# RashmikaDushan/MocapV2

Hardware: AMD Instinct MI355X
Metric: frames/sec (6-cam 1080p) (higher is better)
Workload: dtype u8+int64+f64; 1 GPU; 6-camera 1920x1080 synthetic IR frames, 8 markers (BASELINE.json configs[1]); cameras=6, width=1920, height=1080, markers=8, distortion=mild, frames_resident_in_hbm=True, batches_in_flight=3, resident_batches=3, status_ok=True, input=gray frames, parallelism=single launch, time-major

## Files before the change

include/mocap_hip.h:

```cpp
#ifndef MOCAP_HIP_H
#define MOCAP_HIP_H

#include <stddef.h>
#include <stdint.h>

#ifdef __cplusplus
extern "C" {
#endif

#define MOCAP_ABI_VERSION 7
#define MOCAP_API __attribute__((visibility("default")))

enum {
    MOCAP_OK = 0,
    MOCAP_E_INVALID = -1,
    MOCAP_E_HIP = -2,
    MOCAP_E_UNSUPPORTED = -3,
    MOCAP_E_STATE = -4
};

enum {
    MOCAP_BLOB_E_CANDIDATES = -2,
    MOCAP_BLOB_E_CONTOURS = -3,
    MOCAP_BLOB_E_STEPS = -4,
    MOCAP_BLOB_E_DEPTH = -5,
    MOCAP_CORR_E_GROUPS = -2,
    MOCAP_CORR_E_TRUNCATED = -3,
    MOCAP_CORR_E_BLOB = -4,
    MOCAP_FUND_E_SAMPLE = -2,
    MOCAP_FUND_E_DEGENERATE = -3
};

typedef struct mocap_ctx* mocap_ctx_t;

typedef struct mocap_blob_params {
    int32_t ksize;
    int32_t median;
    double thresh;
    double min_area;
    double min_circ;
} mocap_blob_params;

typedef struct mocap_contour {
    int32_t key, is_hole, sx, sy, npts, steps;
    int64_t a00, a10, a01;
    double area, perimeter;
    int32_t kept, cx, cy, link, parent, order;
} mocap_contour;

MOCAP_API int mocap_abi_version(void);
MOCAP_API const char* mocap_last_error(void);

MOCAP_API int mocap_ctx_create(int device_id, int width, int height, int n_slots, mocap_ctx_t* out);
MOCAP_API int mocap_ctx_destroy(mocap_ctx_t ctx);
MOCAP_API int mocap_sync(mocap_ctx_t ctx, void* stream);

MOCAP_API int mocap_set_blob_params(mocap_ctx_t ctx, const mocap_blob_params* p);

MOCAP_API int mocap_set_tuning(mocap_ctx_t ctx, const char* name, int value);

MOCAP_API int mocap_set_undistort(mocap_ctx_t ctx, int slot, const double K[9], const double dist[5], int* identity_out);

typedef struct mocap_undistort_info_t {
    int32_t identity;
    int32_t compact_table;
    int32_t early_out_provable;
    int32_t max_source_weight;
    int32_t sparse_path;
} mocap_undistort_info_t;
MOCAP_API int mocap_undistort_info(mocap_ctx_t ctx, int slot, mocap_undistort_info_t* out);

MOCAP_API int mocap_set_cameras(mocap_ctx_t ctx, int n, const double* K , const double* dist ,
                      const double* R , const double* t );
MOCAP_API int mocap_set_fundamentals(mocap_ctx_t ctx, int n, const double* F );

MOCAP_API int mocap_blob_centroids(mocap_ctx_t ctx, const void* frames_dev, int n_images, int cam_mod, int slot_base,
                         size_t image_stride, int pitch, int32_t* out_xy_dev, long xy_stride, int32_t* out_count_dev,
                         long count_stride, int max_blobs, void* stream);

MOCAP_API int mocap_filter_mask(mocap_ctx_t ctx, const void* frames_dev, int n_images, int cam_mod, int slot_base,
                      size_t image_stride, int pitch, uint32_t* mask_dev, void* stream);
MOCAP_API int mocap_contours_from_mask(mocap_ctx_t ctx, const uint32_t* mask_dev, int n_images, int32_t* out_xy_dev,
                             long xy_stride, int32_t* out_count_dev, long count_stride, int max_blobs,
                             mocap_contour* dbg_dev , int32_t* dbg_count_dev,
                             int dbg_cap, void* stream);

MOCAP_API int mocap_image_filter_u8(mocap_ctx_t ctx, const void* src_dev, void* dst_dev, int spitch, int dpitch, int order,
                          int slot, void* stream);
MOCAP_API int mocap_undistort_u8(mocap_ctx_t ctx, int slot, const void* src_dev, void* dst_dev, int spitch, int dpitch,
                       void* stream);
MOCAP_API int mocap_box_blur_u8(mocap_ctx_t ctx, const void* src_dev, void* dst_dev, int height, int width, int spitch,
                      int dpitch, int ksize, void* stream);
MOCAP_API int mocap_bayer_gray_u8(mocap_ctx_t ctx, const void* bayer_dev, void* gray_dev, int n_images, int height, int width,
                        long spitch, long dpitch, size_t src_image_stride, size_t dst_image_stride, int pattern,
                        int gray_shift, void* stream);
MOCAP_API int mocap_blob_centroids_bayer(mocap_ctx_t ctx, const void* bayer_frames_dev, void* gray_frames_dev, int n_images,
                               int cam_mod, int slot_base, size_t image_stride, int pitch, int pattern, int gray_shift,
                               int32_t* out_xy_dev, long xy_stride, int32_t* out_count_dev, long count_stride,
                               int max_blobs, void* stream);
MOCAP_API int mocap_demosaic_u8(mocap_ctx_t ctx, const void* bayer_dev, void* bgr_dev, int height, int width, int spitch,
                      void* stream);

MOCAP_API int mocap_correspond(mocap_ctx_t ctx, const void* pts_dev, long pt_stride_t, long pt_stride_c,
                     const int32_t* counts_dev, long cnt_stride_t, long cnt_stride_c, int pts_f64, int T, int C,
                     int P, double cutoff, int max_groups, double* root_xyz_dev, double* root_err_dev,
                     double* root_grp_dev, int32_t* root_idx_dev, int32_t* order_dev, int32_t* n_roots_dev,
                     void* stream);

MOCAP_API int mocap_epipolar_scores(mocap_ctx_t ctx, const void* roots_dev, int n_roots, const void* cand_dev, int n_cand,
                                    int pts_f64, int f_index, double* dist_dev, float* lines_dev, void* stream);

MOCAP_API int mocap_triangulate_batch(mocap_ctx_t ctx, const double* pts_dev, const uint8_t* valid_dev, int N, int C,
                            int compact_k, double* xyz_dev, int32_t* ok_dev, void* stream);
MOCAP_API int mocap_reproject_batch(mocap_ctx_t ctx, const double* pts_dev, const uint8_t* valid_dev, const double* xyz_dev,
                          int N, int C, int compact_k, double* mse_dev, int32_t* ok_dev, void* stream);

MOCAP_API int mocap_ba_residuals(mocap_ctx_t ctx, const double* params_host, int B, const double* pts_dev,
                                 const uint8_t* valid_dev, int N, int C, float* residuals_host, int32_t* counts_host,
                                 void* stream);

MOCAP_API int mocap_fundamental_ransac(mocap_ctx_t ctx, int n_pairs, const double* pts_a_dev, const double* pts_b_dev,
                                       const int32_t* pair_offset_host, const int32_t* samples_dev, int H, double threshold,
                                       int refit, double* F_sample_dev, double* F_refit_dev, uint8_t* inlier_dev,
                                       int32_t* status_dev, int32_t* counts_dev, void* stream);

enum {
    MOCAP_RIG_STOP_MAX_ITERS = 1,
    MOCAP_RIG_STOP_FTOL = 2,
    MOCAP_RIG_STOP_LAMBDA = 3,
    MOCAP_RIG_STOP_CHOLESKY = 4,
    MOCAP_RIG_E_LAYOUT = -2,
    MOCAP_RIG_E_BEHIND = -3
};
MOCAP_API int mocap_rig_bundle_adjust(mocap_ctx_t ctx, int C, int N, int n_obs, const int32_t* obs_offset_dev,
                                      const int32_t* obs_cam_dev, const double* obs_uv_dev, double* poses_dev, double* points_dev,
                                      int max_iters, double ftol, double lambda0, double* history_dev, double* result_dev,
                                      void* stream);
MOCAP_API int mocap_rig_linearize(mocap_ctx_t ctx, int C, int N, int n_obs, const int32_t* obs_offset_dev,
                                  const int32_t* obs_cam_dev, const double* obs_uv_dev, const double* poses_dev,
                                  const double* points_dev, double lambda, double* cost_dev, double* gradient_dev, double* S_dev,
                                  double* rhs_dev, int32_t* status_dev, void* stream);

enum {
    MOCAP_INTR_E_LAYOUT = -2,
    MOCAP_INTR_E_BEHIND = -3,
    MOCAP_INTR_E_DEGENERATE = -4
};
MOCAP_API int mocap_intrinsics_calibrate(mocap_ctx_t ctx, int n_cams, const int32_t* view_offset_host,
                                         const int32_t* point_offset_host, const double* obj_xy_dev, const double* img_uv_dev,
                                         const int32_t* image_size_host, int have_start, int max_iters, double ftol,
                                         double lambda0, double* kd_dev, double* view_poses_dev, double* view_rms_dev,
                                         double* history_dev, double* result_dev, void* stream);
MOCAP_API int mocap_intrinsics_linearize(mocap_ctx_t ctx, int n_cams, const int32_t* view_offset_host,
                                         const int32_t* point_offset_host, const double* obj_xy_dev, const double* img_uv_dev,
                                         const double* kd_dev, const double* view_poses_dev, double lambda, double* cost_dev,
                                         double* gradient_dev, double* S_dev, double* rhs_dev, int32_t* status_dev, void* stream);

#define MOCAP_COMM_ID_BYTES 128
MOCAP_API int mocap_comm_unique_id(void* id_out );
MOCAP_API int mocap_comm_available(void);
MOCAP_API int mocap_comm_init(mocap_ctx_t ctx, const void* id , int rank, int world);
MOCAP_API int mocap_comm_share(mocap_ctx_t dst, mocap_ctx_t src);
MOCAP_API int mocap_comm_destroy(mocap_ctx_t ctx);
MOCAP_API int mocap_allgather_centroids(mocap_ctx_t ctx, const int32_t* local_records_dev, int32_t* gathered_dev,
                                        long ints_per_rank, void* stream);

MOCAP_API int mocap_tile_stats(mocap_ctx_t ctx, uint64_t* tiles, uint64_t* skipped);
MOCAP_API int mocap_profile_enable(mocap_ctx_t ctx, int on);
MOCAP_API int mocap_profile_read(mocap_ctx_t ctx, double ms[5], int launches[5]);

#ifdef __cplusplus
}
#endif
#endif
```

mocapv2_amd/_abi.py:

```python
import ctypes as C
import os

_HERE = os.path.dirname(os.path.abspath(__file__))
LIB_PATH = os.path.join(_HERE, "libmocap_hip.so")
ABI_VERSION = 7
COMM_ID_BYTES = 128


class MocapError(RuntimeError):
    def __init__(self, code, msg):
        super().__init__(f"libmocap_hip error {code}: {msg}")
        self.code = code


class BlobParams(C.Structure):
    _fields_ = [("ksize", C.c_int32), ("median", C.c_int32), ("thresh", C.c_double), ("min_area", C.c_double),
                ("min_circ", C.c_double)]


class UndistortInfo(C.Structure):
    _fields_ = [("identity", C.c_int32), ("compact_table", C.c_int32), ("early_out_provable", C.c_int32),
                ("max_source_weight", C.c_int32), ("sparse_path", C.c_int32)]


class Contour(C.Structure):
    _fields_ = [("key", C.c_int32), ("is_hole", C.c_int32), ("sx", C.c_int32), ("sy", C.c_int32), ("npts", C.c_int32),
                ("steps", C.c_int32), ("a00", C.c_int64), ("a10", C.c_int64), ("a01", C.c_int64), ("area", C.c_double),
                ("perimeter", C.c_double), ("kept", C.c_int32), ("cx", C.c_int32), ("cy", C.c_int32), ("link", C.c_int32),
                ("parent", C.c_int32), ("order", C.c_int32)]


_vp, _i, _d, _sz, _l = C.c_void_p, C.c_int, C.c_double, C.c_size_t, C.c_long
_dp, _ip = C.POINTER(C.c_double), C.POINTER(C.c_int)

SIGNATURES = {
    "mocap_abi_version": [],
    "mocap_last_error": [],
    "mocap_ctx_create": [_i, _i, _i, _i, C.POINTER(_vp)],
    "mocap_ctx_destroy": [_vp],
    "mocap_sync": [_vp, _vp],
    "mocap_set_blob_params": [_vp, C.POINTER(BlobParams)],
    "mocap_set_tuning": [_vp, C.c_char_p, _i],
    "mocap_set_undistort": [_vp, _i, _dp, _dp, _ip],
    "mocap_undistort_info": [_vp, _i, C.POINTER(UndistortInfo)],
    "mocap_set_cameras": [_vp, _i, _dp, _dp, _dp, _dp],
    "mocap_set_fundamentals": [_vp, _i, _dp],
    "mocap_blob_centroids": [_vp, _vp, _i, _i, _i, _sz, _i, _vp, _l, _vp, _l, _i, _vp],
    "mocap_blob_centroids_bayer": [_vp, _vp, _vp, _i, _i, _i, _sz, _i, _i, _i, _vp, _l, _vp, _l, _i, _vp],
    "mocap_filter_mask": [_vp, _vp, _i, _i, _i, _sz, _i, _vp, _vp],
    "mocap_contours_from_mask": [_vp, _vp, _i, _vp, _l, _vp, _l, _i, _vp, _vp, _i, _vp],
    "mocap_image_filter_u8": [_vp, _vp, _vp, _i, _i, _i, _i, _vp],
    "mocap_undistort_u8": [_vp, _i, _vp, _vp, _i, _i, _vp],
    "mocap_box_blur_u8": [_vp, _vp, _vp, _i, _i, _i, _i, _i, _vp],
    "mocap_demosaic_u8": [_vp, _vp, _vp, _i, _i, _i, _vp],
    "mocap_bayer_gray_u8": [_vp, _vp, _vp, _i, _i, _i, _l, _l, _sz, _sz, _i, _i, _vp],
    "mocap_correspond": [_vp, _vp, _l, _l, _vp, _l, _l, _i, _i, _i, _i, _d, _i, _vp, _vp, _vp, _vp, _vp, _vp, _vp],
    "mocap_epipolar_scores": [_vp, _vp, _i, _vp, _i, _i, _i, _vp, _vp, _vp],
    "mocap_ba_residuals": [_vp, _dp, _i, _vp, _vp, _i, _i, C.POINTER(C.c_float), _ip, _vp],
    "mocap_fundamental_ransac": [_vp, _i, _vp, _vp, _ip, _vp, _i, _d, _i, _vp, _vp, _vp, _vp, _vp, _vp],
    "mocap_rig_bundle_adjust": [_vp, _i, _i, _i, _vp, _vp, _vp, _vp, _vp, _i, _d, _d, _vp, _vp, _vp],
    "mocap_rig_linearize": [_vp, _i, _i, _i, _vp, _vp, _vp, _vp, _vp, _d, _vp, _vp, _vp, _vp, _vp, _vp],
    "mocap_intrinsics_calibrate": [_vp, _i, _ip, _ip, _vp, _vp, _ip, _i, _i, _d, _d, _vp, _vp, _vp, _vp, _vp, _vp],
    "mocap_intrinsics_linearize": [_vp, _i, _ip, _ip, _vp, _vp, _vp, _vp, _d, _vp, _vp, _vp, _vp, _vp, _vp],
    "mocap_triangulate_batch": [_vp, _vp, _vp, _i, _i, _i, _vp, _vp, _vp],
    "mocap_reproject_batch": [_vp, _vp, _vp, _vp, _i, _i, _i, _vp, _vp, _vp],
    "mocap_comm_unique_id": [_vp],
    "mocap_comm_available": [],
    "mocap_comm_init": [_vp, _vp, _i, _i],
    "mocap_comm_share": [_vp, _vp],
    "mocap_comm_destroy": [_vp],
    "mocap_allgather_centroids": [_vp, _vp, _vp, _l, _vp],
    "mocap_tile_stats": [_vp, C.POINTER(C.c_uint64), C.POINTER(C.c_uint64)],
    "mocap_profile_enable": [_vp, _i],
    "mocap_profile_read": [_vp, _dp, _ip],
}

_lib = None


def load():
    global _lib
    if _lib is not None:
        return _lib
    if not os.path.exists(LIB_PATH):
        raise RuntimeError(f"{LIB_PATH} is missing: build it with `make -C mocapv2_amd/csrc` "
                           "(hipcc --offload-arch=gfx950); there is no CPU fallback")
    try:
        import torch
    except ImportError:
        pass
    lib = C.CDLL(LIB_PATH)
    for name, args in SIGNATURES.items():
        fn = getattr(lib, name)
        fn.argtypes = args
        fn.restype = C.c_char_p if name == "mocap_last_error" else C.c_int
    if lib.mocap_abi_version() != ABI_VERSION:
        raise RuntimeError(f"libmocap_hip ABI {lib.mocap_abi_version()} != expected {ABI_VERSION}")
    _lib = lib
    return lib


def check(rc):
    if rc != 0:
        msg = load().mocap_last_error()
        raise MocapError(rc, msg.decode() if msg else "")
```

mocapv2_amd/csrc/abi.hip:

```cpp
#include <hip/hip_runtime.h>
#include <stdint.h>
#include <stdio.h>
#include <stdarg.h>
#include <stdlib.h>
#include <string.h>
#include <math.h>
#include <string>
#include <vector>
#include <mutex>
#include <memory>
#include <dlfcn.h>
#include "../../include/mocap_hip.h"
#include "kernels.h"

using namespace mocap;

static_assert(sizeof(mocap_contour) == sizeof(ContourRec), "debug record layout");

static thread_local std::string g_err;

static int fail(int code, const char* fmt, ...)
{
    char buf[512];
    va_list ap;
    va_start(ap, fmt);
    vsnprintf(buf, sizeof(buf), fmt, ap);
    va_end(ap);
    g_err = buf;
    return code;
}

#define HIP_TRY(expr)                                                                                         \
    do {                                                                                                      \
        hipError_t e_ = (expr);                                                                               \
        if (e_ != hipSuccess) return fail(MOCAP_E_HIP, "%s failed: %s", #expr, hipGetErrorString(e_));        \
    } while (0)
#define TRY(expr) do { if (int rc_ = (expr)) return rc_; } while (0)

template <class T, bool Pinned = false>
struct Buf {
    T* p = nullptr;
    size_t n = 0;
    Buf() = default;
    Buf(Buf&& o) : p(o.p), n(o.n) { o.p = nullptr; o.n = 0; }
    Buf& operator=(Buf&& o) { if (this != &o) { release(); p = o.p; n = o.n; o.p = nullptr; o.n = 0; } return *this; }
    ~Buf() { release(); }
    operator T*() const { return p; }
    T* operator->() const { return p; }
    void release()
    {
        if (p) (void)(Pinned ? hipHostFree(p) : hipFree(p));
        p = nullptr; n = 0;
    }
    int reserve(size_t count, bool zero = false)
    {
        if (count <= n) return 0;
        if (p) { HIP_TRY(hipDeviceSynchronize()); release(); }
        HIP_TRY(Pinned ? hipHostMalloc((void**)&p, sizeof(T) * count) : hipMalloc((void**)&p, sizeof(T) * count));
        if (zero) HIP_TRY(hipMemset(p, 0, sizeof(T) * count));
        n = count;
        return 0;
    }
};

struct EvPair { hipEvent_t a, b; };
constexpr size_t PROBE_BYTES = 128 * mocap::PROBE_STRIDE * sizeof(uint32_t);
using mocap::PROBE_STRIDE;

struct SharedComm {
    void* comm = nullptr;
    int rank = 0, world = 1, device = 0;
    hipEvent_t last = nullptr;
    bool have_last = false;
    std::mutex mu;
    bool (*destroy_comm)(void*) = nullptr;
    ~SharedComm()
    {
        if (!comm && !last) return;
        (void)hipSetDevice(device);
        if (last) { if (have_last) (void)hipEventSynchronize(last); (void)hipEventDestroy(last); }
        if (comm && destroy_comm) (void)destroy_comm(comm);
    }
};

struct Tuning {
    int rows = 68;
    int general_filter = 0;
    int skip_dark = 1;
    int dense_boxes = 0;
    int remap_pipeline = 1;
    int cluster = 1;
    int wide_quads_remap = 34, wide_quads_identity = 34;
    int wide_bands = 1;
    int wide_fork = 0;
    int box_prio = 0, scan_prio = 0, contour_prio = 0, corr_prio = 0;
    int box_stage_bytes = BOX_SCAP;
    int box_blocks_per_cu = 0;
    int box_timing = 0, contour_timing = 0, follow_timing = 0;
    int scan_wide = 1;
    int rows_staged = 0;
    int wide_blocks_per_cu = 3;
    int rows_stage_dw = -1;
    int scan_serial = 1;
    int scan_hotmap = 1;
    int scan_blocks_per_cu = 0;
    int scan_slices = 1;
    int excess_base = -1;
    int base_sel = 1;
    int probe_debug = 0;
    int contour_boxes = 1;
    int contours_split = 1;
    int contour_defer = 1;
    int mark_blocks_per_cu = 0;
    int contour_blocks_per_cu = 0;
    int corr_threads = 256;
    int corr_step_groups = 0;
};
struct TuneName { const char* name; int Tuning::*field; int lo, hi; };
static const TuneName kTuneNames[] = {
    {"rows", &Tuning::rows, 16, 68}, {"general_filter", &Tuning::general_filter, 0, 1}, {"skip_dark", &Tuning::skip_dark, 0, 1},
    {"dense_boxes", &Tuning::dense_boxes, 0, 1}, {"remap_pipeline", &Tuning::remap_pipeline, 0, 1}, {"cluster", &Tuning::cluster, 0, 1},
    {"wide_quads_remap", &Tuning::wide_quads_remap, 0, 100000}, {"wide_quads_identity", &Tuning::wide_quads_identity, 0, 100000},
    {"wide_bands", &Tuning::wide_bands, 1, 4}, {"wide_fork", &Tuning::wide_fork, 0, 1},
    {"box_prio", &Tuning::box_prio, 0, 1}, {"scan_prio", &Tuning::scan_prio, 0, 3}, {"contour_prio", &Tuning::contour_prio, 0, 3},
    {"corr_prio", &Tuning::corr_prio, 0, 3}, {"box_stage_bytes", &Tuning::box_stage_bytes, 0, BOX_SCAP},
    {"box_blocks_per_cu", &Tuning::box_blocks_per_cu, 0, 32}, {"box_timing", &Tuning::box_timing, 0, 1},
    {"contour_timing", &Tuning::contour_timing, 0, 1}, {"follow_timing", &Tuning::follow_timing, 0, 2}, {"scan_wide", &Tuning::scan_wide, 0, 1}, {"scan_hotmap", &Tuning::scan_hotmap, 0, 2}, {"scan_serial", &Tuning::scan_serial, 0, 1}, {"rows_staged", &Tuning::rows_staged, 0, 1}, {"wide_blocks_per_cu", &Tuning::wide_blocks_per_cu, 1, 8}, {"rows_stage_dw", &Tuning::rows_stage_dw, -1, 1 << 20}, {"scan_blocks_per_cu", &Tuning::scan_blocks_per_cu, 0, 64}, {"scan_slices", &Tuning::scan_slices, 1, 64}, {"excess_base", &Tuning::excess_base, -1, 254},
    {"base_sel", &Tuning::base_sel, 0, 1}, {"probe_debug", &Tuning::probe_debug, 0, 1}, {"contour_boxes", &Tuning::contour_boxes, 0, 1},
    {"contours_split", &Tuning::contours_split, 0, 1}, {"contour_blocks_per_cu", &Tuning::contour_blocks_per_cu, 0, 16}, {"mark_blocks_per_cu", &Tuning::mark_blocks_per_cu, 0, 16}, {"contour_defer", &Tuning::contour_defer, 0, 2}, {"corr_threads", &Tuning::corr_threads, 64, 256},
    {"corr_step_groups", &Tuning::corr_step_groups, 0, 0x7fffffff},
};
static bool tune_set(Tuning& t, const char* name, int v)
{
    for (const TuneName& n : kTuneNames)
        if (!strcmp(n.name, name)) {
            t.*(n.field) = v < n.lo ? n.lo : (v > n.hi ? n.hi : v);
            return true;
        }
    return false;
}
static Tuning tuning_from_env()
{
    Tuning t;
    for (const TuneName& n : kTuneNames) {
        char env[64] = "MOCAP_";
        size_t k = strlen(env);
        for (const char* p = n.name; *p && k + 1 < sizeof(env); p++) env[k++] = (char)((*p >= 'a' && *p <= 'z') ? *p - 32 : *p);
        env[k] = 0;
        const char* e = getenv(env);
        if (e && *e) tune_set(t, n.name, atoi(e));
    }
    { const char* e = getenv("MOCAP_WIDE_QUADS"); int r_ = 0, i_ = 0;
      if (e && sscanf(e, "%d,%d", &r_, &i_) == 2) { tune_set(t, "wide_quads_remap", r_); tune_set(t, "wide_quads_identity", i_); } }
    return t;
}

struct mocap_ctx {
    int device = 0, W = 0, H = 0, n_slots = 0, wpr = 0;
    int box_grid = 2048;
    int n_cu = 256;
    mocap_blob_params prm{5, 5, 255 * 0.85, 500.0, 0.5};
    Tuning tune;
    Buf<uint32_t> maps;
    Buf<uint32_t> map4;
    Buf<ushort4> srcbox;
    Buf<ushort4> rowbox;
    Buf<uint32_t> map_flags;
    std::vector<int> slot_state;
    std::vector<int> slot_compact;
    std::vector<uint32_t> slot_wmax;
    Buf<uint2> reach;
    Buf<uint8_t> cflags;
    Buf<uint32_t> mask; size_t mask_images = 0;
    bool mask_dirty = false;
    Buf<uint32_t> cells;
    int last_images = 0;
    Buf<uint32_t> hotmap;
    Buf<uint32_t> tile_rows;
    int tile_rows_flip = 0;
    int tile_rows_hold[2] = {0, 0};
    Buf<uint32_t> cur_box;
    Buf<BoxItem> items;
    Buf<uint4> wide_tiles;
    Buf<uint32_t> n_items;
    hipStream_t side = nullptr; hipEvent_t ev_fork = nullptr, ev_join = nullptr;
    int base_sel = 1; int probe_age = 0; bool probe_pending = false; Buf<uint32_t> probe_dev; Buf<uint32_t, true> probe_host; hipEvent_t probe_ev = nullptr;
    bool walk_count_zeroed = false;
    int probe_images = 0;
    bool hot_dense = false;
    Buf<uint32_t> cells_ext, cur_box_ext; size_t cells_ext_images = 0;
    Buf<uint32_t> mask_out;
    Buf<uint32_t> mask_in;
    Buf<uint8_t> gray_scratch;
    Buf<uint8_t> cwork; size_t cwork_images = 0;
    Buf<uint64_t> walk_list, link_list;
    Buf<uint32_t> walk_count;
    Buf<CameraTable> cams; int n_cam = 0, n_F = 0;
    Buf<double> scratch;
    Buf<double> ba_obj;
    Buf<char> fund_scratch;
    Buf<char> rig_scratch;
    Buf<char> intr_scratch;
    Buf<char, true> ba_pinned;
    std::shared_ptr<struct SharedComm> comm;
    bool profiling = false;
    std::vector<EvPair> ev[5];
    std::mutex mu;
};

static int set_device(mocap_ctx* c) { HIP_TRY(hipSetDevice(c->device)); return 0; }

struct ScanTurn { std::mutex mu; hipEvent_t done = nullptr; bool have = false; };
static ScanTurn g_scan_turn[64];

struct Tiling { int rows, n_cgroups, n_strips; };
static Tiling tiling(const mocap_ctx* c)
{
    Tiling t;
    t.rows = c->tune.rows;
    if (c->H < 4 * 32) t.rows = (c->H + 3) / 4 > 8 ? (c->H + 3) / 4 : 8;
    t.n_cgroups = (c->H + 4 * t.rows - 1) / (4 * t.rows);
    t.n_strips = (c->W + 239) / 240;
    return t;
}

static size_t source_cells(const mocap_ctx* c) { return (size_t)((c->H + 7) / 8) * ((c->W + 7) / 8); }
static size_t cells_per_image(const mocap_ctx* c) { Tiling t = tiling(c); return (size_t)t.n_cgroups * 4 * t.n_strips; }
static uint32_t* slot_map(const mocap_ctx* c, int slot) { return c->maps ? c->maps + (size_t)slot * c->H * c->W : nullptr; }
static uint32_t* slot_mapw(const mocap_ctx* c, int slot) { return c->maps ? c->maps + (size_t)(c->n_slots + slot) * c->H * c->W : nullptr; }
static uint32_t* slot_map4(const mocap_ctx* c, int slot) { return c->map4 ? c->map4 + (size_t)slot * c->H * c->W : nullptr; }

struct IdBytes { char internal[MOCAP_COMM_ID_BYTES]; };
namespace {
struct Rccl {
    void* lib = nullptr;
    int (*GetUniqueId)(void*) = nullptr;
    int (*CommInitRank)(void**, int, IdBytes, int) = nullptr;
    int (*CommDestroy)(void*) = nullptr;
    int (*AllGather)(const void*, void*, size_t, int, void*, hipStream_t) = nullptr;
    const char* (*GetErrorString)(int) = nullptr;
};
}
static Rccl g_rccl;
static std::mutex g_rccl_mu;
static int load_rccl()
{
    std::lock_guard<std::mutex> lk(g_rccl_mu);
    if (g_rccl.lib) return 0;
    void* h = dlopen("librccl.so.1", RTLD_NOW | RTLD_GLOBAL);
    if (!h) h = dlopen("librccl.so", RTLD_NOW | RTLD_GLOBAL);
    if (!h) h = dlopen("/opt/rocm/lib/librccl.so.1", RTLD_NOW | RTLD_GLOBAL);
    if (!h) return fail(MOCAP_E_UNSUPPORTED, "librccl.so.1 not found: %s", dlerror());
    Rccl r;
    r.GetUniqueId = (decltype(r.GetUniqueId))dlsym(h, "ncclGetUniqueId");
    r.CommInitRank = (decltype(r.CommInitRank))dlsym(h, "ncclCommInitRank");
    r.CommDestroy = (decltype(r.CommDestroy))dlsym(h, "ncclCommDestroy");
    r.AllGather = (decltype(r.AllGather))dlsym(h, "ncclAllGather");
    r.GetErrorString = (decltype(r.GetErrorString))dlsym(h, "ncclGetErrorString");
    if (!r.GetUniqueId || !r.CommInitRank || !r.CommDestroy || !r.AllGather || !r.GetErrorString)
        return fail(MOCAP_E_UNSUPPORTED, "librccl lacks an expected symbol");
    r.lib = h;
    g_rccl = r;
    return 0;
}
#define RCCL_TRY(expr)                                                                                        \
    do {                                                                                                      \
        int r_ = (expr);                                                                                      \
        if (r_ != 0) return fail(MOCAP_E_HIP, "%s failed: %s", #expr, g_rccl.GetErrorString(r_));             \
    } while (0)

struct Carver {
    char* base;
    size_t used = 0;
    template <class T> void take(T*& p, size_t count) { p = base ? (T*)(base + used) : nullptr; used += (sizeof(T) * count + 15) & ~(size_t)15; }
};

extern "C" {

int mocap_abi_version(void) { return MOCAP_ABI_VERSION; }
const char* mocap_last_error(void) { return g_err.c_str(); }

int mocap_ctx_create(int device_id, int width, int height, int n_slots, mocap_ctx_t* out)
{
    if (!out || width < 1 || height < 1 || width > 32767 || height > 32767 || n_slots < 1 || n_slots > 64)
        return fail(MOCAP_E_INVALID, "mocap_ctx_create: bad geometry %dx%d slots=%d", width, height, n_slots);
    int ndev = 0;
    HIP_TRY(hipGetDeviceCount(&ndev));
    if (device_id < 0 || device_id >= ndev) return fail(MOCAP_E_HIP, "mocap_ctx_create: no HIP device %d (%d visible)", device_id, ndev);
    HIP_TRY(hipSetDevice(device_id));
    std::unique_ptr<mocap_ctx, int (*)(mocap_ctx*)> c(new mocap_ctx(), mocap_ctx_destroy);
    c->device = device_id; c->W = width; c->H = height; c->n_slots = n_slots; c->wpr = (width + 31) / 32;
    c->tune = tuning_from_env();
    c->base_sel = c->tune.base_sel;
    {
        hipDeviceProp_t prop;
        if (hipGetDeviceProperties(&prop, device_id) == hipSuccess && prop.multiProcessorCount > 0) {
            c->box_grid = box_filter_blocks_per_cu() * prop.multiProcessorCount;
            c->n_cu = prop.multiProcessorCount;
            if (c->tune.box_blocks_per_cu >= 1) c->box_grid = c->tune.box_blocks_per_cu * prop.multiProcessorCount;
        }
    }
    c->slot_state.assign(n_slots, 0);
    c->slot_compact.assign(n_slots, 0);
    c->slot_wmax.assign(n_slots, 0);
    TRY(c->map_flags.reserve(n_slots + 64, true));
    TRY(c->n_items.reserve(256, true));
    TRY(c->probe_dev.reserve(PROBE_BYTES / sizeof(uint32_t)));
    TRY(c->probe_host.reserve(PROBE_BYTES / sizeof(uint32_t)));
    HIP_TRY(hipEventCreateWithFlags(&c->probe_ev, hipEventDisableTiming));
    HIP_TRY(hipEventCreateWithFlags(&c->ev_fork, hipEventDisableTiming));
    HIP_TRY(hipEventCreateWithFlags(&c->ev_join, hipEventDisableTiming));
    TRY(c->cams.reserve(1, true));
    *out = c.release();
    return MOCAP_OK;
}

int mocap_ctx_destroy(mocap_ctx_t c)
{
    if (!c) return MOCAP_OK;
    (void)hipSetDevice(c->device);
    for (auto& v : c->ev) for (auto& p : v) { (void)hipEventDestroy(p.a); (void)hipEventDestroy(p.b); }
    (void)mocap_comm_destroy(c);
    if (c->side) { (void)hipStreamSynchronize(c->side); (void)hipStreamDestroy(c->side); }
    if (c->ev_fork) (void)hipEventDestroy(c->ev_fork);
    if (c->ev_join) (void)hipEventDestroy(c->ev_join);
    if (c->probe_ev) { (void)hipEventSynchronize(c->probe_ev); (void)hipEventDestroy(c->probe_ev); }
    delete c;
    return MOCAP_OK;
}

int mocap_sync(mocap_ctx_t c, void* stream)
{
    if (!c) return fail(MOCAP_E_INVALID, "null context");
// ... 30 lines not shown
    std::lock_guard<std::mutex> lk(c->mu);
    size_t per = (size_t)c->H * c->W;
    TRY(c->maps.reserve(per * c->n_slots * 2));
    TRY(c->map4.reserve(per * c->n_slots + 4));
    const int ncx_ = (c->W + 7) / 8, ncy_ = (c->H + 7) / 8;
    TRY(c->srcbox.reserve((size_t)ncx_ * ncy_ * c->n_slots));
    const int n_strips_ = tiling(c).n_strips;
    TRY(c->rowbox.reserve((size_t)c->H * n_strips_ * c->n_slots));
    MapArgs m;
    memcpy(m.K, K, sizeof(m.K));
    memcpy(m.dist, dist, sizeof(m.dist));
    m.H = c->H; m.W = c->W;
    m.map = slot_map(c, slot);
    m.mapw = slot_mapw(c, slot);
    m.map4 = slot_map4(c, slot);
    m.flags = c->map_flags + slot;
    HIP_TRY(hipMemset(m.flags, 0, sizeof(uint32_t)));
    launch_undistort_map(m, 0);
    HIP_TRY(hipGetLastError());
    uint32_t flags = 0;
    HIP_TRY(hipMemcpy(&flags, m.flags, sizeof(flags), hipMemcpyDeviceToHost));
    c->slot_state[slot] = (flags & 1u) ? 2 : 1;
    c->slot_compact[slot] = (flags & 2u) ? 0 : 1;
    c->slot_wmax[slot] = c->slot_state[slot] == 1 ? 1024u : 0u;
    launch_srcbox(m.map4, c->srcbox + (size_t)ncx_ * ncy_ * slot, c->H, c->W, 0);
    HIP_TRY(hipGetLastError());
    launch_rowbox(m.map4, c->rowbox + (size_t)c->H * n_strips_ * slot, c->H, c->W, n_strips_, 0);
    HIP_TRY(hipGetLastError());
    std::vector<uint32_t> edge((size_t)ncx_ * ncy_, 0);
    std::vector<int> reach32((size_t)ncx_ * ncy_ * 4);
    for (size_t i = 0; i < reach32.size(); i += 2) { reach32[i] = 0x7fffffff; reach32[i + 1] = -0x7fffffff - 1; }
    if (c->slot_state[slot] == 2) {
        Buf<uint32_t> tmp;
        const size_t edge_words = edge.size();
        TRY(tmp.reserve(per + 4 + edge_words + reach32.size()));
        HIP_TRY(hipMemset(tmp, 0, sizeof(uint32_t) * (per + 4 + edge_words)));
        int* reach_dev = (int*)(tmp + per + 4 + edge_words);
        HIP_TRY(hipMemcpy(reach_dev, reach32.data(), sizeof(int) * reach32.size(), hipMemcpyHostToDevice));
        uint32_t st3[3] = {0, 0, 0};
        StatArgs sg{m.map, m.mapw, tmp, tmp + per, c->H, c->W, tmp + per + 4, reach_dev};
        launch_remap_stats(sg, 0);
        HIP_TRY(hipGetLastError());
        HIP_TRY(hipMemcpy(st3, tmp + per, sizeof(st3), hipMemcpyDeviceToHost));
        HIP_TRY(hipMemcpy(edge.data(), tmp + per + 4, sizeof(uint32_t) * edge.size(), hipMemcpyDeviceToHost));
        HIP_TRY(hipMemcpy(reach32.data(), reach_dev, sizeof(int) * reach32.size(), hipMemcpyDeviceToHost));
        if (st3[1] <= 9 && st3[2] <= 9 && c->W >= 8) c->slot_wmax[slot] = st3[0];
    }
    {
        const int H = c->H, W = c->W, ncx = ncx_, ncy = ncy_;
        std::vector<uint2> reach((size_t)ncx * ncy);
        std::vector<uint8_t> cflags((size_t)ncx * ncy);
        for (int cr = 0; cr < ncy; cr++)
            for (int cx = 0; cx < ncx; cx++) {
                const size_t i = (size_t)cr * ncx + cx;
                int x0, x1, y0, y1;
                if (c->slot_state[slot] == 1) {
                    x0 = 8 * cx; x1 = 8 * cx + 7 < W - 1 ? 8 * cx + 7 : W - 1; y0 = 8 * cr; y1 = 8 * cr + 7 < H - 1 ? 8 * cr + 7 : H - 1;
                    const bool xc = 8 * cx < 4 || 8 * cx + 7 >= W - 4, yc = 8 * cr < 4 || 8 * cr + 7 >= H - 4;
                    edge[i] = (xc && yc) ? 2u : (xc || yc) ? 1u : 0u;
                } else {
                    x0 = reach32[4 * i]; x1 = reach32[4 * i + 1]; y0 = reach32[4 * i + 2]; y1 = reach32[4 * i + 3];
                }
                if (x0 > x1 || y0 > y1) reach[i] = make_uint2(1u, 0u);
                else reach[i] = make_uint2((uint32_t)x0 | ((uint32_t)x1 << 16), (uint32_t)y0 | ((uint32_t)y1 << 16));
                cflags[i] = (edge[i] & 2u) ? 2 : (edge[i] & 1u) ? 1 : 0;
            }
        TRY(c->reach.reserve(reach.size() * c->n_slots));
        HIP_TRY(hipMemcpy(c->reach + reach.size() * slot, reach.data(), sizeof(uint2) * reach.size(), hipMemcpyHostToDevice));
        TRY(c->cflags.reserve(cflags.size() * c->n_slots));
        HIP_TRY(hipMemcpy(c->cflags + cflags.size() * slot, cflags.data(), cflags.size(), hipMemcpyHostToDevice));
    }
    if (identity_out) *identity_out = c->slot_state[slot] == 1;
    return MOCAP_OK;
}

int mocap_undistort_info(mocap_ctx_t c, int slot, mocap_undistort_info_t* out)
{
    if (!c || !out) return fail(MOCAP_E_INVALID, "null argument");
    if (slot < 0 || slot >= c->n_slots) return fail(MOCAP_E_INVALID, "slot %d out of range", slot);
    if (c->slot_state[slot] == 0) return fail(MOCAP_E_STATE, "mocap_set_undistort was not called for slot %d", slot);
    out->identity = c->slot_state[slot] == 1;
    out->compact_table = c->slot_compact[slot] != 0 && c->W >= 8;
    out->early_out_provable = c->slot_wmax[slot] != 0 && c->W >= 8;
    out->max_source_weight = (int32_t)c->slot_wmax[slot];
    out->sparse_path = out->compact_table && out->early_out_provable && c->tune.skip_dark && !c->tune.general_filter;
    return MOCAP_OK;
}

int mocap_set_cameras(mocap_ctx_t c, int n, const double* K, const double* dist, const double* R, const double* t)
{
    if (!c || !K || !dist || !R || !t) return fail(MOCAP_E_INVALID, "null argument");
    if (n < 1 || n > 32) return fail(MOCAP_E_INVALID, "camera count %d not in 1..32", n);
    if (set_device(c)) return MOCAP_E_HIP;
    HIP_TRY(hipMemcpy(&c->cams->K[0][0], K, sizeof(double) * 9 * n, hipMemcpyHostToDevice));
    HIP_TRY(hipMemcpy(&c->cams->dist[0][0], dist, sizeof(double) * 5 * n, hipMemcpyHostToDevice));
    HIP_TRY(hipMemcpy(&c->cams->R[0][0], R, sizeof(double) * 9 * n, hipMemcpyHostToDevice));
    HIP_TRY(hipMemcpy(&c->cams->t[0][0], t, sizeof(double) * 3 * n, hipMemcpyHostToDevice));
    c->n_cam = n;
    return MOCAP_OK;
}

int mocap_set_fundamentals(mocap_ctx_t c, int n, const double* F)
{
    if (!c || (n > 0 && !F)) return fail(MOCAP_E_INVALID, "null argument");
    if (n < 0 || n > 31) return fail(MOCAP_E_INVALID, "fundamental matrix count %d not in 0..31", n);
    if (set_device(c)) return MOCAP_E_HIP;
    if (n) HIP_TRY(hipMemcpy(&c->cams->F[0][0], F, sizeof(double) * 9 * n, hipMemcpyHostToDevice));
    c->n_F = n;
    return MOCAP_OK;
}

static void prof_begin(mocap_ctx* c, int which, hipStream_t s, EvPair& p, bool& on)
{
    on = c->profiling;
    if (!on) return;
    if (hipEventCreate(&p.a) != hipSuccess || hipEventCreate(&p.b) != hipSuccess) { on = false; return; }
    (void)hipEventRecord(p.a, s);
    (void)which;
}
static void prof_end(mocap_ctx* c, int which, hipStream_t s, EvPair& p, bool on)
{
    if (!on) return;
    (void)hipEventRecord(p.b, s);
    std::lock_guard<std::mutex> lk(c->mu);
    c->ev[which].push_back(p);
}

int mocap_profile_enable(mocap_ctx_t c, int on)
{
    if (!c) return fail(MOCAP_E_INVALID, "null context");
    c->profiling = on != 0;
    return MOCAP_OK;
}

int mocap_profile_read(mocap_ctx_t c, double ms[5], int cnt[5])
{
    if (!c || !ms || !cnt) return fail(MOCAP_E_INVALID, "null argument");
    if (set_device(c)) return MOCAP_E_HIP;
    for (int w = 0; w < 5; w++) { ms[w] = 0; cnt[w] = 0; }
    std::lock_guard<std::mutex> lk(c->mu);
    for (int w = 0; w < 5; w++) {
        for (auto& p : c->ev[w]) {
            HIP_TRY(hipEventSynchronize(p.b));
            float f = 0;
            HIP_TRY(hipEventElapsedTime(&f, p.a, p.b));
            ms[w] += f; cnt[w]++;
            (void)hipEventDestroy(p.a); (void)hipEventDestroy(p.b);
        }
        c->ev[w].clear();
    }
    return MOCAP_OK;
}

int mocap_tile_stats(mocap_ctx_t c, uint64_t* tiles, uint64_t* skipped)
{
    if (!c) return fail(MOCAP_E_INVALID, "null context");
    if (set_device(c)) return MOCAP_E_HIP;
    uint64_t total = 0, full = 0;
    if (c->cells && c->last_images > 0) {
        HIP_TRY(hipDeviceSynchronize());
        Tiling t = tiling(c);
        size_t per = cells_per_image(c), n = per * (size_t)c->last_images;
        std::vector<uint32_t> w(n);
        HIP_TRY(hipMemcpy(w.data(), c->cells, sizeof(uint32_t) * n, hipMemcpyDeviceToHost));
        int valid_chunks = (c->H + t.rows - 1) / t.rows;
        total = (uint64_t)c->last_images * valid_chunks * t.n_strips;
        for (size_t i = 0; i < n; i++) full += w[i] >> 31;
    }
    if (tiles) *tiles = total;
    if (skipped) *skipped = total - full;
    return MOCAP_OK;
}

static int check_frames(mocap_ctx* c, const void* frames, int n_images, int cam_mod, int slot_base, size_t image_stride, int pitch)
{
    if (!c || !frames) return fail(MOCAP_E_INVALID, "null argument");
    if (n_images < 1) return fail(MOCAP_E_INVALID, "n_images = %d", n_images);
    if (cam_mod < 1 || slot_base < 0 || slot_base + cam_mod > c->n_slots)
        return fail(MOCAP_E_INVALID, "slots %d..%d not in 0..%d", slot_base, slot_base + cam_mod - 1, c->n_slots - 1);
    if (pitch < c->W) return fail(MOCAP_E_INVALID, "pitch %d < width %d", pitch, c->W);
    if (n_images > 1 && image_stride < (size_t)pitch * (c->H - 1) + c->W) return fail(MOCAP_E_INVALID, "image_stride too small");
    for (int s = slot_base; s < slot_base + cam_mod; s++)
        if (c->slot_state[s] == 0) return fail(MOCAP_E_STATE, "mocap_set_undistort was not called for slot %d", s);
    return 0;
}


static int excess_base(int thr_mul, int sel)
{
    int c = sel ? thr_mul - 67 : thr_mul - 154;
    if (c > thr_mul - 1) c = thr_mul - 1;
    if (c > 254) c = 254;
    return c < 0 ? 0 : c;
}

static int ensure_gray_scratch(mocap_ctx* c, size_t bytes)
{
    if (bytes <= c->gray_scratch.n) return 0;
    std::lock_guard<std::mutex> lk(c->mu);
    return c->gray_scratch.reserve(bytes);
}

static int threshold_mul(const mocap_ctx* c)
{
    const double ft = floor(c->prm.thresh);
    return ft < -1.0 ? 0 : (ft > 255.0 ? 256 : (int)ft + 1);
}

static FilterArgs filter_args(const mocap_ctx* c, const void* src, size_t image_stride, int pitch, uint32_t* mask, uint32_t* cells,
                              int slot_base, int cam_mod, int n_images, int thr_mul)
{
    const Tiling tl = tiling(c);
    FilterArgs a{};
    a.src = (const uint8_t*)src; a.image_stride = image_stride; a.pitch = pitch; a.H = c->H; a.W = c->W;
    a.mask = mask; a.words_per_row = c->wpr; a.cam_mod = cam_mod; a.cells = cells;
    a.n_images = n_images; a.n_steps = (n_images + cam_mod - 1) / cam_mod;
    a.thr_mul = thr_mul;
    a.n_strips = tl.n_strips; a.rows_per_chunk = tl.rows; a.n_cgroups = tl.n_cgroups;
    a.pipelined = c->W >= 4 && (c->W & 3) == 0 && c->H >= 2;
    if (slot_base >= 0) {
        a.map = slot_map(c, slot_base); a.mapw = slot_mapw(c, slot_base); a.map4 = slot_map4(c, slot_base);
        a.rowbox = c->rowbox ? c->rowbox + (size_t)slot_base * c->H * tl.n_strips : nullptr;
    }
    return a;
}

struct Batch {
    int n_images, cam_mod, slot_base;
    size_t image_stride; int pitch;
    uint32_t* mask; uint32_t* cells;
    bool own_mask;
    hipStream_t s;
};

static void read_probe(mocap_ctx* c, int thr_mul)
{
    if (!c->probe_pending || hipEventQuery(c->probe_ev) != hipSuccess) return;
    unsigned long long n_cur = 0, n_alt = 0;
    for (int i = 0; i < 128; i++) { n_cur += c->probe_host[PROBE_STRIDE * i]; n_alt += c->probe_host[PROBE_STRIDE * i + 1]; }
    if (c->tune.probe_debug) fprintf(stderr, "[probe] base %d: %llu hot cells, alternative %d: %llu\n", excess_base(thr_mul, c->base_sel), n_cur, excess_base(thr_mul, c->base_sel ^ 1), n_alt);
    const unsigned long long n_lo = c->base_sel == 0 ? n_cur : n_alt, n_hi = c->base_sel == 0 ? n_alt : n_cur;
    c->base_sel = (n_lo * 4 <= n_hi * 5) ? 0 : 1;
    const unsigned long long n_now = c->base_sel == 0 ? n_lo : n_hi;
    c->hot_dense = c->probe_images > 0 && n_now > 400ull * (unsigned long long)c->probe_images;
    c->probe_pending = false;
}

struct ScanBounds {
    int thr_mul;
    int fixed_base;
    int base, base_alt;
    int allow, allow_cut1, allow_cut2, allow_alt;
};
static ScanBounds scan_bounds(const mocap_ctx* c, int slot_base, int cam_mod, int thr_mul)
{
    ScanBounds b{thr_mul, c->tune.excess_base, 0, 0, -1, -1, -1, -1};
    if (b.fixed_base >= 0) { if (b.fixed_base > thr_mul - 1) b.fixed_base = thr_mul - 1; if (b.fixed_base > 254) b.fixed_base = 254; if (b.fixed_base < 0) b.fixed_base = 0; }
    b.base = b.fixed_base >= 0 ? b.fixed_base : excess_base(thr_mul, c->base_sel);
    b.base_alt = excess_base(thr_mul, c->base_sel ^ 1);
    long long wmax = 0;
    bool ok = true;
    for (int sl = slot_base; sl < slot_base + cam_mod; sl++) {
        if (c->slot_wmax[sl] == 0) ok = false;
        wmax = c->slot_wmax[sl] > wmax ? c->slot_wmax[sl] : wmax;
    }
    auto t5 = [](int n) { return (n - 1 < 2 ? n - 1 : 2) + 1; };
    auto t5full = [](int n) { return n < 5 ? n : 5; };
    const long long per_tap = 1024LL * (2LL * thr_mul - 2LL * b.base - 1), per_tap_alt = 1024LL * (2LL * thr_mul - 2LL * b.base_alt - 1);
    if (!c->tile_rows || !c->reach || !c->cflags) ok = false;
    if (ok && wmax > 0 && per_tap > 0) {
        b.allow = (int)((per_tap * t5full(c->W) * t5full(c->H) - 1) / wmax);
        const long long taps1 = t5(c->W) * t5full(c->H) < t5full(c->W) * t5(c->H) ? t5(c->W) * t5full(c->H) : t5full(c->W) * t5(c->H);
        b.allow_cut1 = (int)((per_tap * taps1 - 1) / wmax);
        b.allow_cut2 = (int)((per_tap * t5(c->W) * t5(c->H) - 1) / wmax);
        if (per_tap_alt > 0) b.allow_alt = (int)((per_tap_alt * t5full(c->W) * t5full(c->H) - 1) / wmax);
    }
    if (!c->tune.skip_dark) b.allow = -1;
    return b;
}

struct FilterPath {
    bool remap;
    bool compact;
    bool rows_staged;
    bool direct;
    bool bayer;
    uint64_t remap_bits;
    int rows_dw;
    const void* frames;
    BayerArgs bl;
};
static int choose_path(mocap_ctx* c, const Batch& bt, const void* frames, const BayerArgs* bayer, int allow, FilterPath& p)
{
    p = FilterPath{};
    p.compact = c->W >= 8 && bt.cam_mod <= 64;
    for (int sl = bt.slot_base; sl < bt.slot_base + bt.cam_mod; sl++) {
        if (c->slot_state[sl] == 2) { p.remap = true; if (sl - bt.slot_base < 64) p.remap_bits |= 1ull << (sl - bt.slot_base); }
        if (c->slot_state[sl] == 2 && !c->slot_compact[sl]) p.compact = false;
    }
    if (c->tune.general_filter) p.compact = false;
    p.rows_staged = p.remap && c->tune.rows_staged && c->map4 && c->rowbox && (c->W & 15) == 0 && c->H >= 2;
    for (int sl = bt.slot_base; sl < bt.slot_base + bt.cam_mod; sl++)
        if (!c->slot_compact[sl]) p.rows_staged = false;
    p.rows_dw = c->tune.rows_stage_dw < 0 || c->tune.rows_stage_dw > rows_stage_dwords() ? rows_stage_dwords() : c->tune.rows_stage_dw;
    if (allow < 0 && !c->tune.dense_boxes) p.compact = false;
    p.frames = frames;
    p.bayer = bayer != nullptr;
    if (bayer) p.bl = *bayer;
    if (bayer && !bayer->dst) {
        p.direct = p.compact && allow >= 0 && bt.own_mask && bayer_scan_direct(p.bl);
        if (!p.direct) {
            const size_t bytes = (size_t)(bt.n_images - 1) * bt.image_stride + (size_t)(c->H - 1) * bt.pitch + c->W;
            TRY(ensure_gray_scratch(c, bytes));
            p.bl.dst = c->gray_scratch;
        }
        p.frames = p.direct ? (const void*)p.bl.src : (const void*)p.bl.dst;
    }
    return 0;
}

static int filter_dense(mocap_ctx* c, const Batch& bt, const FilterPath& p, int thr_mul)
{
    FilterArgs a = filter_args(c, p.frames, bt.image_stride, bt.pitch, bt.mask, bt.cells, bt.slot_base, bt.cam_mod, bt.n_images, thr_mul);
    if (!c->tune.remap_pipeline) a.pipelined = 0;
    a.staged = p.rows_staged; a.stage_dw = p.rows_dw;
    if (p.bayer) { launch_bayer_gray(p.bl, bt.s); HIP_TRY(hipGetLastError()); }
    if (bt.own_mask) c->mask_dirty = true;
    EvPair ev; bool on;
    prof_begin(c, 0, bt.s, ev, on);
    launch_filter_mask(a, p.remap, bt.s);
    prof_end(c, 0, bt.s, ev, on);
    HIP_TRY(hipGetLastError());
    return 0;
}

static BoxArgs box_args(const mocap_ctx* c, const Batch& bt, const FilterPath& p, const ScanBounds& sb)
{
    const Tiling tl = tiling(c);
    BoxArgs a{};
    a.src = (const uint8_t*)p.frames; a.image_stride = bt.image_stride; a.pitch = bt.pitch; a.H = c->H; a.W = c->W;
    a.mask = bt.mask; a.words_per_row = c->wpr; a.cells = bt.cells;
    a.map4 = slot_map4(c, bt.slot_base);
    a.srcbox = c->srcbox ? c->srcbox + (size_t)bt.slot_base * source_cells(c) : nullptr;
    a.remap_bits = p.remap_bits;
    a.cam_mod = bt.cam_mod; a.n_images = bt.n_images; a.n_steps = (bt.n_images + bt.cam_mod - 1) / bt.cam_mod;
    a.thr_mul = sb.thr_mul;
    a.rows_per_chunk = tl.rows; a.n_strips = tl.n_strips; a.n_chunks = tl.n_cgroups * 4;
    const size_t tr_words = c->mask_images * cells_per_image(c) * 4;
    a.tile_rows = c->tile_rows + (c->tile_rows_flip ? tr_words : 0);
    a.tile_rows_next = c->tile_rows + (c->tile_rows_flip ? 0 : tr_words);
    a.n_clear = c->tile_rows_hold[c->tile_rows_flip ^ 1];
    a.cluster = c->tune.cluster;
    a.cur_box = bt.own_mask ? c->cur_box : c->cur_box_ext;
    a.items = c->items; a.n_items = c->n_items; a.cap_items = (uint32_t)c->items.n;
    a.dense = sb.allow < 0;
    a.wide_tiles = c->wide_tiles; a.cap_wide = (uint32_t)c->wide_tiles.n; a.wide_quads_remap = c->tune.wide_quads_remap; a.wide_quads_identity = c->tune.wide_quads_identity;
    a.wide_bands = c->tune.wide_bands;
    if (c->W < 4 || p.direct) a.wide_tiles = nullptr;
    a.bayer = p.direct ? p.bl : BayerArgs{};
    a.stage_bytes = c->tune.box_stage_bytes;
    a.prio = c->tune.box_prio;
    a.ext_mask = bt.own_mask ? 0 : 1;
    return a;
}

static BrightArgs bright_args(const mocap_ctx* c, const Batch& bt, const FilterPath& p, const ScanBounds& sb, uint32_t* tile_rows, bool scan_zeroes)
{
    const Tiling tl = tiling(c);
    uint64_t ncx64 = (uint64_t)((c->W + 7) / 8);
    const uint64_t ncells = ncx64 * (uint64_t)((c->H + 7) / 8);
    int wide = (c->W % 16 == 0) && (bt.pitch % 16 == 0) && (bt.image_stride % 16 == 0) && (((uintptr_t)p.frames & 15) == 0) && ncx64 >= 4;
    if (wide && ncells * (ncx64 / 2) >= (1ull << 32)) wide = 0;
    if (!c->tune.scan_wide) wide = 0;
    if (wide) ncx64 /= 2;
    const uint32_t ncx_magic = (ncx64 > 1 && ncells * ncx64 < (1ull << 32)) ? (uint32_t)(((1ull << 32) + ncx64 - 1) / ncx64) : 0u;
    BrightArgs b{(const uint8_t*)p.frames, bt.image_stride, bt.pitch, c->H, c->W, bt.n_images, bt.cam_mod, ncx_magic, wide, sb.base, sb.allow / 4, sb.allow_cut1 / 4, sb.allow_cut2 / 4,
                 c->reach + (size_t)bt.slot_base * source_cells(c), c->cflags + (size_t)bt.slot_base * source_cells(c),
                 tile_rows, tl.n_cgroups * 4, tl.n_strips, (uint32_t)(((1u << 23) + tl.rows - 1) / tl.rows),
                 bt.mask, bt.own_mask ? 0 : (size_t)bt.n_images * mask_image_words(c->H, c->wpr), ((uintptr_t)bt.mask & 15) == 0, nullptr, sb.base_alt, sb.allow_alt / 4, 0};
    b.prio = c->tune.scan_prio;
    b.max_blocks = c->tune.scan_blocks_per_cu * c->n_cu; b.blocks_x = 0;
    b.zero_counters = scan_zeroes ? c->n_items.p : nullptr;
    b.block_ctr = c->n_items + 160;
    b.slices = c->tune.scan_slices; b.image0 = 0; b.slice_images = bt.n_images;
    return b;
}

static int scan_tiles(mocap_ctx* c, const Batch& bt, const FilterPath& p, const ScanBounds& sb, uint32_t* tile_rows, bool scan_zeroes,
                      BrightArgs& b, bool& mark_after_scan)
{
    const hipStream_t s = bt.s;
    b = bright_args(c, bt, p, sb, tile_rows, scan_zeroes);
    const bool probe = sb.fixed_base < 0 && !c->probe_pending && sb.allow_alt >= 0 && sb.base_alt != sb.base && !p.bayer &&
                       (c->probe_age == 0 || c->probe_age >= 32);
    if (probe) {
        HIP_TRY(hipMemsetAsync(c->probe_dev, 0, PROBE_BYTES, s));
        b.probe = c->probe_dev;
    }
    c->probe_age = probe ? 1 : c->probe_age + 1;
    const bool fused = p.bayer && bt.own_mask && (p.direct || bayer_scan_fusable(p.bl));
    const bool two_step = !fused && c->hotmap && (c->tune.scan_hotmap == 2 || (c->tune.scan_hotmap == 1 && c->hot_dense));
    if (two_step) { b.hotmap = c->hotmap; b.hot_words = hot_map_words(c->H, c->W, b.wide); b.mark_grid = c->tune.mark_blocks_per_cu * c->n_cu; }
    ScanTurn* turn = c->tune.scan_serial && c->device >= 0 && c->device < 64 ? &g_scan_turn[c->device] : nullptr;
    std::unique_lock<std::mutex> turn_lock;
    if (turn) {
        turn_lock = std::unique_lock<std::mutex>(turn->mu);
        if (!turn->done) HIP_TRY(hipEventCreateWithFlags(&turn->done, hipEventDisableTiming));
        if (turn->have) HIP_TRY(hipStreamWaitEvent(s, turn->done, 0));
    }
    EvPair ev; bool on;
    prof_begin(c, 3, s, ev, on);
    if (fused) launch_bayer_gray_scan(p.bl, b, s);
    else {
        if (p.bayer) launch_bayer_gray(p.bl, s);
        launch_bright_cells(b, s);
    }
    prof_end(c, 3, s, ev, on);
    HIP_TRY(hipGetLastError());
    if (turn) {
        HIP_TRY(hipEventRecord(turn->done, s));
        turn->have = true;
        turn_lock.unlock();
    }
    mark_after_scan = two_step;
    if (probe) {
        HIP_TRY(hipMemcpyAsync(c->probe_host, c->probe_dev, PROBE_BYTES, hipMemcpyDeviceToHost, s));
        HIP_TRY(hipEventRecord(c->probe_ev, s));
        c->probe_pending = true;
        c->probe_images = (bt.n_images + 15) / 16;
    }
    return 0;
}

static int settle_tiles(mocap_ctx* c, const BoxArgs& a, const BrightArgs& mark_args, bool mark_after_scan, hipStream_t s)
{
    EvPair ev; bool on;
    prof_begin(c, 4, s, ev, on);
    if (mark_after_scan) {
        launch_mark_tiles(mark_args, s);
        HIP_TRY(hipGetLastError());
    }
    launch_settle_tiles(a, s);
    prof_end(c, 4, s, ev, on);
    HIP_TRY(hipGetLastError());
    if (!a.dense) {
        if (a.n_images > c->tile_rows_hold[c->tile_rows_flip]) c->tile_rows_hold[c->tile_rows_flip] = a.n_images;
        c->tile_rows_hold[c->tile_rows_flip ^ 1] = 0;
        c->tile_rows_flip ^= 1;
    }
    return 0;
}

static int report_box_timing(mocap_ctx* c, const uint64_t* timing, hipStream_t s)
{
    std::vector<uint64_t> t((size_t)6 * c->box_grid);
    HIP_TRY(hipStreamSynchronize(s));
    HIP_TRY(hipMemcpy(t.data(), timing, sizeof(uint64_t) * t.size(), hipMemcpyDeviceToHost));
    double sum[6] = {0, 0, 0, 0, 0, 0}, mx = 0;
    for (int b = 0; b < c->box_grid; b++) {
        double tot = 0;
        for (int i = 0; i < 6; i++) { sum[i] += (double)t[6 * b + i]; if (i < 5) tot += (double)t[6 * b + i]; }
        mx = tot > mx ? tot : mx;
    }
    const double n = sum[5] > 0 ? sum[5] : 1;
    uint32_t cnt[16];
    HIP_TRY(hipMemcpy(cnt, c->n_items, sizeof(cnt), hipMemcpyDeviceToHost));
    fprintf(stderr, "[box] list: %u items, %u wide-tile entries\n", cnt[0], cnt[8]);
    fprintf(stderr, "[box] items %.0f (%.1f per wave) | cycles per item: header+wait %.0f, stage %.0f, patch %.0f, threshold %.0f, majority+next %.0f | busiest wave %.0f cycles\n",
            sum[5], sum[5] / c->box_grid, sum[0] / n, sum[1] / n, sum[2] / n, sum[3] / n, sum[4] / n, mx);
    return 0;
}

static int filter_boxes(mocap_ctx* c, const Batch& bt, const FilterPath& p, BoxArgs& a)
{
    const hipStream_t s = bt.s;
    Buf<uint64_t> timing;
    if (c->tune.box_timing) {
        TRY(timing.reserve((size_t)6 * c->box_grid));
        HIP_TRY(hipMemsetAsync(timing, 0, sizeof(uint64_t) * 6 * c->box_grid, s));
    }
    a.timing = timing;
    EvPair ev; bool on;
    prof_begin(c, 0, s, ev, on);
    const bool fork_wide = c->tune.wide_fork != 0;
    if (a.wide_tiles) {
        FilterArgs f = filter_args(c, a.src, bt.image_stride, bt.pitch, bt.mask, bt.cells, bt.slot_base, bt.cam_mod, bt.n_images, a.thr_mul);
        f.tiles = c->wide_tiles; f.n_tiles = c->n_items + 8; f.cap_tiles = a.cap_wide;
        f.staged = p.rows_staged; f.stage_dw = p.rows_dw;
        hipStream_t ws = s;
        if (fork_wide) {
            HIP_TRY(hipEventRecord(c->ev_fork, s));
            if (!c->side) HIP_TRY(hipStreamCreateWithFlags(&c->side, hipStreamNonBlocking));
            HIP_TRY(hipStreamWaitEvent(c->side, c->ev_fork, 0));
            ws = c->side;
        }
        launch_filter_tiles(f, p.remap, c->tune.wide_blocks_per_cu * c->n_cu, ws);
        HIP_TRY(hipGetLastError());
        if (fork_wide) HIP_TRY(hipEventRecord(c->ev_join, c->side));
    }
    launch_box_filter(a, c->box_grid, s, p.direct);
    HIP_TRY(hipGetLastError());
    if (a.wide_tiles && fork_wide) HIP_TRY(hipStreamWaitEvent(s, c->ev_join, 0));
    prof_end(c, 0, s, ev, on);
    return timing ? report_box_timing(c, timing, s) : 0;
}

static int run_filter(mocap_ctx* c, const void* frames, int n_images, int cam_mod, int slot_base, size_t image_stride,
                      int pitch, uint32_t* mask, uint32_t* cells, hipStream_t s, const BayerArgs* bayer = nullptr)
{
    const Batch bt{n_images, cam_mod, slot_base, image_stride, pitch, mask, cells, mask == c->mask, s};
    c->walk_count_zeroed = false;
    if (cells == c->cells) c->last_images = n_images;
    const int thr_mul = threshold_mul(c);
    read_probe(c, thr_mul);
    const ScanBounds sb = scan_bounds(c, slot_base, cam_mod, thr_mul);
    FilterPath p;
    TRY(choose_path(c, bt, frames, bayer, sb.allow, p));
    if (!p.compact) return filter_dense(c, bt, p, thr_mul);
    if (bt.own_mask && c->mask_dirty) {
        HIP_TRY(hipMemsetAsync(c->mask, 0, sizeof(uint32_t) * c->mask_images * mask_image_words(c->H, c->wpr), s));
        std::vector<uint32_t> init(c->mask_images * cells_per_image(c) * 4);
        for (size_t i = 0; i < init.size(); i += 4) { init[i] = 1u; init[i + 1] = 1u; init[i + 2] = 1u; init[i + 3] = 1u; }
        HIP_TRY(hipStreamSynchronize(s));
        HIP_TRY(hipMemcpy(c->cur_box, init.data(), sizeof(uint32_t) * init.size(), hipMemcpyHostToDevice));
        c->mask_dirty = false;
    }
    BoxArgs a = box_args(c, bt, p, sb);
    if ((size_t)n_images * cells_per_image(c) * BOX_MAX_PARTS > c->items.n) return fail(MOCAP_E_STATE, "work list smaller than the batch");
    const bool scan_zeroes = !a.dense && !p.bayer && c->tune.scan_blocks_per_cu == 0 && c->tune.scan_slices <= 1;
    if (!scan_zeroes) HIP_TRY(hipMemsetAsync(c->n_items, 0, 1024, s));
    a.zero8 = bt.own_mask ? c->walk_count.p : nullptr;
    c->walk_count_zeroed = a.zero8 != nullptr;
    BrightArgs mark_args{}; bool mark_after_scan = false;
    if (!a.dense) TRY(scan_tiles(c, bt, p, sb, a.tile_rows, scan_zeroes, mark_args, mark_after_scan));
    else if (p.bayer) {
        launch_bayer_gray(p.bl, s);
        HIP_TRY(hipGetLastError());
    }
    TRY(settle_tiles(c, a, mark_args, mark_after_scan, s));
    return filter_boxes(c, bt, p, a);
}

static const uint32_t* contour_boxes(mocap_ctx* c)
{
    return (c->mask_dirty || !c->tune.contour_boxes) ? nullptr : c->cur_box;
}

static int ensure_contour_work(mocap_ctx* c, size_t n_images)
{
    if (n_images <= c->cwork_images) return 0;
    std::lock_guard<std::mutex> lk(c->mu);
    if (n_images <= c->cwork_images) return 0;
    c->cwork_images = 0;
    int rc = c->cwork.reserve(contour_work_bytes() * n_images);
    if (!rc) rc = c->walk_list.reserve((contour_walk_bytes() * n_images + 7) / 8);
    if (!rc) rc = c->link_list.reserve(((contour_link_bytes() + sizeof(uint32_t)) * n_images + 7) / 8);
    if (!rc) rc = c->walk_count.reserve(64);
    if (rc) { c->cwork.release(); c->walk_list.release(); c->link_list.release(); return rc; }
    c->cwork_images = n_images;
    return 0;
}

static int report_follow_timing(const uint64_t* follow_dbg, int follow_grid, hipStream_t s)
{
    std::vector<uint64_t> t((size_t)8 * follow_grid);
    HIP_TRY(hipStreamSynchronize(s));
    HIP_TRY(hipMemcpy(t.data(), follow_dbg, sizeof(uint64_t) * t.size(), hipMemcpyDeviceToHost));
    double sum[8] = {0, 0, 0, 0, 0, 0, 0, 0}, mx[3] = {0, 0, 0}, mxsteps = 0; int used = 0;
    for (int b = 0; b < follow_grid; b++) {
        if (t[8 * b + 5] == 0) continue;
        used++;
        for (int i = 0; i < 8; i++) sum[i] += (double)t[8 * b + i];
        for (int i = 0; i < 3; i++) mx[i] = (double)t[8 * b + i] > mx[i] ? (double)t[8 * b + i] : mx[i];
        mxsteps = (double)t[8 * b + 3] > mxsteps ? (double)t[8 * b + 3] : mxsteps;
    }
    const double u = used ? used : 1;
    fprintf(stderr, "[follow] %d of %d waves had work | per wave (mean / max us): store %.1f / %.1f, refill %.1f / %.1f, walk %.1f / %.1f | wave steps %.0f (max %.0f), "
                    "lanes alive per step %.1f, walks %.1f, refills %.1f | us per wave step %.3f\n",
            used, follow_grid, sum[0] / u / 100, mx[0] / 100, sum[1] / u / 100, mx[1] / 100, sum[2] / u / 100, mx[2] / 100, sum[3] / u, mxsteps,
            sum[3] > 0 ? sum[4] / sum[3] : 0.0, sum[5] / u, sum[6] / u, sum[3] > 0 ? sum[2] / 100 / sum[3] : 0.0);
    return 0;
}

static int report_contour_timing(const uint64_t* timing, int n_images, hipStream_t s)
{
    std::vector<uint64_t> t((size_t)8 * n_images);
    HIP_TRY(hipStreamSynchronize(s));
    HIP_TRY(hipMemcpy(t.data(), timing, sizeof(uint64_t) * t.size(), hipMemcpyDeviceToHost));
    double sum[4] = {0, 0, 0, 0}, mx = 0; uint64_t lo = ~0ull, hi = 0;
    for (int i = 0; i < n_images; i++) {
        for (int k = 0; k < 4; k++) sum[k] += (double)(t[8 * i + k + 1] - t[8 * i + k]);
        double tot = (double)(t[8 * i + 4] - t[8 * i]); mx = tot > mx ? tot : mx;
        lo = t[8 * i] < lo ? t[8 * i] : lo; hi = t[8 * i + 4] > hi ? t[8 * i + 4] : hi;
    }
    {
        int worst = 0; double wt = 0, sc = 0, ss = 0;
        for (int i = 0; i < n_images; i++) {
            double tot = (double)(t[8 * i + 4] - t[8 * i]);
            if (tot > wt) { wt = tot; worst = i; }
            sc += (double)t[8 * i + 5]; ss += (double)t[8 * i + 6];
        }
        fprintf(stderr, "[contours] slowest image %d: %.1f us, candidates %llu, longest border %llu steps, borders %llu | mean candidates %.1f, mean longest border %.1f steps\n",
                worst, wt / 100, (unsigned long long)t[8 * worst + 5], (unsigned long long)t[8 * worst + 6], (unsigned long long)t[8 * worst + 7],
                sc / n_images, ss / n_images);
    }
    fprintf(stderr, "[contours] mean us per block: candidates %.1f follow %.1f link %.1f order %.1f | slowest block %.1f | first start to last end %.1f\n",
            sum[0] / n_images / 100, sum[1] / n_images / 100, sum[2] / n_images / 100, sum[3] / n_images / 100, mx / 100, (double)(hi - lo) / 100);
    return 0;
}

static int run_contours(mocap_ctx* c, const uint32_t* mask, const uint32_t* cells, const uint32_t* boxes, int n_images, int32_t* out_xy, long xy_stride,
                        int32_t* out_count, long count_stride, int max_blobs, mocap_contour* dbg, int32_t* dbg_count, int dbg_cap, hipStream_t s)
{
    ContourArgs a;
    a.mask = mask; a.words_per_row = c->wpr; a.H = c->H; a.W = c->W; a.n_images = n_images;
    a.out_xy = out_xy; a.out_count = out_count; a.max_blobs = max_blobs;
    a.xy_stride = xy_stride; a.count_stride = count_stride;
    a.min_area = c->prm.min_area; a.min_circ = c->prm.min_circ;
    a.dbg = (ContourRec*)dbg; a.dbg_count = dbg_count; a.dbg_cap = dbg_cap;
    long long ms = 4LL * c->H * c->W + 16;
    a.max_steps = ms > (1 << 22) ? (1 << 22) : (int)ms;
    Tiling tl = tiling(c);
    a.cells = cells; a.boxes = boxes; a.rows_per_chunk = tl.rows; a.n_chunks = tl.n_cgroups * 4; a.n_strips = tl.n_strips;
    if ((long long)a.n_chunks * a.n_strips * ((tl.rows + 7) / 8) > 65535 || c->wpr > 4096) a.cells = nullptr;
    TRY(ensure_contour_work(c, n_images));
    a.work = c->cwork;
    const bool split = c->tune.contours_split != 0;
    a.walk_list = split ? c->walk_list : nullptr; a.link_list = c->link_list; a.walk_count = c->walk_count;
    a.follow_grid = c->n_cu * 4;
    a.follow_grid2 = c->n_cu;
    a.image_grid = c->tune.contour_blocks_per_cu * c->n_cu;
    a.counters_zeroed = mask == c->mask && c->walk_count_zeroed;
    c->walk_count_zeroed = false;
    a.defer_links = c->tune.contour_defer == 2 || (c->tune.contour_defer == 1 && c->hot_dense);
    a.wait_list = (uint32_t*)((uint8_t*)c->link_list.p + contour_link_bytes() * c->cwork_images);
    a.follow_list = 0; a.tree_pass = 0; a.follow_dbg_list = c->tune.follow_timing == 2 ? 1 : 0;
    Buf<uint64_t> follow_dbg, timing;
    if (c->tune.follow_timing && split) {
        TRY(follow_dbg.reserve((size_t)8 * a.follow_grid));
        HIP_TRY(hipMemsetAsync(follow_dbg, 0, sizeof(uint64_t) * 8 * a.follow_grid, s));
    }
    a.follow_dbg = follow_dbg;
    a.prio = c->tune.contour_prio;
    if (c->tune.contour_timing) {
        TRY(timing.reserve((size_t)8 * n_images));
        HIP_TRY(hipMemsetAsync(timing, 0, sizeof(uint64_t) * 8 * n_images, s));
    }
    a.timing = timing;
    EvPair p; bool on;
    prof_begin(c, 1, s, p, on);
    launch_contours(a, s);
    prof_end(c, 1, s, p, on);
    HIP_TRY(hipGetLastError());
    if (follow_dbg) TRY(report_follow_timing(follow_dbg, a.follow_grid, s));
    if (timing) TRY(report_contour_timing(timing, n_images, s));
    return 0;
}

static int grow_mask_group(mocap_ctx* c, size_t n_images)
{
    const size_t tiles = n_images * cells_per_image(c);
    TRY(c->mask.reserve(n_images * mask_image_words(c->H, c->wpr), true));
    TRY(c->cells.reserve(tiles, true));
    std::vector<uint32_t> init(tiles * 4);
    for (size_t i = 0; i < init.size(); i += 2) { init[i] = 0xffffffffu; init[i + 1] = 0u; }
    TRY(c->tile_rows.reserve(2 * init.size()));
    HIP_TRY(hipMemcpy(c->tile_rows, init.data(), sizeof(uint32_t) * init.size(), hipMemcpyHostToDevice));
    HIP_TRY(hipMemcpy(c->tile_rows + init.size(), init.data(), sizeof(uint32_t) * init.size(), hipMemcpyHostToDevice));
    const int hw0 = hot_map_words(c->H, c->W, 0), hw1 = hot_map_words(c->H, c->W, 1);
    TRY(c->hotmap.reserve(n_images * (hw0 > hw1 ? hw0 : hw1), true));
    for (size_t i = 0; i < init.size(); i++) init[i] = 1u;
    TRY(c->cur_box.reserve(init.size()));
    HIP_TRY(hipMemcpy(c->cur_box, init.data(), sizeof(uint32_t) * init.size(), hipMemcpyHostToDevice));
    const size_t cap = tiles * BOX_MAX_PARTS;
    if (cap > 0xffffffffull) return fail(MOCAP_E_UNSUPPORTED, "batch too large for the work list");
    TRY(c->items.reserve(cap));
    return c->wide_tiles.reserve(4 * tiles);
}
static int ensure_mask(mocap_ctx* c, int n_images)
{
    if ((size_t)n_images <= c->mask_images) return 0;
    std::lock_guard<std::mutex> lk(c->mu);
    if ((size_t)n_images <= c->mask_images) return 0;
    c->mask_images = 0; c->last_images = 0;
    if (int rc = grow_mask_group(c, n_images)) {
        c->mask.release(); c->cells.release(); c->tile_rows.release(); c->hotmap.release(); c->cur_box.release();
        c->items.release(); c->wide_tiles.release();
        return rc;
    }
    c->tile_rows_flip = 0; c->tile_rows_hold[0] = c->tile_rows_hold[1] = 0;
    c->mask_dirty = false;
    c->mask_images = n_images;
    return 0;
}

static int ensure_blocked(mocap_ctx* c, Buf<uint32_t>& m, int n_images)
{
    const size_t words = (size_t)n_images * mask_image_words(c->H, c->wpr);
    if (words <= m.n) return 0;
    std::lock_guard<std::mutex> lk(c->mu);
    return m.reserve(words, true);
}

static int ensure_ext(mocap_ctx* c, int n_images)
{
    if ((size_t)n_images <= c->cells_ext_images) return 0;
    std::lock_guard<std::mutex> lk(c->mu);
    if ((size_t)n_images <= c->cells_ext_images) return 0;
    c->cells_ext_images = 0;
    int rc = c->cells_ext.reserve((size_t)n_images * cells_per_image(c));
    if (!rc) rc = c->cur_box_ext.reserve(4 * (size_t)n_images * cells_per_image(c));
    if (rc) { c->cells_ext.release(); c->cur_box_ext.release(); return rc; }
    c->cells_ext_images = n_images;
    return 0;
}

int mocap_filter_mask(mocap_ctx_t c, const void* frames, int n_images, int cam_mod, int slot_base, size_t image_stride,
                      int pitch, uint32_t* mask_dev, void* stream)
{
    int rc = check_frames(c, frames, n_images, cam_mod, slot_base, image_stride, pitch);
    if (rc) return rc;
    if (!mask_dev) return fail(MOCAP_E_INVALID, "null mask");
    if (set_device(c)) return MOCAP_E_HIP;
    if ((rc = ensure_mask(c, n_images))) return rc;
    if ((rc = ensure_ext(c, n_images))) return rc;
    if ((rc = ensure_blocked(c, c->mask_out, n_images))) return rc;
    if ((rc = run_filter(c, frames, n_images, cam_mod, slot_base, image_stride, pitch, c->mask_out, c->cells_ext, (hipStream_t)stream)))
        return rc;
    launch_mask_convert(c->mask_out, mask_dev, n_images, c->H, c->wpr, false, (hipStream_t)stream);
    HIP_TRY(hipGetLastError());
    return MOCAP_OK;
}

int mocap_contours_from_mask(mocap_ctx_t c, const uint32_t* mask_dev, int n_images, int32_t* out_xy, long xy_stride,
                             int32_t* out_count, long count_stride, int max_blobs, mocap_contour* dbg, int32_t* dbg_count,
                             int dbg_cap, void* stream)
{
    if (!c || !mask_dev || !out_xy || !out_count) return fail(MOCAP_E_INVALID, "null argument");
    if (n_images < 1 || max_blobs < 1 || xy_stride < 2L * max_blobs || count_stride < 1)
        return fail(MOCAP_E_INVALID, "n_images=%d max_blobs=%d strides %ld %ld", n_images, max_blobs, xy_stride, count_stride);
    if ((dbg != nullptr) != (dbg_count != nullptr) || (dbg && dbg_cap < 1)) return fail(MOCAP_E_INVALID, "inconsistent debug buffers");
    if (set_device(c)) return MOCAP_E_HIP;
    int rc = ensure_blocked(c, c->mask_in, n_images);
    if (rc) return rc;
    launch_mask_convert(mask_dev, c->mask_in, n_images, c->H, c->wpr, true, (hipStream_t)stream);
    HIP_TRY(hipGetLastError());
    return run_contours(c, c->mask_in, nullptr, nullptr, n_images, out_xy, xy_stride, out_count, count_stride, max_blobs, dbg, dbg_count, dbg_cap,
                        (hipStream_t)stream);
}

int mocap_blob_centroids(mocap_ctx_t c, const void* frames, int n_images, int cam_mod, int slot_base, size_t image_stride,
                         int pitch, int32_t* out_xy, long xy_stride, int32_t* out_count, long count_stride, int max_blobs,
                         void* stream)
{
    int rc = check_frames(c, frames, n_images, cam_mod, slot_base, image_stride, pitch);
    if (rc) return rc;
    if (!out_xy || !out_count || max_blobs < 1 || xy_stride < 2L * max_blobs || count_stride < 1)
        return fail(MOCAP_E_INVALID, "bad output arguments");
    if (set_device(c)) return MOCAP_E_HIP;
    if ((rc = ensure_mask(c, n_images))) return rc;
    if ((rc = run_filter(c, frames, n_images, cam_mod, slot_base, image_stride, pitch, c->mask, c->cells, (hipStream_t)stream))) return rc;
    return run_contours(c, c->mask, c->cells, contour_boxes(c), n_images, out_xy, xy_stride, out_count, count_stride, max_blobs, nullptr, nullptr, 0,
                        (hipStream_t)stream);
}

static int bayer_args(BayerArgs& a, const void* bayer, void* gray, int n_images, int H, int W, long spitch, long dpitch,
                      size_t src_image_stride, size_t dst_image_stride, int pattern, int gray_shift, bool gray_optional = false);

int mocap_blob_centroids_bayer(mocap_ctx_t c, const void* bayer_frames, void* gray_frames, int n_images, int cam_mod, int slot_base,
                               size_t image_stride, int pitch, int pattern, int gray_shift, int32_t* out_xy, long xy_stride,
                               int32_t* out_count, long count_stride, int max_blobs, void* stream)
{
    int rc = check_frames(c, bayer_frames, n_images, cam_mod, slot_base, image_stride, pitch);
    if (rc) return rc;
    if (!out_xy || !out_count || max_blobs < 1 || xy_stride < 2L * max_blobs || count_stride < 1)
        return fail(MOCAP_E_INVALID, "bad output arguments");
    BayerArgs b;
    if ((rc = bayer_args(b, bayer_frames, gray_frames, n_images, c->H, c->W, pitch, pitch, image_stride, image_stride, pattern, gray_shift,
                         true)))
        return rc;
    if (set_device(c)) return MOCAP_E_HIP;
    if ((rc = ensure_mask(c, n_images))) return rc;
    if ((rc = run_filter(c, gray_frames, n_images, cam_mod, slot_base, image_stride, pitch, c->mask, c->cells, (hipStream_t)stream, &b)))
        return rc;
    return run_contours(c, c->mask, c->cells, contour_boxes(c), n_images, out_xy, xy_stride, out_count, count_stride, max_blobs, nullptr, nullptr, 0,
                        (hipStream_t)stream);
}

int mocap_undistort_u8(mocap_ctx_t c, int slot, const void* src, void* dst, int spitch, int dpitch, void* stream)
{
    if (!c || !src || !dst) return fail(MOCAP_E_INVALID, "null argument");
    if (slot < 0 || slot >= c->n_slots || c->slot_state[slot] == 0) return fail(MOCAP_E_STATE, "undistort slot %d not set", slot);
    if (spitch < c->W || dpitch < c->W) return fail(MOCAP_E_INVALID, "pitch < width");
    if (set_device(c)) return MOCAP_E_HIP;
    launch_undistort((const uint8_t*)src, (uint8_t*)dst, c->H, c->W, spitch, dpitch, slot_map(c, slot), slot_mapw(c, slot), (hipStream_t)stream);
    HIP_TRY(hipGetLastError());
    return MOCAP_OK;
}

int mocap_image_filter_u8(mocap_ctx_t c, const void* src, void* dst, int spitch, int dpitch, int order, int slot, void* stream)
{
    if (!c || !src || !dst) return fail(MOCAP_E_INVALID, "null argument");
    if (order != 0 && order != 1) return fail(MOCAP_E_INVALID, "order must be 0 (image_filter_gpu) or 1 (image_filter_cpu)");
    if (spitch < c->W || dpitch < c->W) return fail(MOCAP_E_INVALID, "pitch < width");
    if (slot >= c->n_slots || (slot >= 0 && c->slot_state[slot] == 0)) return fail(MOCAP_E_STATE, "undistort slot %d not set", slot);
    if (set_device(c)) return MOCAP_E_HIP;
    hipStream_t s = (hipStream_t)stream;
    const int thr_mul = threshold_mul(c), ithresh = thr_mul - 1;
    if (order == 1) {
        const uint8_t* in = (const uint8_t*)src;
        int ip = spitch;
        if (slot >= 0 && c->slot_state[slot] == 2) {
            return fail(MOCAP_E_UNSUPPORTED, "image_filter_cpu order with undistortion: call mocap_undistort_u8 first");
        }
        launch_median5(in, (uint8_t*)dst, c->H, c->W, ip, dpitch, ithresh, 1, s);
        HIP_TRY(hipGetLastError());
        return MOCAP_OK;
    }
    int rc = ensure_mask(c, 1);
    if (rc) return rc;
    const FilterArgs a = filter_args(c, src, 0, spitch, c->mask, c->cells, slot, 1, 1, thr_mul);
    c->mask_dirty = true; c->last_images = 1;
    launch_filter_mask(a, slot >= 0 && c->slot_state[slot] == 2, s);
    HIP_TRY(hipGetLastError());
    launch_mask_expand(c->mask, c->wpr, (uint8_t*)dst, c->H, c->W, dpitch, s);
    HIP_TRY(hipGetLastError());
    return MOCAP_OK;
}

int mocap_box_blur_u8(mocap_ctx_t c, const void* src, void* dst, int H, int W, int spitch, int dpitch, int ksize, void* stream)
{
    if (!c || !src || !dst) return fail(MOCAP_E_INVALID, "null argument");
    if (H < 1 || W < 1 || spitch < W || dpitch < W || ksize < 1 || ksize > 31) return fail(MOCAP_E_INVALID, "bad geometry");
    if (set_device(c)) return MOCAP_E_HIP;
    launch_box_blur((const uint8_t*)src, (uint8_t*)dst, H, W, spitch, dpitch, ksize, (hipStream_t)stream);
    HIP_TRY(hipGetLastError());
    return MOCAP_OK;
}

// ... 439 lines not shown
```

mocapv2_amd/csrc/bayer_gray.hip:

```cpp
#include <hip/hip_runtime.h>
#include <stdint.h>
#include "kernels.h"
#include "scan_mark.h"
#include "bayer.h"

namespace mocap {

__device__ __forceinline__ uint32_t wave_prev(uint32_t v) { return (uint32_t)__builtin_amdgcn_update_dpp(0, (int)v, 0x138, 0xf, 0xf, true); }
__device__ __forceinline__ uint32_t wave_next(uint32_t v) { return (uint32_t)__builtin_amdgcn_update_dpp(0, (int)v, 0x130, 0xf, 0xf, true); }

template <int ND> struct RowPairs { uint32_t e[ND], o[ND], Le[ND], Ro[ND]; };

template <int ND, bool NEED_LE, bool NEED_RO>
__device__ __forceinline__ RowPairs<ND> row_pairs(const uint32_t (&w)[ND])
{
    RowPairs<ND> r;
#pragma unroll
    for (int i = 0; i < ND; i++) {
        r.e[i] = prm(0, w[i], 0x0c020c00u);
        r.o[i] = prm(0, w[i], 0x0c030c01u);
    }
    if (NEED_LE) {
        const uint32_t pw = wave_prev(w[ND - 1]);
        r.Le[0] = prm(pw, w[0], 0x0c010c07u);
// ... 9 lines not shown
    return r;
}

template <int ND> struct LaneLoad;
template <> struct LaneLoad<2> { typedef uint2 type; };
template <> struct LaneLoad<4> { typedef uint4 type; };

template <int ND>
__global__ __launch_bounds__(256) void bayer_gray_kernel(BayerArgs a)
{
    constexpr int PX = 4 * ND, WAVE_PX = 62 * PX;
    typedef typename LaneLoad<ND>::type vec_t;
    const int lane = threadIdx.x;
    const int y = __builtin_amdgcn_readfirstlane(blockIdx.y * 4 + threadIdx.y);
    if (y >= a.H) return;
    const int x0 = blockIdx.x * WAVE_PX - PX + PX * lane;
    const int yc = y < 1 ? 1 : (y > a.H - 2 ? a.H - 2 : y);
    const uint8_t* __restrict__ src = a.src + (size_t)blockIdx.z * a.sstride + (size_t)(yc - 1) * a.spitch;
    const bool in = x0 >= 0 && x0 < a.W;
    const uint32_t off = in ? (uint32_t)x0 : 0u;
    uint32_t wu[ND], wc[ND], wd[ND];
    {
        const vec_t vu = *(const vec_t*)(src + off), vc = *(const vec_t*)(src + a.spitch + off), vd = *(const vec_t*)(src + 2 * a.spitch + off);
        __builtin_memcpy(wu, &vu, sizeof(vu)); __builtin_memcpy(wc, &vc, sizeof(vc)); __builtin_memcpy(wd, &vd, sizeof(vd));
    }
    if (!in) {
#pragma unroll
        for (int i = 0; i < ND; i++) wu[i] = wc[i] = wd[i] = 0u;
    }

    const bool red_row = (yc & 1) == a.ry;
    const bool even_is_colour = (red_row ? a.rx : 1 - a.rx) == 0;
    const uint32_t cx = red_row ? a.cr : a.cb, cy = red_row ? a.cb : a.cr;
    const LumaCoef k{cx, a.cg, cy, cx << 16, a.cg << 16, cy << 16, 1u << (a.shift - 1), a.shift};

    uint32_t g[PX];
    const RowPairs<ND> C = row_pairs<ND, true, true>(wc);
    if (even_is_colour) {
        const RowPairs<ND> U = row_pairs<ND, true, false>(wu), D = row_pairs<ND, true, false>(wd);
#pragma unroll
        for (int i = 0; i < ND; i++) {
            luma2(C.e[i], mean4(C.Le[i], C.o[i], U.e[i], D.e[i]), mean4(U.Le[i], U.o[i], D.Le[i], D.o[i]), k, g[4 * i], g[4 * i + 2]);
            luma2(mean2(C.e[i], C.Ro[i]), C.o[i], mean2(U.o[i], D.o[i]), k, g[4 * i + 1], g[4 * i + 3]);
        }
    } else {
        const RowPairs<ND> U = row_pairs<ND, false, true>(wu), D = row_pairs<ND, false, true>(wd);
#pragma unroll
        for (int i = 0; i < ND; i++) {
            luma2(mean2(C.Le[i], C.o[i]), C.e[i], mean2(U.e[i], D.e[i]), k, g[4 * i], g[4 * i + 2]);
            luma2(C.o[i], mean4(C.e[i], C.Ro[i], U.o[i], D.o[i]), mean4(U.e[i], U.Ro[i], D.e[i], D.Ro[i]), k, g[4 * i + 1], g[4 * i + 3]);
        }
    }
    if (x0 == 0) g[0] = g[1];
    if (x0 + PX == a.W) g[PX - 1] = g[PX - 2];
    if (in && lane >= 1 && lane <= 62) {
        uint32_t out[ND];
#pragma unroll
        for (int i = 0; i < ND; i++) out[i] = g[4 * i] | (g[4 * i + 1] << 8) | (g[4 * i + 2] << 16) | (g[4 * i + 3] << 24);
        vec_t v;
        __builtin_memcpy(&v, out, sizeof(v));
        *(vec_t*)(a.dst + (size_t)blockIdx.z * a.dstride + (size_t)y * a.dpitch + x0) = v;
    }
}

__device__ __forceinline__ LumaCoef luma_coef(const BayerArgs& a, bool red_row)
{
    const uint32_t cx = red_row ? a.cr : a.cb, cy = red_row ? a.cb : a.cr;
    return LumaCoef{cx, a.cg, cy, cx << 16, a.cg << 16, cy << 16, 1u << (a.shift - 1), a.shift};
}

template <bool WRITE>
__global__ __launch_bounds__(256) void bayer_gray_scan_kernel(BayerArgs a, BrightArgs b)
{
    constexpr int ND = 4, PX = 16, WAVE_PX = 62 * PX;
    const int lane = threadIdx.x;
    const int cy = __builtin_amdgcn_readfirstlane(blockIdx.y * 4 + threadIdx.y);
    if (8 * cy >= a.H) return;
    const int image = blockIdx.z;
    const int x0 = blockIdx.x * WAVE_PX - PX + PX * lane;
    const bool in = x0 >= 0 && x0 < a.W;
    const uint32_t off = in ? (uint32_t)x0 : 0u;
    const uint8_t* __restrict__ src = a.src + (size_t)image * a.sstride;
    uint8_t* __restrict__ dst = a.dst + (size_t)image * a.dstride;

    const bool red0 = a.ry == 0, red1 = a.ry == 1;
    const bool eic0 = (red0 ? a.rx : 1 - a.rx) == 0, eic1 = (red1 ? a.rx : 1 - a.rx) == 0;
    const LumaCoef k0 = luma_coef(a, red0), k1 = luma_coef(a, red1);

    auto load_row = [&](int r) {
        r = r < 0 ? 0 : (r > a.H - 1 ? a.H - 1 : r);
        uint4 v = *(const uint4*)(src + (size_t)r * a.spitch + off);
        if (!in) v = make_uint4(0u, 0u, 0u, 0u);
        return v;
    };
    auto pairs_of = [&](uint4 v) {
        uint32_t w[ND];
        __builtin_memcpy(w, &v, sizeof(v));
        return row_pairs<ND, true, true>(w);
    };
    uint4 raw[10];
#pragma unroll
    for (int r = 0; r < 10; r++) raw[r] = load_row(8 * cy - 1 + r);

    RowPairs<ND> U = pairs_of(raw[0]), C = pairs_of(raw[1]);
    uint32_t acc0 = 0, acc1 = 0;
    const bool writer = in && lane >= 1 && lane <= 62;
#pragma unroll
    for (int j = 0; j < 8; j++) {
        const int y = 8 * cy + j;
        const RowPairs<ND> D = pairs_of(raw[j + 2]);
        if (y != 0 && y != a.H - 1) {
            const bool eic = (j & 1) ? eic1 : eic0;
            const LumaCoef& k = (j & 1) ? k1 : k0;
            uint32_t g[PX];
            if (eic) {
#pragma unroll
                for (int i = 0; i < ND; i++) {
                    luma2(C.e[i], mean4(C.Le[i], C.o[i], U.e[i], D.e[i]), mean4(U.Le[i], U.o[i], D.Le[i], D.o[i]), k, g[4 * i], g[4 * i + 2]);
                    luma2(mean2(C.e[i], C.Ro[i]), C.o[i], mean2(U.o[i], D.o[i]), k, g[4 * i + 1], g[4 * i + 3]);
                }
            } else {
#pragma unroll
                for (int i = 0; i < ND; i++) {
                    luma2(mean2(C.Le[i], C.o[i]), C.e[i], mean2(U.e[i], D.e[i]), k, g[4 * i], g[4 * i + 2]);
                    luma2(C.o[i], mean4(C.e[i], C.Ro[i], U.o[i], D.o[i]), mean4(U.e[i], U.Ro[i], D.e[i], D.Ro[i]), k, g[4 * i + 1], g[4 * i + 3]);
                }
            }
            if (x0 == 0) g[0] = g[1];
            if (x0 + PX == a.W) g[PX - 1] = g[PX - 2];
            uint4 out;
            out.x = g[0] | (g[1] << 8) | (g[2] << 16) | (g[3] << 24);
            out.y = g[4] | (g[5] << 8) | (g[6] << 16) | (g[7] << 24);
            out.z = g[8] | (g[9] << 8) | (g[10] << 16) | (g[11] << 24);
            out.w = g[12] | (g[13] << 8) | (g[14] << 16) | (g[15] << 24);
            const bool twice = y == 1 || y == a.H - 2;
            if (WRITE && writer) {
                *(uint4*)(dst + (size_t)y * a.dpitch + x0) = out;
                if (y == 1) *(uint4*)(dst + x0) = out;
                if (y == a.H - 2) *(uint4*)(dst + (size_t)(a.H - 1) * a.dpitch + x0) = out;
            }
            const uint32_t base4 = (uint32_t)b.base * 0x01010101u, c8 = 8u * (uint32_t)b.base;
            const uint32_t e0 = excess2_row(out.x, out.y, base4, c8), e1 = excess2_row(out.z, out.w, base4, c8);
            acc0 += twice ? 2u * e0 : e0;
            acc1 += twice ? 2u * e1 : e1;
        }
        U = C; C = D;
    }
    if (writer) {
        const int ncx = a.W >> 3, n = ncx * (a.H >> 3);
        const int slot = image % b.cam_mod;
        const uint2* __restrict__ reach = b.reach + (size_t)slot * n;
        const uint8_t* __restrict__ cflags = b.cflags + (size_t)slot * n;
        uint32_t* __restrict__ rows = b.tile_rows + (size_t)image * b.n_chunks * b.n_strips * 4;
        const int ci = cy * ncx + (x0 >> 3);
        mark_hot_cell(b, reach, cflags, rows, ci, acc0);
        mark_hot_cell(b, reach, cflags, rows, ci + 1, acc1);
    }
}

__global__ __launch_bounds__(256) void bayer_gray_any_kernel(BayerArgs a)
{
    const int x = blockIdx.x * 64 + threadIdx.x, y = blockIdx.y * 4 + threadIdx.y;
    if (x >= a.W || y >= a.H) return;
    const int yc = y < 1 ? 1 : (y > a.H - 2 ? a.H - 2 : y), xc = x < 1 ? 1 : (x > a.W - 2 ? a.W - 2 : x);
    const uint8_t* __restrict__ p = a.src + (size_t)blockIdx.z * a.sstride + (size_t)yc * a.spitch + xc;
    const long sp = a.spitch;
    a.dst[(size_t)blockIdx.z * a.dstride + (size_t)y * a.dpitch + x] =
        (uint8_t)site_gray(p[0], p[-1], p[1], p[-sp], p[sp], p[-sp - 1], p[-sp + 1], p[sp - 1], p[sp + 1], (yc & 1) == a.ry,
                           (xc & 1) == a.rx, a);
}

void launch_bayer_gray(const BayerArgs& a, hipStream_t s)
{
    auto aligned = [&](int n) {
        return a.W % n == 0 && a.spitch % n == 0 && a.dpitch % n == 0 && a.sstride % n == 0 && a.dstride % n == 0 &&
               (uintptr_t)a.src % n == 0 && (uintptr_t)a.dst % n == 0;
    };
    if (aligned(16))
        hipLaunchKernelGGL(bayer_gray_kernel<4>, dim3((a.W + 62 * 16 - 1) / (62 * 16), (a.H + 3) / 4, a.n_images), dim3(64, 4), 0, s, a);
    else if (aligned(8))
        hipLaunchKernelGGL(bayer_gray_kernel<2>, dim3((a.W + 62 * 8 - 1) / (62 * 8), (a.H + 3) / 4, a.n_images), dim3(64, 4), 0, s, a);
    else
        hipLaunchKernelGGL(bayer_gray_any_kernel, dim3((a.W + 63) / 64, (a.H + 3) / 4, a.n_images), dim3(64, 4), 0, s, a);
}

bool bayer_scan_direct(const BayerArgs& a)
{
    return a.W % 16 == 0 && a.H % 8 == 0 && a.H >= 8 && a.spitch % 16 == 0 && a.sstride % 16 == 0 && (uintptr_t)a.src % 16 == 0;
}

bool bayer_scan_fusable(const BayerArgs& a)
{
    return bayer_scan_direct(a) && a.dpitch % 16 == 0 && a.dstride % 16 == 0 && (uintptr_t)a.dst % 16 == 0;
}

void launch_bayer_gray_scan(const BayerArgs& a, const BrightArgs& b, hipStream_t s)
{
    const dim3 grid((a.W + 62 * 16 - 1) / (62 * 16), (a.H / 8 + 3) / 4, a.n_images);
    if (a.dst) hipLaunchKernelGGL(bayer_gray_scan_kernel<true>, grid, dim3(64, 4), 0, s, a, b);
    else hipLaunchKernelGGL(bayer_gray_scan_kernel<false>, grid, dim3(64, 4), 0, s, a, b);
}

}
```

mocapv2_amd/csrc/blob_boxes.hip:

```cpp
#include <hip/hip_runtime.h>
#include <stdint.h>
#include <type_traits>
#include "kernels.h"
#include "bayer.h"

namespace mocap {

namespace {

__device__ __forceinline__ uint32_t from_prev(uint32_t v)
{
    return (uint32_t)__builtin_amdgcn_update_dpp(0, (int)v, 0x138 , 0xf, 0xf, true);
}
__device__ __forceinline__ uint32_t from_next(uint32_t v)
{
    return (uint32_t)__builtin_amdgcn_update_dpp(0, (int)v, 0x130 , 0xf, 0xf, true);
}
__device__ __forceinline__ uint32_t dot4(uint32_t a, uint32_t sel, uint32_t acc) { return __builtin_amdgcn_udot4(a, sel, acc, false); }
__device__ __forceinline__ int uni(int v) { return __builtin_amdgcn_readfirstlane(v); }
__device__ __forceinline__ int imin(int a, int b) { return a < b ? a : b; }
__device__ __forceinline__ int imax(int a, int b) { return a > b ? a : b; }
__device__ __forceinline__ int taps5(int v, int n)
{
    int lo = v - 2 < 0 ? 0 : v - 2, hi = v + 2 > n - 1 ? n - 1 : v + 2;
    return hi - lo + 1;
}
__device__ __forceinline__ int small_div(int n, float rcp_d) { return (int)(((float)n + 0.5f) * rcp_d); }

struct BayerK { int ry, rx; uint32_t cb, cg, cr; int shift; };

struct BayerWin { uint32_t w[9]; };
__device__ __forceinline__ void bayer_win_load(BayerWin& b, const uint8_t* __restrict__ img, int pitch, int W, int H, int x, int y)
{
    const int yc = y < 1 ? 1 : (y > H - 2 ? H - 2 : y);
    const uint32_t xl = (uint32_t)imax(x - 4, 0), xr = (uint32_t)imin(x + 4, W - 4);
#pragma unroll
    for (int r = 0; r < 3; r++) {
        const uint32_t o = (uint32_t)(yc - 1 + r) * (uint32_t)pitch;
        b.w[3 * r] = *(const uint32_t*)(img + o + xl);
        b.w[3 * r + 1] = *(const uint32_t*)(img + o + (uint32_t)x);
        b.w[3 * r + 2] = *(const uint32_t*)(img + o + xr);
    }
}
__device__ __forceinline__ uint32_t bayer_gray4(const BayerWin& b, int W, int H, int x, int y, const BayerK& k)
{
    const int yc = y < 1 ? 1 : (y > H - 2 ? H - 2 : y);
    const bool red_row = (yc & 1) == k.ry;
    const bool eic = (red_row ? k.rx : 1 - k.rx) == 0;
    uint32_t Pc[3], Lc[3], Rc[3], Pg[3];
    uint32_t Lg = 0, Rg = 0;
#pragma unroll
    for (int r = 0; r < 3; r++) {
        const uint32_t pw = b.w[3 * r], w = b.w[3 * r + 1], nw = b.w[3 * r + 2];
        const uint32_t e = prm(0, w, 0x0c020c00u), o = prm(0, w, 0x0c030c01u);
        const uint32_t Le = prm(pw, w, 0x0c010c07u), Ro = prm(nw, w, 0x0c040c02u);
        Pc[r] = eic ? e : o; Lc[r] = eic ? Le : e; Rc[r] = eic ? o : Ro; Pg[r] = eic ? o : e;
        if (r == 1) { Lg = eic ? e : Le; Rg = eic ? Ro : o; }
    }
    const uint32_t cx = red_row ? k.cr : k.cb, cy = red_row ? k.cb : k.cr;
    const LumaCoef kc{cx, k.cg, cy, cx << 16, k.cg << 16, cy << 16, 1u << (k.shift - 1), k.shift};
    uint32_t ca, cb, ga, gb;
    luma2(Pc[1], mean4(Lc[1], Rc[1], Pc[0], Pc[2]), mean4(Lc[0], Rc[0], Lc[2], Rc[2]), kc, ca, cb);
    luma2(mean2(Lg, Rg), Pg[1], mean2(Pg[0], Pg[2]), kc, ga, gb);
    uint32_t g0 = eic ? ca : ga, g1 = eic ? ga : ca, g2 = eic ? cb : gb, g3 = eic ? gb : cb;
    if (x == 0) g0 = g1;
    if (x + 3 == W - 1) g3 = g2;
    return g0 | (g1 << 8) | (g2 << 16) | (g3 << 24);
}
__device__ __forceinline__ uint32_t bayer_gray1(const uint8_t* __restrict__ img, int pitch, int W, int H, int x, int y, const BayerK& k)
{
    const int yc = y < 1 ? 1 : (y > H - 2 ? H - 2 : y), xc = x < 1 ? 1 : (x > W - 2 ? W - 2 : x);
    const uint32_t c = (uint32_t)yc * (uint32_t)pitch + (uint32_t)xc, u = c - (uint32_t)pitch, d = c + (uint32_t)pitch;
    return site_gray(img[c], img[c - 1], img[c + 1], img[u], img[d], img[u - 1], img[u + 1], img[d - 1], img[d + 1], (yc & 1) == k.ry,
                     (xc & 1) == k.rx, k);
}

}

__global__ void srcbox_kernel(const uint32_t* __restrict__ map4, ushort4* __restrict__ srcbox, int H, int W)
{
    const int ncx = (W + 7) >> 3, ncy = (H + 7) >> 3;
    const int c = blockIdx.x * blockDim.x + threadIdx.x;
    if (c >= ncx * ncy) return;
    const int cy = c / ncx, cx = c - cy * ncx;
    int x0 = 0x7fff, x1 = -0x8000, y0 = 0x7fff, y1 = -0x8000;
    for (int y = 8 * cy; y < 8 * cy + 8 && y < H; y++)
        for (int x = 8 * cx; x < 8 * cx + 8 && x < W; x++) {
            const uint32_t w = map4[(size_t)y * W + x];
            const int sx = x + ((int)(w << 21) >> 21), sy = y + ((int)(w << 10) >> 21);
            x0 = imin(x0, sx); x1 = imax(x1, sx + 1); y0 = imin(y0, sy); y1 = imax(y1, sy + 1);
        }
    srcbox[c] = make_ushort4((unsigned short)(x0 + 2), (unsigned short)(x1 + 2), (unsigned short)(y0 + 2), (unsigned short)(y1 + 2));
}

void launch_srcbox(const uint32_t* map4, ushort4* srcbox, int H, int W, hipStream_t s)
{
    const int n = ((W + 7) >> 3) * ((H + 7) >> 3);
    hipLaunchKernelGGL(srcbox_kernel, dim3((n + 63) / 64), dim3(64), 0, s, map4, srcbox, H, W);
}

__device__ __forceinline__ void choose_split(int nb, int h, int& nx, int& ny)
{
    int best = 0x7fffffff;
    nx = 1; ny = 1;
    for (int cx = 1; cx <= 4; cx++) {
        const int pb = (nb + cx - 1) / cx, Q = 2 * pb + 2;
        if (Q > 64) continue;
        const int rpw = 64 / Q, mr = BOX_HCAP / Q - 8;
        if (mr < 1) continue;
        const int cy = (h + mr - 1) / mr;
        if (cx * cy > BOX_MAX_PARTS) continue;
        const int ph = (h + cy - 1) / cy;
        const int cost = cx * cy * ((ph + 8 + rpw - 1) / rpw + 8);
        if (cost < best) { best = cost; nx = cx; ny = cy; }
    }
}

__global__ __launch_bounds__(256) void settle_tiles_kernel(BoxArgs a)
{
    const int lane = threadIdx.x & 63;
    if (a.zero8 && blockIdx.x == 0 && threadIdx.x < 8) a.zero8[threadIdx.x] = 0u;
    const int tiles = a.n_chunks * a.n_strips;
    const int n_all = a.n_clear > a.n_images ? a.n_clear : a.n_images;
    const int steps_all = (n_all + a.cam_mod - 1) / a.cam_mod;
    const long long total = (long long)tiles * a.cam_mod * steps_all;
    const long long i = (long long)blockIdx.x * 256 + threadIdx.x;
    int image = 0, chunk = 0, strip = 0;
    bool valid = i < total;
    if (valid) {
        const int t = (int)(i % steps_all);
        const long long rest = i / steps_all;
        const int slot = (int)(rest % a.cam_mod), tile = (int)(rest / a.cam_mod);
        image = t * a.cam_mod + slot;
        chunk = tile / a.n_strips; strip = tile - chunk * a.n_strips;
        valid = chunk * a.rows_per_chunk < a.H;
    }
    const size_t idx = ((size_t)image * a.n_chunks + chunk) * a.n_strips + strip;
    if (valid && !a.dense && image < n_all) {
        const uint4 nxt = *(const uint4*)(a.tile_rows_next + 4 * idx);
        if (nxt.x <= nxt.y) *(uint4*)(a.tile_rows_next + 4 * idx) = make_uint4(0xffffffffu, 0u, 0xffffffffu, 0u);
    }
    valid = valid && image < a.n_images;
    const int tile_r0 = chunk * a.rows_per_chunk, tile_r1 = imin(tile_r0 + a.rows_per_chunk, a.H) - 1;
    const int tile_x0 = 240 * strip, tile_x1 = imin(tile_x0 + 239, a.W - 1);
    int bx0 = 0, bx1 = a.W - 1, by0 = 0, by1 = a.H - 1;
    bool marked = valid;
    uint4 raw = make_uint4(0xffffffffu, 0u, 0xffffffffu, 0u);
    if (valid && !a.dense) {
        raw = *(const uint4*)(a.tile_rows + 4 * idx);
        marked = raw.x <= raw.y;
        if (marked) { by0 = (int)raw.x; by1 = (int)raw.y; bx0 = (int)raw.z; bx1 = (int)raw.w; }
    }
    int ox0 = imax(bx0, tile_x0) & ~7, ox1 = imin(imin(bx1, tile_x1) | 7, tile_x1);
    int oy0 = imax(by0, tile_r0), oy1 = imin(by1, tile_r1);
    if (marked && (ox0 > ox1 || oy0 > oy1)) marked = false;
    if (!marked) { ox0 = 1; ox1 = 0; oy0 = 1; oy1 = 0; }
    int nx = 0, ny = 0, nb = 0, h = 0;
    bool wide = false;
    int ix0 = ox0, ix1 = ox1, iy0 = oy0, iy1 = oy1;
    int ux0 = bx0, ux1 = bx1, uy0 = by0, uy1 = by1;
    bool emits = marked;
    if (marked && !a.dense && a.cluster) {
        const int c0 = chunk & ~1, s0 = strip & ~1;
        int n_marked = 0, first = -1, X0 = 0x7fffffff, X1 = -1, Y0 = 0x7fffffff, Y1 = -1;
        for (int k = 0; k < 4; k++) {
            const int cy = c0 + (k >> 1), sx = s0 + (k & 1);
            if (cy >= a.n_chunks || sx >= a.n_strips || cy * a.rows_per_chunk >= a.H) continue;
            const uint4 o = *(const uint4*)(a.tile_rows + 4 * (((size_t)image * a.n_chunks + cy) * a.n_strips + sx));
            if (o.x > o.y) continue;
            if (first < 0) first = k;
            n_marked++;
            Y0 = imin(Y0, (int)o.x); Y1 = imax(Y1, (int)o.y); X0 = imin(X0, (int)o.z); X1 = imax(X1, (int)o.w);
        }
        if (n_marked >= 2) {
            const int bx_lo = 240 * s0, bx_hi = imin(240 * (s0 + 2) - 1, a.W - 1), by_lo = c0 * a.rows_per_chunk, by_hi = imin((c0 + 2) * a.rows_per_chunk, a.H) - 1;
            const int ex0 = imax(X0, bx_lo) & ~7, ex1 = imin(X1 | 7, bx_hi), ey0 = imax(Y0, by_lo), ey1 = imin(Y1, by_hi);
            if (((ex1 - ex0 + 8) >> 3) <= 13 && ey1 - ey0 + 1 <= 100) {
                emits = first == ((chunk - c0) * 2 + (strip - s0));
                ix0 = ex0; ix1 = ex1; iy0 = ey0; iy1 = ey1;
                ux0 = X0; ux1 = X1; uy0 = Y0; uy1 = Y1;
            }
        }
    }
    if (marked) {
        nb = (ix1 - ix0 + 8) >> 3; h = iy1 - iy0 + 1;
        choose_split(nb, h, nx, ny);
        const int slot_ = image % a.cam_mod;
        const int limit = ((a.remap_bits >> slot_) & 1ull) ? a.wide_quads_remap : a.wide_quads_identity;
        wide = emits && ix0 == ox0 && ix1 == ox1 && iy0 == oy0 && iy1 == oy1 && a.wide_tiles != nullptr && 2 * nb + 2 * nx >= limit;
        if (wide) { ox0 = tile_x0; ox1 = tile_x1; ix0 = ox0; ix1 = ox1; }
    }
    const uint32_t nout_x = (uint32_t)ox0 | ((uint32_t)ox1 << 16), nout_y = (uint32_t)oy0 | ((uint32_t)oy1 << 16);

    bool need_clear = false;
    uint32_t pout_x = 1u, pout_y = 1u;
    if (valid) {
        uint4* cb = (uint4*)(a.cur_box + 4 * idx);
        if (!a.ext_mask) {
            const uint4 prev = *cb;
            pout_x = prev.x; pout_y = prev.y;
            const int px0 = (int)(prev.x & 0xffffu), px1 = (int)(prev.x >> 16), py0 = (int)(prev.y & 0xffffu), py1 = (int)(prev.y >> 16);
            if (px0 <= px1) need_clear = !(marked && ox0 <= px0 && px1 <= ox1 && oy0 <= py0 && py1 <= oy1);
            if (prev.x != nout_x || prev.y != nout_y || marked)
                *cb = make_uint4(nout_x, nout_y, (uint32_t)bx0 | ((uint32_t)bx1 << 16), (uint32_t)by0 | ((uint32_t)by1 << 16));
            if (a.cells[idx] != 0u) a.cells[idx] = 0u;
        } else {
            *cb = make_uint4(nout_x, nout_y, (uint32_t)bx0 | ((uint32_t)bx1 << 16), (uint32_t)by0 | ((uint32_t)by1 << 16));
            a.cells[idx] = 0u;
        }
    }
    for (uint64_t todo = __ballot(need_clear); todo; todo &= todo - 1) {
        const int src = __ffsll((long long)todo) - 1;
        const uint32_t cx = (uint32_t)__builtin_amdgcn_readlane((int)pout_x, src), cy = (uint32_t)__builtin_amdgcn_readlane((int)pout_y, src);
        const int cimage = __builtin_amdgcn_readlane(image, src);
        const int x0 = (int)(cx & 0xffffu), x1 = (int)(cx >> 16), y0 = (int)(cy & 0xffffu), y1 = (int)(cy >> 16);
        uint8_t* m = (uint8_t*)(a.mask + (size_t)cimage * mask_image_words(a.H, a.words_per_row));
        const int b0 = x0 >> 3, nr = y1 - y0 + 1, n = nr * ((x1 >> 3) - b0 + 1);
        for (int i = lane; i < n; i += 64) {
            const int bc = i / nr;
            m[mask_byte_index(y0 + (i - bc * nr), b0 + bc, a.words_per_row)] = 0;
        }
    }

    if (uint64_t wb = __ballot(wide)) {
        const int nbands = a.wide_bands;
        uint32_t base_w = 0;
        if (lane == 0) base_w = atomicAdd(a.n_items + 8, (uint32_t)(__popcll(wb) * nbands));
        base_w = (uint32_t)__builtin_amdgcn_readfirstlane((int)base_w);
        const uint32_t ow = base_w + (uint32_t)(__popcll(wb & ((1ull << lane) - 1ull)) * nbands);
        if (wide) {
            const int hb = (oy1 - oy0 + nbands) / nbands;
            for (int b = 0; b < nbands; b++) {
                const int y0 = oy0 + b * hb, y1 = imin(y0 + hb - 1, oy1);
                if (ow + b < a.cap_wide)
                    a.wide_tiles[ow + b] = make_uint4((uint32_t)image, (uint32_t)(chunk * a.n_strips + strip), (uint32_t)y0, (uint32_t)(y0 <= y1 ? y1 : y0 - 1));
            }
        }
    }
    const int cnt = (wide || !emits) ? 0 : nx * ny;
    int incl = cnt;
#pragma unroll
    for (int d = 1; d < 64; d <<= 1) {
        const int o = __shfl_up(incl, d);
        if (lane >= d) incl += o;
    }
    const int wave_total = __builtin_amdgcn_readlane(incl, 63);
    if (wave_total == 0) return;
    uint32_t base = 0;
    if (lane == 0) base = atomicAdd(a.n_items, (uint32_t)wave_total);
    base = (uint32_t)__builtin_amdgcn_readfirstlane((int)base);
    uint32_t o = base + (uint32_t)(incl - cnt);
    if (cnt) {
        const int pb = (nb + nx - 1) / nx, ph = (h + ny - 1) / ny;
        for (int jy = 0; jy < ny; jy++)
            for (int jx = 0; jx < nx; jx++, o++) {
                const int x0 = ix0 + 8 * pb * jx, x1 = imin(x0 + 8 * pb - 1, ix1);
                const int y0 = iy0 + ph * jy, y1 = imin(y0 + ph - 1, iy1);
                if (o >= a.cap_items) continue;
                uint4 it;
                it.x = (uint32_t)image;
                it.y = (uint32_t)(chunk * a.n_strips + strip);
                it.z = (uint32_t)x0 | ((uint32_t)x1 << 16);
                it.w = (uint32_t)y0 | ((uint32_t)y1 << 16);
                if (x0 > x1 || y0 > y1) it.z = 1u;
                ((uint4*)a.items)[2 * o] = it;
                ((uint4*)a.items)[2 * o + 1] = make_uint4((uint32_t)ux0 | ((uint32_t)ux1 << 16), (uint32_t)uy0 | ((uint32_t)uy1 << 16), 0u, 0u);
            }
    }
}

#ifndef MOCAP_BOX_GROUP
#define MOCAP_BOX_GROUP 3
#endif
#ifndef MOCAP_BOX_SU
#define MOCAP_BOX_SU 7
#endif
#ifndef MOCAP_BOX_WAVES
#define MOCAP_BOX_WAVES 4
#endif
constexpr int BOX_GROUP = MOCAP_BOX_GROUP;

struct BoxGeom {
    int image, tile, slot, remap;
    int ox0, ox1, oy0, oy1, Q, px0, ty0, ty1, hy0, hy1, PR, ey0, ey1, eq0, eq1;
    bool valid, exact;
};
__device__ __forceinline__ BoxGeom box_geometry(int H, int W, int cam_mod, uint64_t remap_bits, uint4 h0, uint4 h1)
{
    BoxGeom g;
    g.image = uni((int)h0.x); g.tile = uni((int)h0.y);
    g.ox0 = uni((int)(h0.z & 0xffffu)); g.ox1 = uni((int)(h0.z >> 16)); g.oy0 = uni((int)(h0.w & 0xffffu)); g.oy1 = uni((int)(h0.w >> 16));
    const int bx0 = uni((int)(h1.x & 0xffffu)), bx1 = uni((int)(h1.x >> 16)), by0 = uni((int)(h1.y & 0xffffu)), by1 = uni((int)(h1.y >> 16));
    g.valid = g.ox0 <= g.ox1 && g.oy0 <= g.oy1;
    g.slot = g.image % cam_mod;
    g.remap = (int)((remap_bits >> g.slot) & 1ull);
    const int nb = (g.ox1 - g.ox0 + 8) >> 3;
    g.Q = 2 * nb + 2; g.px0 = g.ox0 - 4;
    g.ty0 = imax(g.oy0 - 2, 0); g.ty1 = imin(g.oy1 + 2, H - 1);
    g.hy0 = g.ty0 - 2; g.hy1 = g.ty1 + 2; g.PR = g.hy1 - g.hy0 + 1;
    g.ey0 = imax(imax(by0, g.hy0), 0); g.ey1 = imin(imin(by1, g.hy1), H - 1);
    g.eq0 = imax((imax(bx0, 0) - g.px0) >> 2, 0); g.eq1 = imin((imin(bx1, W - 1) - g.px0) >> 2, g.Q - 1);
    g.exact = g.valid && g.ey0 <= g.ey1 && g.eq0 <= g.eq1;
    return g;
}
struct SrcBounds { int xa, xb, ya, yb; };
__device__ __forceinline__ SrcBounds source_bounds_partial(const ushort4* __restrict__ srcbox, int H, int W, const BoxGeom& g, int lane)
{
    SrcBounds b{0x7fff, -0x8000, 0x7fff, -0x8000};
    if (!g.exact || !g.remap) return b;
    const int ncx8 = (W + 7) >> 3;
    const ushort4* __restrict__ sbx = srcbox + (size_t)g.slot * ncx8 * ((H + 7) >> 3);
    const int cx0 = imax(g.px0 + 4 * g.eq0, 0) >> 3, cx1 = imin(g.px0 + 4 * g.eq1 + 3, W - 1) >> 3, cy0 = g.ey0 >> 3, cy1 = g.ey1 >> 3;
    const int ncw = cx1 - cx0 + 1, ncells = ncw * (cy1 - cy0 + 1);
    const float rcpw = __builtin_amdgcn_rcpf((float)ncw);
    for (int c0 = 0; c0 < ncells; c0 += 64) {
        const int c = imin(c0 + lane, ncells - 1);
        const int cyi = small_div(c, rcpw), cxi = c - cyi * ncw;
        const ushort4 sb = sbx[(cy0 + cyi) * ncx8 + cx0 + cxi];
        b.xa = imin(b.xa, (int)sb.x - 2); b.xb = imax(b.xb, (int)sb.y - 2); b.ya = imin(b.ya, (int)sb.z - 2); b.yb = imax(b.yb, (int)sb.w - 2);
    }
    return b;
}

constexpr size_t BOX_LDS_BYTES = 1024 + (size_t)(BOX_HCAP + 64) * 8 + BOX_SCAP;
template <bool BAYER>
__global__ __attribute__((amdgpu_waves_per_eu(MOCAP_BOX_WAVES, MOCAP_BOX_WAVES))) __launch_bounds__(64) void box_filter_kernel(BoxArgs a)
{
    extern __shared__ __attribute__((aligned(16))) uint8_t box_lds[];
    uint32_t* const lut = (uint32_t*)box_lds;
    uint2* const Hs = (uint2*)(box_lds + 1024);
    uint8_t* const Sbuf = box_lds + 1024 + (size_t)(BOX_HCAP + 64) * 8;
    uint32_t* const Cs = (uint32_t*)Sbuf;
    static_assert((BOX_HCAP + 64) * 4 <= BOX_SCAP, "counts alias the source buffer");

    const int lane = threadIdx.x;
    const uint8_t* __restrict__ const a_src = a.src;
    const size_t a_image_stride = a.image_stride;
    const int a_pitch = a.pitch, a_stage_bytes = a.stage_bytes, a_thr_mul = a.thr_mul, a_words_per_row = a.words_per_row;
    const int a_n_chunks = a.n_chunks, a_n_strips = a.n_strips, a_rows_per_chunk = a.rows_per_chunk;
    const uint32_t* __restrict__ const a_map4 = a.map4;
    uint32_t* __restrict__ const a_mask = a.mask;
    uint32_t* __restrict__ const a_cells = a.cells;
    const uint32_t a_cap_items = a.cap_items;
    const uint32_t* const a_n_items = a.n_items;
    uint64_t* const a_timing = a.timing;
    const BayerK bk{a.bayer.ry, a.bayer.rx, a.bayer.cb, a.bayer.cg, a.bayer.cr, a.bayer.shift};
    if (a.prio) __builtin_amdgcn_s_setprio(2);
#pragma unroll
    for (int e = 0; e < 4; e++) {
        uint32_t i = (uint32_t)(lane + 64 * e), v = 0;
#pragma unroll
        for (int k = 0; k < 4; k++) v |= (uint32_t)__popc((i >> k) & 0x1fu) << (8 * k);
        lut[i] = v;
    }
    uint32_t n_items = *a_n_items;
    n_items = n_items < a_cap_items ? n_items : a_cap_items;
    uint32_t* const heads = a.n_items + 16;
    int shard = blockIdx.x & 7, tries = 0;
    auto take = [&]() __attribute__((always_inline)) -> uint32_t {
        for (;;) {
            const uint32_t lo = (uint32_t)(((uint64_t)n_items * (uint32_t)shard) >> 3), hi = (uint32_t)(((uint64_t)n_items * (uint32_t)(shard + 1)) >> 3);
            uint32_t i = 0;
            if (lane == 0) i = atomicAdd(heads + 16 * shard, 1u);
            i = (uint32_t)__builtin_amdgcn_readfirstlane((int)i);
            if (i < hi - lo) return lo + i;
            if (++tries >= 8) return 0xffffffffu;
            shard = (shard + 1) & 7;
        }
    };
    const int H = a.H, W = a.W, Hm1 = H - 1;
    const int row_bytes = a_words_per_row * 4;
    const int cam_mod = a.cam_mod;
    const uint64_t remap_bits = a.remap_bits;
    const ushort4* __restrict__ srcbox = a.srcbox;
    const uint4* __restrict__ items = (const uint4*)a.items;
    auto take_request = [&]() __attribute__((always_inline)) -> uint32_t {
        uint32_t i = 0;
        if (lane == 0 && tries < 8) i = atomicAdd(heads + 16 * shard, 1u);
        return i;
    };
    auto take_resolve = [&](uint32_t i) __attribute__((always_inline)) -> uint32_t {
        if (tries >= 8) return 0xffffffffu;
        const uint32_t lo = (uint32_t)(((uint64_t)n_items * (uint32_t)shard) >> 3), hi = (uint32_t)(((uint64_t)n_items * (uint32_t)(shard + 1)) >> 3);
        i = (uint32_t)__builtin_amdgcn_readfirstlane((int)i);
        if (i < hi - lo) return lo + i;
        if (++tries >= 8) return 0xffffffffu;
        shard = (shard + 1) & 7;
        return take();
    };
    uint32_t item = take();
    if (item == 0xffffffffu) return;
    uint32_t nitem = take();

    uint64_t tacc[6] = {0, 0, 0, 0, 0, 0}, tlast = a.timing ? __builtin_readcyclecounter() : 0;
    auto tick = [&](int i) __attribute__((always_inline)) { if (a_timing) { const uint64_t now = __builtin_readcyclecounter(); tacc[i] += now - tlast; tlast = now; } };
    uint4 h0 = items[2 * item], h1 = items[2 * item + 1];
    BoxGeom g = box_geometry(H, W, cam_mod, remap_bits, h0, h1);
    SrcBounds sbp = source_bounds_partial(srcbox, H, W, g, lane);

    while (item != 0xffffffffu) {
        const uint32_t nxt = nitem != 0xffffffffu ? nitem : item;
        const uint4 n0 = items[2 * nxt], n1 = items[2 * nxt + 1];
        const uint32_t nn_raw = take_request();
        if (!g.valid) {
            g = box_geometry(H, W, cam_mod, remap_bits, n0, n1);
            sbp = source_bounds_partial(srcbox, H, W, g, lane);
            item = nitem;
            nitem = take_resolve(nn_raw);
            continue;
        }
        const int image = g.image, slot = g.slot;
        const int ox0 = g.ox0, oy0 = g.oy0, oy1 = g.oy1, Q = g.Q, px0 = g.px0, ty0 = g.ty0, ty1 = g.ty1, hy0 = g.hy0, PR = g.PR;
        const int ey0 = g.ey0, ey1 = g.ey1, eq0 = g.eq0, eq1 = g.eq1;
        const float rcpQ = __builtin_amdgcn_rcpf((float)Q);
        const int rpw = small_div(64, rcpQ);
        const int rsub = small_div(lane, rcpQ), q = lane - rsub * Q;
        const bool lane_on = rsub < rpw;
        const int x = px0 + 4 * q;
        uint32_t bytemask = 0, colmask = 0;
#pragma unroll
// ... 384 lines not shown
```

mocapv2_amd/csrc/blob_filter.hip:

```cpp
#include <hip/hip_runtime.h>
#include <stdint.h>
#include <type_traits>
#include "kernels.h"
#include "scan_mark.h"

namespace mocap {

__device__ __forceinline__ uint32_t lane_from_prev(uint32_t v)
{
    return (uint32_t)__builtin_amdgcn_update_dpp(0, (int)v, 0x138 , 0xf, 0xf, true);
}
__device__ __forceinline__ uint32_t lane_from_next(uint32_t v)
{
    return (uint32_t)__builtin_amdgcn_update_dpp(0, (int)v, 0x130 , 0xf, 0xf, true);
}
__device__ __forceinline__ uint32_t dot4(uint32_t a, uint32_t sel, uint32_t acc)
{
    return __builtin_amdgcn_udot4(a, sel, acc, false);
}

__device__ __forceinline__ uint32_t load_u32(const uint8_t* p)
{
    uint32_t v;
    __builtin_memcpy(&v, p, 4);
// ... 33 lines not shown
    int sh = (xl - ax) * 8;
    c.shift = sh < 0 ? 0u : (sh > 24 ? 24u : (uint32_t)sh);
    c.bytemask = 0;
#pragma unroll
    for (int k = 0; k < 4; k++)
        if ((unsigned)(xl + k) < (unsigned)W) c.bytemask |= 0xffu << (8 * k);
    c.interior = xl >= 0 && xl + 3 < W;
    return c;
}

template <bool REMAP, bool TINY>
__device__ __forceinline__ uint32_t fetch_src4(const FilterArgs& a, const uint8_t* __restrict__ img,
                                               const uint32_t* __restrict__ map, int y, int xl, const LaneCols& lc)
{
    const int yc = y < 0 ? 0 : (y > a.H - 1 ? a.H - 1 : y);
    if (REMAP) {
        if ((unsigned)y >= (unsigned)a.H) return 0u;
        uint32_t out = 0;
        const uint32_t* mrow = map + (size_t)yc * a.W;
        const uint32_t* wrow = a.mapw + (map - a.map) + (size_t)yc * a.W;
#pragma unroll
        for (int k = 0; k < 4; k++) {
            int x = xl + k;
            if ((unsigned)x < (unsigned)a.W) out |= remap_px(img, a.pitch, mrow[x], wrow[x], x, yc) << (8 * k);
        }
        return out;
    } else {
        if (!TINY) return load_u32(img + ((uint32_t)yc * (uint32_t)a.pitch + (uint32_t)lc.addr_x));
        const uint8_t* p = img + (size_t)yc * a.pitch;
        uint32_t v = 0;
#pragma unroll
        for (int k = 0; k < 4; k++)
            if ((unsigned)(xl + k) < (unsigned)a.W) v |= (uint32_t)p[xl + k] << (8 * k);
        return v;
    }
}

template <bool REMAP, bool TINY>
__device__ __forceinline__ uint32_t finish_src4(uint32_t raw, bool row_ok, const LaneCols& lc)
{
    if (REMAP) return raw;
    uint32_t v = TINY ? raw : ((raw >> lc.shift) & lc.bytemask);
    return row_ok ? v : 0u;
}

struct MapSlot { uint4 m; };
struct TapSlot { uint32_t t0[4], t1[4], w[4]; };

__device__ __forceinline__ void remap_issue_map(MapSlot& ms, const uint32_t* __restrict__ map, int row, int H, int W,
                                                const LaneCols& lc)
{
    int rc = row < 0 ? 0 : (row > H - 1 ? H - 1 : row);
    __builtin_memcpy(&ms.m, map + ((uint32_t)rc * (uint32_t)W + (uint32_t)lc.addr_x), 16);
}

__device__ __forceinline__ void remap_issue_taps(TapSlot& ts, const MapSlot& ms, const uint8_t* __restrict__ img,
                                                 const uint32_t* __restrict__ mapw, int pitch, int H, int W, int row,
                                                 const int xq[4], const LaneCols& lc)
{
    row = row < 0 ? 0 : (row > H - 1 ? H - 1 : row);
    const uint32_t mm[4] = {ms.m.x, ms.m.y, ms.m.z, ms.m.w};
    uint4 wv4;
    __builtin_memcpy(&wv4, mapw + ((uint32_t)row * (uint32_t)W + (uint32_t)lc.addr_x), 16);
    ts.w[0] = wv4.x; ts.w[1] = wv4.y; ts.w[2] = wv4.z; ts.w[3] = wv4.w;
#pragma unroll
    for (int k = 0; k < 4; k++) {
        uint32_t m = mm[k];
        int sx = xq[k] + (int)(int16_t)(m & 0xffffu), sy = row + ((int)m >> 16);
        uint32_t off0 = __umul24((uint32_t)sy, (uint32_t)pitch) + (uint32_t)sx, off1 = off0 + (uint32_t)pitch;
        ts.t0[k] = load_u16(img + off0);
        ts.t1[k] = load_u16(img + off1);
    }
}

__device__ __forceinline__ uint32_t remap_combine(const TapSlot& ts, const LaneCols& lc)
{
    uint32_t out = 0;
#pragma unroll
    for (int k = 0; k < 4; k++) {
        uint32_t w = ts.w[k];
        uint32_t top = dot4(ts.t0[k], w, 0u), bot = dot4(ts.t1[k], w, 0u);
        uint32_t r = __umul24(top, w >> 24) + 512u;
        r += __umul24(bot, (w >> 16) & 0xffu);
        out |= (r >> 10) << (8 * k);
    }
    return out & lc.bytemask;
}

__device__ __forceinline__ uint4 load_once16(const uint8_t* p)
{
    typedef unsigned int u32x4 __attribute__((ext_vector_type(4)));
    const u32x4 q = __builtin_nontemporal_load((const u32x4*)p);
    return make_uint4(q.x, q.y, q.z, q.w);
}

template <bool WIDE, bool FULL, bool MAP>
__device__ __forceinline__ void bright_cells_block(const BrightArgs& a, const int bx, const int image)
{
    const int ncx = (a.W + 7) >> 3, ncy = (a.H + 7) >> 3, n = ncx * ncy;
    const uint8_t* __restrict__ img = a.src + (size_t)image * a.image_stride;
    uint2 v[2][8];
    int ci[2], cr[2];
    uint32_t sh[2];
    bool in_range[2];
    if (WIDE) {
        const int half = ncx >> 1, np = half * ncy;
        int p = bx * 256 + threadIdx.x;
        in_range[0] = in_range[1] = p < np;
        p = p < np ? p : np - 1;
        const int row = (int)__umulhi((uint32_t)p, a.ncx_magic), cxp = p - row * half;
        cr[0] = cr[1] = row;
        ci[0] = row * ncx + 2 * cxp; ci[1] = ci[0] + 1;
        sh[0] = sh[1] = 0;
        if (FULL) {
            const uint32_t off0 = (uint32_t)(8 * row) * (uint32_t)a.pitch + 16u * (uint32_t)cxp;
#pragma unroll
            for (int j = 0; j < 8; j++) {
                const uint4 q = load_once16(img + (off0 + (uint32_t)(j * a.pitch)));
                v[0][j] = make_uint2(q.x, q.y); v[1][j] = make_uint2(q.z, q.w);
            }
        } else {
#pragma unroll
            for (int j = 0; j < 8; j++) {
                int r = 8 * row + j;
                r = r < a.H ? r : a.H - 1;
                const uint4 q = load_once16(img + ((uint32_t)r * (uint32_t)a.pitch + 16u * (uint32_t)cxp));
                v[0][j] = make_uint2(q.x, q.y); v[1][j] = make_uint2(q.z, q.w);
            }
        }
    } else {
        const int i0 = bx * 512 + threadIdx.x;
#pragma unroll
        for (int u = 0; u < 2; u++) {
            int i = i0 + 256 * u;
            in_range[u] = i < n;
            i = i < n ? i : n - 1;
            ci[u] = i;
            cr[u] = a.ncx_magic ? (int)__umulhi((uint32_t)i, a.ncx_magic) : i / ncx;
            const int cx = i - cr[u] * ncx;
            const int c = 8 * cx, cc = c < a.W - 8 ? c : a.W - 8;
            sh[u] = (uint32_t)(8 * (c - cc));
#pragma unroll
            for (int j = 0; j < 8; j++) {
                int r = 8 * cr[u] + j;
                r = r < a.H ? r : a.H - 1;
                __builtin_memcpy(&v[u][j], img + ((uint32_t)r * (uint32_t)a.pitch + (uint32_t)cc), 8);
            }
        }
    }
    const int slot = image % a.cam_mod;
    const uint2* __restrict__ reach = a.reach + (size_t)slot * n;
    const uint8_t* __restrict__ cflags = a.cflags + (size_t)slot * n;
    uint32_t* __restrict__ rows = a.tile_rows + (size_t)image * a.n_chunks * a.n_strips * 4;
    const uint32_t base4 = (uint32_t)a.base * 0x01010101u, c8 = 8u * (uint32_t)a.base;
    uint32_t level[2] = {0u, 0u};
#pragma unroll
    for (int u = 0; u < 2; u++) {
        uint32_t acc = 0;
#pragma unroll
        for (int j = 0; j < 8; j++) {
            if (WIDE) {
                const uint32_t e2 = excess2_row(v[u][j].x, v[u][j].y, base4, c8);
                if (FULL || 8 * cr[u] + j < a.H) acc += e2;
            } else {
                uint64_t vv = (((uint64_t)v[u][j].y << 32) | v[u][j].x) >> sh[u];
                const uint32_t e2 = excess2_row((uint32_t)vv, (uint32_t)(vv >> 32), base4, c8);
                if (8 * cr[u] + j < a.H) acc += e2;
            }
        }
        if (MAP) level[u] = in_range[u] ? hot_level(a, acc) : 0u;
        else mark_hot_cell(a, reach, cflags, rows, ci[u], acc);
        if (a.probe && (image & 15) == 0) {
            const uint32_t alt4 = (uint32_t)a.base_alt * 0x01010101u, alt8 = 8u * (uint32_t)a.base_alt;
            uint32_t acc2 = 0;
#pragma unroll
            for (int j = 0; j < 8; j++) {
                const uint64_t vv = WIDE ? (((uint64_t)v[u][j].y << 32) | v[u][j].x) : ((((uint64_t)v[u][j].y << 32) | v[u][j].x) >> sh[u]);
                const uint32_t e2 = excess2_row((uint32_t)vv, (uint32_t)(vv >> 32), alt4, alt8);
                if (FULL || 8 * cr[u] + j < a.H) acc2 += e2;
            }
            const int n_cur = __popcll(__ballot((int)acc > a.hot)), n_alt = __popcll(__ballot((int)acc2 > a.hot_alt));
            if ((threadIdx.x & 63) == 0) {
                atomicAdd(&a.probe[PROBE_STRIDE * (bx & 127)], (uint32_t)n_cur);
                atomicAdd(&a.probe[PROBE_STRIDE * (bx & 127) + 1], (uint32_t)n_alt);
            }
        }
    }
    if (MAP) {
        const int lane = threadIdx.x & 63;
        uint32_t* __restrict__ hm = a.hotmap + (size_t)image * a.hot_words;
        if (WIDE) {
            uint32_t w = (level[0] | (level[1] << 2)) << (4 * (lane & 7));
            w |= (uint32_t)__builtin_amdgcn_update_dpp(0, (int)w, 0xB1 , 0xf, 0xf, true);
            w |= (uint32_t)__builtin_amdgcn_update_dpp(0, (int)w, 0x4E , 0xf, 0xf, true);
            w |= (uint32_t)__builtin_amdgcn_update_dpp(0, (int)w, 0x141 , 0xf, 0xf, true);
            if ((lane & 7) == 0 && w != 0u) hm[(bx * 256 + (int)threadIdx.x) >> 3] = w;
        } else {
#pragma unroll
            for (int u = 0; u < 2; u++) {
                uint32_t w = level[u] << (2 * (lane & 15));
                w |= (uint32_t)__builtin_amdgcn_update_dpp(0, (int)w, 0xB1, 0xf, 0xf, true);
                w |= (uint32_t)__builtin_amdgcn_update_dpp(0, (int)w, 0x4E, 0xf, 0xf, true);
                w |= (uint32_t)__builtin_amdgcn_update_dpp(0, (int)w, 0x141, 0xf, 0xf, true);
                w |= (uint32_t)__builtin_amdgcn_update_dpp(0, (int)w, 0x140 , 0xf, 0xf, true);
                if ((lane & 15) == 0 && w != 0u) hm[(bx * 512 + (int)threadIdx.x + 256 * u) >> 4] = w;
            }
        }
    }
}

__global__ __launch_bounds__(256) void mark_tiles_kernel(BrightArgs a)
{
    __shared__ uint16_t s_list[4][1024];
    __shared__ uint32_t s_tab[4][32][5];
    const int lane = threadIdx.x & 63, wv = threadIdx.x >> 6;
    const int wpi = (a.hot_words + 255) >> 8;
    const int n_cells = ((a.W + 7) >> 3) * ((a.H + 7) >> 3);
    for (long long piece = (long long)blockIdx.x * 4 + wv; piece < (long long)wpi * a.n_images; piece += (long long)gridDim.x * 4) {
    const int image = (int)(piece / wpi), wave_word0 = (int)(piece - (long long)image * wpi) * 256;
    uint32_t* __restrict__ hm = a.hotmap + (size_t)image * a.hot_words;
    uint32_t wk[4];
#pragma unroll
    for (int k = 0; k < 4; k++) {
        const int wi = wave_word0 + 64 * k + lane;
        wk[k] = wi < a.hot_words ? hm[wi] : 0u;
    }
    if (__ballot((wk[0] | wk[1] | wk[2] | wk[3]) != 0u) == 0ull) continue;
#pragma unroll
    for (int k = 0; k < 4; k++)
        if (wk[k] != 0u) hm[wave_word0 + 64 * k + lane] = 0u;
    uint32_t (*tab)[5] = s_tab[wv];
    if (lane < 32) { tab[lane][0] = 0xffffffffu; tab[lane][1] = 0xffffffffu; tab[lane][2] = 0u; tab[lane][3] = 0xffffffffu; tab[lane][4] = 0u; }
    const int slot = image % a.cam_mod;
    const uint2* __restrict__ reach = a.reach + (size_t)slot * n_cells;
    const uint8_t* __restrict__ cflags = a.cflags + (size_t)slot * n_cells;
    uint32_t* __restrict__ rows = a.tile_rows + (size_t)image * a.n_chunks * a.n_strips * 4;
    auto widen = [&](int t, uint32_t ya, uint32_t yb, uint32_t xa, uint32_t xb) __attribute__((always_inline)) {
        const uint4 cur = *(const uint4*)(rows + 4 * t);
        if (cur.x <= ya && cur.y >= yb && cur.z <= xa && cur.w >= xb) return;
        atomicMin(&rows[4 * t], ya);
        atomicMax(&rows[4 * t + 1], yb);
        atomicMin(&rows[4 * t + 2], xa);
        atomicMax(&rows[4 * t + 3], xb);
    };
#pragma unroll 1
    for (int k = 0; k < 4; k++) {
        const uint32_t w = k == 0 ? wk[0] : (k == 1 ? wk[1] : (k == 2 ? wk[2] : wk[3]));
        const uint32_t nz = (w | (w >> 1)) & 0x55555555u;
        const int cnt = __popc(nz);
        if (__ballot(cnt != 0) == 0ull) continue;
        const int word0 = wave_word0 + 64 * k;
        int incl = cnt;
#pragma unroll
        for (int d = 1; d < 64; d <<= 1) {
            const int o = __shfl_up(incl, d);
            if (lane >= d) incl += o;
        }
        const int total = __builtin_amdgcn_readlane(incl, 63);
        int at = incl - cnt;
        for (uint32_t m = nz; m; m &= m - 1) {
            const int j2 = __ffs((int)m) - 1;
            s_list[wv][at++] = (uint16_t)((lane << 6) | (j2 << 1) | ((w >> j2) & 3u));
        }
        __builtin_amdgcn_s_waitcnt(0xc07f);
        __builtin_amdgcn_wave_barrier();
        for (int e0 = 0; e0 < total; e0 += 64) {
            const int e = e0 + lane;
            if (e < total) {
                const uint32_t v = s_list[wv][e];
                const int ci = 16 * (word0 + (int)(v >> 6)) + (int)((v >> 2) & 15u);
                if (ci < n_cells) {
                    const uint2 rc = reach[ci];
                    const int x0 = (int)(rc.x & 0xffffu), x1 = (int)(rc.x >> 16), y0 = (int)(rc.y & 0xffffu), y1 = (int)(rc.y >> 16);
                    if (x0 <= x1 && level_is_hot(v & 3u, cflags[ci])) {
                        const int xa = x0 - 4 > 0 ? x0 - 4 : 0, xb = x1 + 4 < a.W - 1 ? x1 + 4 : a.W - 1;
                        const int ya = y0 - 4 > 0 ? y0 - 4 : 0, yb = y1 + 4 < a.H - 1 ? y1 + 4 : a.H - 1;
                        const int ch0 = (int)(((uint32_t)ya * a.rows_magic) >> 23), ch1 = (int)(((uint32_t)yb * a.rows_magic) >> 23);
                        const int st0 = (int)(((uint32_t)xa * 34953u) >> 23), st1 = (int)(((uint32_t)xb * 34953u) >> 23);
                        for (int ch = ch0; ch <= ch1; ch++)
                            for (int st = st0; st <= st1; st++) {
                                const int t = ch * a.n_strips + st, q = t & 31;
                                const uint32_t old = atomicCAS(&tab[q][0], 0xffffffffu, (uint32_t)t);
                                if (old == 0xffffffffu || old == (uint32_t)t) {
                                    atomicMin(&tab[q][1], (uint32_t)ya); atomicMax(&tab[q][2], (uint32_t)yb);
                                    atomicMin(&tab[q][3], (uint32_t)xa); atomicMax(&tab[q][4], (uint32_t)xb);
                                } else
                                    widen(t, (uint32_t)ya, (uint32_t)yb, (uint32_t)xa, (uint32_t)xb);
                            }
                    }
                }
            }
        }
        __builtin_amdgcn_s_waitcnt(0xc07f);
        __builtin_amdgcn_wave_barrier();
    }
    if (lane < 32 && tab[lane][0] != 0xffffffffu) widen((int)tab[lane][0], tab[lane][1], tab[lane][2], tab[lane][3], tab[lane][4]);
    __builtin_amdgcn_s_waitcnt(0xc07f);
    __builtin_amdgcn_wave_barrier();
    }
}

template <bool WIDE, bool FULL = false, bool MAP = true>
__global__ __launch_bounds__(256) void bright_cells_kernel(BrightArgs a)
{
    if (a.prio == 1) __builtin_amdgcn_s_setprio(1);
    else if (a.prio == 2) __builtin_amdgcn_s_setprio(2);
    else if (a.prio == 3) __builtin_amdgcn_s_setprio(3);
    const uint32_t total = (uint32_t)a.blocks_x * (uint32_t)a.slice_images;
    if (a.zero_counters && blockIdx.x == 0) a.zero_counters[threadIdx.x] = 0u;
    if (a.block_ctr == nullptr) {
        for (uint32_t vb = blockIdx.x; vb < total; vb += gridDim.x) {
            const uint32_t image = vb / (uint32_t)a.blocks_x;
            bright_cells_block<WIDE, FULL, MAP>(a, (int)(vb - image * (uint32_t)a.blocks_x), a.image0 + (int)image);
        }
    } else {
        __shared__ uint32_t s_next[2];
        constexpr uint32_t CH = 16;
        uint32_t v0 = blockIdx.x * CH;
        for (int it = 0; v0 < total; it++) {
            if (threadIdx.x == 0) s_next[it & 1] = gridDim.x * CH + atomicAdd(a.block_ctr, CH);
            for (uint32_t vb = v0; vb < v0 + CH && vb < total; vb++) {
                const uint32_t image = vb / (uint32_t)a.blocks_x;
                bright_cells_block<WIDE, FULL, MAP>(a, (int)(vb - image * (uint32_t)a.blocks_x), a.image0 + (int)image);
            }
            __syncthreads();
            v0 = s_next[it & 1];
        }
    }
    if (a.mask_words) {
        const size_t nthreads = (size_t)gridDim.x * 256;
        const size_t g = (size_t)blockIdx.x * 256 + threadIdx.x;
        if (a.mask_aligned16) {
            const size_t quads = a.mask_words >> 2;
            for (size_t q = g; q < quads; q += nthreads) ((uint4*)a.mask)[q] = make_uint4(0u, 0u, 0u, 0u);
            if (g < (a.mask_words & 3)) a.mask[(quads << 2) + g] = 0u;
        } else {
            for (size_t q = g; q < a.mask_words; q += nthreads) a.mask[q] = 0u;
        }
    }
}

__device__ __forceinline__ int taps5(int v, int n)
{
    int lo = v - 2 < 0 ? 0 : v - 2, hi = v + 2 > n - 1 ? n - 1 : v + 2;
    return hi - lo + 1;
}

template <int J> struct IC { static constexpr int value = J; };


struct TileId { int slot, cgroup, image; bool valid; };
__device__ __forceinline__ TileId decode_tile(const FilterArgs& a, int b)
{
    TileId t;
    const int groups = a.cam_mod * a.n_cgroups;
    const int grp = b / a.n_steps, tstep = b - grp * a.n_steps;
    t.slot = grp % a.cam_mod;
    t.cgroup = grp / a.cam_mod;
    t.image = tstep * a.cam_mod + t.slot;
    t.valid = grp < groups && t.image < a.n_images;
    return t;
}

#ifndef MOCAP_ROWS_WAVES
#define MOCAP_ROWS_WAVES 1
#endif
template <bool REMAP, bool TINY, bool PIPE, bool LIST>
__global__ __attribute__((amdgpu_waves_per_eu(MOCAP_ROWS_WAVES))) __launch_bounds__(256) void filter_mask_kernel(FilterArgs a)
{
    __shared__ uint32_t lut[256];
    __shared__ uint2 hring[4][8][64];
    __shared__ uint32_t cring[4][8][64];

    const int lane = threadIdx.x & 63;
    const int wv = __builtin_amdgcn_readfirstlane(threadIdx.x >> 6);

    int slot = 0, image = 0, chunk = 0;
    uint32_t n_list = 0;
    if (LIST) {
        n_list = *a.n_tiles;
        n_list = n_list < a.cap_tiles ? n_list : a.cap_tiles;
        if ((uint32_t)(blockIdx.x * 4 + wv) >= n_list) return;
    } else {
        const TileId tid_ = decode_tile(a, blockIdx.x);
        if (!tid_.valid) return;
        slot = tid_.slot; image = tid_.image;
        chunk = tid_.cgroup * 4 + wv;
        if (chunk * a.rows_per_chunk >= a.H) return;
    }
#pragma unroll
    for (int e = 0; e < 4; e++) {
        uint32_t i = (uint32_t)(lane + 64 * e), v = 0;
#pragma unroll
        for (int k = 0; k < 4; k++) v |= (uint32_t)__popc((i >> k) & 0x1fu) << (8 * k);
        lut[i] = v;
    }
    const uint32_t it_first = LIST ? (uint32_t)(blockIdx.x * 4 + wv) : 0u, it_end = LIST ? n_list : (uint32_t)a.n_strips;
    const uint32_t it_step = LIST ? gridDim.x * 4u : 1u;
    for (uint32_t it = it_first; it < it_end; it += it_step) {
        int strip = (int)it, r0e = 0, r1e = 0x7fffffff;
        if (LIST) {
            const uint4 e = a.tiles[it];
            image = __builtin_amdgcn_readfirstlane((int)e.x);
            const int tile = __builtin_amdgcn_readfirstlane((int)e.y);
            r0e = __builtin_amdgcn_readfirstlane((int)e.z); r1e = __builtin_amdgcn_readfirstlane((int)e.w) + 1;
            chunk = tile / a.n_strips; strip = tile - chunk * a.n_strips;
            slot = image % a.cam_mod;
        }
        const int tile_r0 = chunk * a.rows_per_chunk;
        const int tile_r1 = tile_r0 + a.rows_per_chunk < a.H ? tile_r0 + a.rows_per_chunk : a.H;
        const size_t cell_index = ((size_t)image * a.n_cgroups * 4 + chunk) * a.n_strips + strip;
        const int r0 = r0e > tile_r0 ? r0e : tile_r0, r1 = r1e < tile_r1 ? r1e : tile_r1;
        if (LIST && r0 >= r1) continue;
        const int xbase = strip * 240 - 8;

        const int Hm1 = a.H - 1;
        int kfirst = r0 - 2;
        kfirst = kfirst < 0 ? 0 : (kfirst > Hm1 ? Hm1 : kfirst);
        const int ks = r0 - 1 > 1 ? r0 - 1 : 1;
        const int ke = r1 + 1 < Hm1 ? r1 + 1 : Hm1;

    #pragma unroll
        for (int s = 0; s < 8; s++) {
            hring[wv][s][lane] = make_uint2(0u, 0u);
            cring[wv][s][lane] = 0u;
        }

        const uint8_t* __restrict__ img = a.src + (size_t)image * a.image_stride;
        const uint32_t* __restrict__ map = REMAP ? a.map + (size_t)slot * a.H * a.W : nullptr;
        const uint32_t* __restrict__ mapw = REMAP ? a.mapw + (size_t)slot * a.H * a.W : nullptr;
        uint8_t* __restrict__ mrow_base = (uint8_t*)(a.mask + (size_t)image * mask_image_words(a.H, a.words_per_row));
        const int row_bytes = a.words_per_row * 4;
        const int wpr = a.words_per_row;

        const int xl = xbase + 4 * lane;

        uint32_t cx01, cx23, colmask = 0;
        {
            int c0 = taps5(xl, a.W), c1 = taps5(xl + 1, a.W), c2 = taps5(xl + 2, a.W), c3 = taps5(xl + 3, a.W);
            cx01 = (uint32_t)(c0 & 0xffff) | ((uint32_t)c1 << 16);
            cx23 = (uint32_t)(c2 & 0xffff) | ((uint32_t)c3 << 16);
    #pragma unroll
            for (int k = 0; k < 4; k++)
                if ((unsigned)(xl + k) < (unsigned)a.W) colmask |= 1u << k;
        }
        const LaneCols lc = lane_cols(xl, a.W);
        const bool left_edge = xbase < 0;
        const bool right_edge = xbase + 255 >= a.W;
        const int lane_r = (a.W - 1 - xbase) >> 2, bit_r = (a.W - 1 - xbase) & 3;
// ... 865 lines not shown
```

mocapv2_amd/csrc/kernels.h:

```cpp
#pragma once
#include <hip/hip_runtime.h>
#include <stdint.h>

namespace mocap {

__host__ __device__ __forceinline__ uint32_t mask_word_index(int y, int k, int wpr)
{
    return ((uint32_t)(y >> 5) * (uint32_t)wpr + (uint32_t)k) * 32u + (uint32_t)(y & 31);
}
__host__ __device__ __forceinline__ uint32_t mask_byte_index(int y, int b, int wpr)
{
    return mask_word_index(y, b >> 2, wpr) * 4u + (uint32_t)(b & 3);
}
__host__ __device__ __forceinline__ size_t mask_image_words(int H, int wpr) { return (size_t)((H + 31) >> 5) * 32 * (size_t)wpr; }

__device__ __forceinline__ double wave_sum(double v)
{
#pragma unroll
    for (int o = 32; o > 0; o >>= 1) v += __shfl_down(v, o, 64);
    return v;
}
__device__ __forceinline__ double block_sum(double v, double* s_part )
{
    v = wave_sum(v);
    __syncthreads();
    if ((threadIdx.x & 63) == 0) s_part[threadIdx.x >> 6] = v;
    __syncthreads();
    return (s_part[0] + s_part[1]) + (s_part[2] + s_part[3]);
}

void launch_mask_convert(const uint32_t* src, uint32_t* dst, int n_images, int H, int wpr, bool to_blocked, hipStream_t s);

struct FilterArgs {
    const uint8_t* src;
    size_t image_stride;
    int pitch, H, W;
    uint32_t* mask;
    int words_per_row;
    uint32_t* cells;
    const uint32_t* map;
    const uint32_t* mapw;
    const uint4* tiles; const uint32_t* n_tiles; uint32_t cap_tiles;
    int pipelined;
    int cam_mod;
    int n_images, n_steps;
    int thr_mul;
    int rows_per_chunk, n_strips, n_cgroups;
    int staged = 0;
    const uint32_t* map4 = nullptr;
    const ushort4* rowbox = nullptr;
    int stage_dw = 0;
};
void launch_rowbox(const uint32_t* map4, ushort4* rowbox, int H, int W, int n_strips, hipStream_t s);
int rows_stage_dwords();

struct BayerArgs {
    const uint8_t* src; uint8_t* dst;
    int H, W, n_images;
    long spitch, dpitch;
    size_t sstride, dstride;
    int ry, rx;
    uint32_t cb, cg, cr;
    int shift;
};

#ifndef MOCAP_BOX_HCAP
#define MOCAP_BOX_HCAP 1536
#define MOCAP_BOX_SCAP 6656
#define MOCAP_BOX_MAX_PARTS 4
#endif
constexpr int BOX_HCAP = MOCAP_BOX_HCAP;
constexpr int BOX_SCAP = MOCAP_BOX_SCAP;
constexpr int BOX_MAX_PARTS = MOCAP_BOX_MAX_PARTS;
struct BoxItem { uint32_t image, tile, x01, y01, bx01, by01, pad0, pad1; };
struct BoxArgs {
    const uint8_t* src; size_t image_stride; int pitch, H, W;
    uint32_t* mask; int words_per_row;
    uint32_t* cells;
    const uint32_t* map4;
    const ushort4* srcbox;
    uint64_t remap_bits;
    int cam_mod, n_images, n_steps;
    int thr_mul;
    int rows_per_chunk, n_strips, n_chunks;
    uint32_t* tile_rows;
    uint32_t* tile_rows_next;
    int n_clear;
    int cluster;
    uint32_t* cur_box;
    BoxItem* items; uint32_t* n_items; uint32_t cap_items;
    uint64_t* timing;
    int prio;
    int stage_bytes;
    uint4* wide_tiles;
    uint32_t cap_wide; int wide_quads_remap, wide_quads_identity, wide_bands;
    uint32_t* zero8;
    int dense;
    int ext_mask;
    BayerArgs bayer;
};
void launch_settle_tiles(const BoxArgs& a, hipStream_t s);
void launch_box_filter(const BoxArgs& a, int grid, hipStream_t s, bool bayer = false);
int box_filter_blocks_per_cu();
void launch_srcbox(const uint32_t* map4, ushort4* srcbox, int H, int W, hipStream_t s);

struct MapArgs {
    double K[9], dist[5];
    int H, W;
    uint32_t* map;
    uint32_t* mapw;
    uint32_t* map4;
    uint32_t* flags;
};

struct ContourRec {
    int32_t key;
    int32_t is_hole;
    int32_t sx, sy;
    int32_t npts;
    int32_t steps;
    int64_t a00, a10, a01;
    double area, perimeter;
    int32_t kept, cx, cy;
    int32_t link;
    int32_t parent;
    int32_t order;
};

struct ContourArgs {
    const uint32_t* mask;
    int words_per_row, H, W, n_images;
    int32_t* out_xy;
    int32_t* out_count;
    long xy_stride, count_stride;
    int max_blobs;
    double min_area, min_circ;
    ContourRec* dbg;
    int32_t* dbg_count;
    int dbg_cap;
    int max_steps;
    const uint32_t* cells;
    const uint32_t* boxes;
    int rows_per_chunk, n_chunks, n_strips;
    uint64_t* timing;
    void* work;
    int prio;
    uint64_t* walk_list;
    uint64_t* link_list;
    uint32_t* walk_count;
    uint32_t* wait_list;
    int follow_grid;
    int follow_grid2;
    int counters_zeroed;
    int defer_links;
    int image_grid;
    int follow_list;
    int tree_pass;
    uint64_t* follow_dbg;
    int follow_dbg_list;
};

enum { BLOB_ERR_CANDIDATES = -2, BLOB_ERR_CONTOURS = -3, BLOB_ERR_STEPS = -4, BLOB_ERR_DEPTH = -5 };

void launch_filter_mask(const FilterArgs& a, bool remap, hipStream_t s);
void launch_filter_tiles(const FilterArgs& a, bool remap, int blocks, hipStream_t s);
constexpr int PROBE_STRIDE = 32;
struct BrightArgs {
    const uint8_t* src; size_t image_stride; int pitch, H, W, n_images;
    int cam_mod;
    uint32_t ncx_magic;
    int wide;
    int base;
    int hot, hot_edge, hot_corner;
    const uint2* reach;
    const uint8_t* cflags;
    uint32_t* tile_rows; int n_chunks, n_strips; uint32_t rows_magic;
    uint32_t* mask; size_t mask_words; int mask_aligned16;
    uint32_t* probe; int base_alt, hot_alt;
    int prio;
    int max_blocks;
    uint32_t* block_ctr;
    int blocks_x;
    int slices;
    int image0, slice_images;
    uint32_t* hotmap;
    int hot_words;
    uint32_t* zero_counters;
    int mark_grid;
};
int hot_map_words(int H, int W, int wide);
void launch_mark_tiles(const BrightArgs& a, hipStream_t s);
void launch_bright_cells(const BrightArgs& a, hipStream_t s);
struct StatArgs { const uint32_t* map; const uint32_t* mapw; uint32_t* acc; uint32_t* stats; int H, W; uint32_t* edge; int* reach; };
void launch_remap_stats(const StatArgs& a, hipStream_t s);
void launch_undistort_map(const MapArgs& m, hipStream_t s);
void launch_contours(const ContourArgs& a, hipStream_t s);
size_t contour_work_bytes();
size_t contour_walk_bytes();
size_t contour_link_bytes();
void launch_box_blur(const uint8_t* src, uint8_t* dst, int H, int W, int sp, int dp, int ksize, hipStream_t s);
void launch_undistort(const uint8_t* src, uint8_t* dst, int H, int W, int sp, int dp, const uint32_t* map, const uint32_t* mapw,
                      hipStream_t s);
void launch_mask_expand(const uint32_t* mask, int wpr, uint8_t* dst, int H, int W, int dp, hipStream_t s);
void launch_median5(const uint8_t* src, uint8_t* dst, int H, int W, int sp, int dp, int ithresh, int apply, hipStream_t s);
void launch_demosaic(const uint8_t* bayer, uint8_t* bgr, int H, int W, int sp, hipStream_t s);
void launch_bayer_gray(const BayerArgs& a, hipStream_t s);
bool bayer_scan_fusable(const BayerArgs& a);
bool bayer_scan_direct(const BayerArgs& a);
void launch_bayer_gray_scan(const BayerArgs& a, const BrightArgs& b, hipStream_t s);

struct CameraTable {
    double K[32][9], dist[32][5], R[32][9], t[32][3];
    double F[31][9];
    int n_cam, n_F;
};

struct CorrArgs {
    const CameraTable* cams;
    const void* pts;
    const int32_t* counts;
    long pt_st, pt_sc, cnt_st, cnt_sc;
    int pts_f64;
    int T, C, P;
    double cutoff;
    int max_groups;
    double* root_xyz;
    double* root_err;
    double* root_grp;
    int32_t* root_idx;
    int32_t* order;
    int32_t* n_roots;
    int prio;
    int threads;
    double* scratch;
    int step_budget;
    int lds_budget;
};

struct TriArgs {
    const CameraTable* cams;
    const double* pts;
    const uint8_t* valid;
    int N, C;
    int compact_k;
    double* xyz;
    int32_t* ok;
};

struct ReprojArgs {
    const CameraTable* cams;
    const double* pts;
    const uint8_t* valid;
    const double* xyz;
    int N, C, compact_k;
    double* mse;
    int32_t* ok;
};

struct EpiArgs {
    const CameraTable* cams;
    const void* roots;
    const void* cand;
    int n_roots, n_cand, pts_f64, f_index;
    double* dist;
    float* lines;
};

struct BaArgs {
    const CameraTable* cams;
    const double* params;
    const double* pts;
    const uint8_t* valid;
    int N, C, B;
    double* obj;
    float* res;
    int32_t* counts;
};

struct FundArgs {
    const double* pts_a;
    const double* pts_b;
    const int32_t* offset;
    const int32_t* samples;
    int n_pairs, H, max_n;
    double thr2;
    double* F_all;
    int32_t* counts;
    int32_t* pair_err;
    double* F_sample;
    double* F_refit;
    uint8_t* inlier;
    int32_t* status;
};

struct LmState {
    double lambda, nu;
    double cost, cost0;
    int32_t stop, status;
    int32_t iters, cur;
    int32_t chol_fail, chol_fail_prev, behind, trial_behind;
};

struct RigState : LmState {
    double t1_norm;
    int32_t layout_err, pad;
};
enum { RIG_LIN_COST = 0, RIG_PRED_CAM = 1, RIG_NORM2_CAM = 2, RIG_N_SCALARS = 4 };
enum { RIG_STOP_MAX_ITERS = 1, RIG_STOP_FTOL = 2, RIG_STOP_LAMBDA = 3, RIG_STOP_CHOLESKY = 4, RIG_ERR_LAYOUT = -2, RIG_ERR_BEHIND = -3 };

struct RigArgs {
    const CameraTable* cams;
    const int32_t* obs_offset;
    const int32_t* obs_cam;
    const double* obs_uv;
    int C, N, n_obs;
    int n_pairs, n_lin_blocks, n_chunks;
    double* poses_io;
    double* points_io;
    RigState* state;
    double* poses;
    double* points;
    uint32_t* mask;
    double* W;
    double* Vinv;
    double* vdiag;
    double* gp;
    double* lin_part;
    double* cost_part;
    double* schur_part;
    double* S;
    double* rhs;
    double* gc;
    double* udiag;
    double* chol;
    double* delta_c;
    double* upd_part;
    double* scalars;
    double* history;
    double* result;
};

// ... 63 lines not shown
```

mocapv2_amd/csrc/scan_mark.h:

```cpp
#pragma once
#include <hip/hip_runtime.h>
#include <stdint.h>
#include "kernels.h"

namespace mocap {

__device__ __forceinline__ uint32_t excess2_row(uint32_t lo, uint32_t hi, uint32_t base4, uint32_t c8)
{
    uint32_t s = __builtin_amdgcn_sad_u8(lo, base4, 0u);
    s = __builtin_amdgcn_sad_u8(lo, 0u, s);
    s = __builtin_amdgcn_sad_u8(hi, base4, s);
    s = __builtin_amdgcn_sad_u8(hi, 0u, s);
    return s - c8;
}

__device__ __forceinline__ void widen_tile_boxes(const BrightArgs& a, const uint2 rc, uint32_t* __restrict__ rows)
{
    const int x0 = (int)(rc.x & 0xffffu), x1 = (int)(rc.x >> 16), y0 = (int)(rc.y & 0xffffu), y1 = (int)(rc.y >> 16);
    if (x0 > x1) return;
    const int xa = x0 - 4 > 0 ? x0 - 4 : 0, xb = x1 + 4 < a.W - 1 ? x1 + 4 : a.W - 1;
    const int ya = y0 - 4 > 0 ? y0 - 4 : 0, yb = y1 + 4 < a.H - 1 ? y1 + 4 : a.H - 1;
    const int ch0 = (int)(((uint32_t)ya * a.rows_magic) >> 23), ch1 = (int)(((uint32_t)yb * a.rows_magic) >> 23);
    const int st0 = (int)(((uint32_t)xa * 34953u) >> 23), st1 = (int)(((uint32_t)xb * 34953u) >> 23);
    for (int ch = ch0; ch <= ch1; ch++)
        for (int st = st0; st <= st1; st++) {
            const int t = ch * a.n_strips + st;
            const uint4 cur = *(const uint4*)(rows + 4 * t);
            if (cur.x <= (uint32_t)ya && cur.y >= (uint32_t)yb && cur.z <= (uint32_t)xa && cur.w >= (uint32_t)xb) continue;
            atomicMin(&rows[4 * t], (uint32_t)ya);
            atomicMax(&rows[4 * t + 1], (uint32_t)yb);
            atomicMin(&rows[4 * t + 2], (uint32_t)xa);
            atomicMax(&rows[4 * t + 3], (uint32_t)xb);
        }
}

__device__ __forceinline__ void mark_hot_cell(const BrightArgs& a, const uint2* __restrict__ reach, const uint8_t* __restrict__ cflags,
                                              uint32_t* __restrict__ rows, int ci, uint32_t acc)
{
    if ((int)acc > a.hot_corner) {
        const uint2 rc = reach[ci];
        const uint32_t fl = cflags[ci];
        if ((int)acc > ((fl & 2u) ? a.hot_corner : (fl & 1u) ? a.hot_edge : a.hot)) widen_tile_boxes(a, rc, rows);
    }
}

__device__ __forceinline__ uint32_t hot_level(const BrightArgs& a, uint32_t acc)
{
    return (uint32_t)((int)acc > a.hot_corner) + (uint32_t)((int)acc > a.hot_edge) + (uint32_t)((int)acc > a.hot);
}
__device__ __forceinline__ bool level_is_hot(uint32_t level, uint32_t fl)
{
    return level >= ((fl & 2u) ? 1u : (fl & 1u) ? 2u : 3u);
}

}
```

mocapv2_amd/engine.py:

```python
import ctypes as C
import threading

import numpy as np
import torch

from . import _abi

MAX_BLOBS = 128
GRAY_SHIFT = 15
REC_INTS = 2 + 2 * MAX_BLOBS


def _ptr(t):
    return C.c_void_p(t.data_ptr()) if t is not None else None


def _stream():
    return C.c_void_p(torch.cuda.current_stream().cuda_stream)


def _dbl(a, n):
    a = np.ascontiguousarray(a, np.float64).reshape(-1)
    assert a.size == n, (a.size, n)
    return a, a.ctypes.data_as(C.POINTER(C.c_double))
# ... 319 lines not shown
            raise ValueError("every point needs 2..C observations")
        if cam.min() < 0 or cam.max() >= Cn:
            raise ValueError(f"obs_cam outside 0..{Cn - 1}")
        inner = np.ones(n_obs, bool)
        inner[off[:-1]] = False
        if (np.diff(cam, prepend=-1)[inner] <= 0).any():
            raise ValueError("a point's observations must come in strictly ascending camera order")
        if getattr(self, "n_cam", 0) < Cn:
            raise ValueError(f"set_cameras: {getattr(self, 'n_cam', 0)} cameras set, {Cn} needed (their K and dist are used)")
        if not (np.isfinite(uv).all() and np.isfinite(poses).all() and np.isfinite(points).all()):
            raise ValueError("observations, poses and points must be finite")
        dev = self.device
        return (Cn, N, n_obs, torch.from_numpy(off).to(dev), torch.from_numpy(cam).to(dev), torch.from_numpy(uv).to(dev),
                torch.from_numpy(poses).to(dev), torch.from_numpy(points).to(dev))

    def rig_linearize(self, obs_offset, obs_cam, obs_uv, poses, points, lam):
        Cn, N, n_obs, d_off, d_cam, d_uv, d_poses, d_pts = self._rig_upload(obs_offset, obs_cam, obs_uv, poses, points)
        D = 6 * (Cn - 1)
        dev = self.device
        cost = torch.zeros((1,), dtype=torch.float64, device=dev)
        grad = torch.zeros((D + 3 * N,), dtype=torch.float64, device=dev)
        S = torch.zeros((D, D), dtype=torch.float64, device=dev)
        rhs = torch.zeros((D,), dtype=torch.float64, device=dev)
        status = torch.zeros((2,), dtype=torch.int32, device=dev)
        _abi.check(self.lib.mocap_rig_linearize(self._h, Cn, N, n_obs, _ptr(d_off), _ptr(d_cam), _ptr(d_uv), _ptr(d_poses),
                                                _ptr(d_pts), float(lam), _ptr(cost), _ptr(grad), _ptr(S), _ptr(rhs), _ptr(status),
                                                _stream()))
        self.sync()
        status = status.cpu().numpy()
        if status[0]:
            raise _abi.MocapError(-2, "mocap_rig_linearize: the observation arrays break the layout rules (MOCAP_RIG_E_LAYOUT)")
        return {"cost": float(cost.cpu().numpy()[0]), "gradient": grad.cpu().numpy(), "S": S.cpu().numpy(), "rhs": rhs.cpu().numpy(),
                "behind": bool(status[1])}

    def rig_bundle_adjust(self, obs_offset, obs_cam, obs_uv, poses, points, max_iters=50, ftol=1e-12, lambda0=1e-3):
        Cn, N, n_obs, d_off, d_cam, d_uv, d_poses, d_pts = self._rig_upload(obs_offset, obs_cam, obs_uv, poses, points)
        max_iters = int(max_iters)
        hist = torch.empty((max_iters, 4), dtype=torch.float64, device=self.device)
        result = torch.zeros((4,), dtype=torch.float64, device=self.device)
        _abi.check(self.lib.mocap_rig_bundle_adjust(self._h, Cn, N, n_obs, _ptr(d_off), _ptr(d_cam), _ptr(d_uv), _ptr(d_poses),
                                                    _ptr(d_pts), max_iters, float(ftol), float(lambda0), _ptr(hist), _ptr(result),
                                                    _stream()))
        self.sync()
        result = result.cpu().numpy()
        status, iters = int(result[0]), int(result[1])
        if status <= 0:
            what = {-2: "the observation arrays break the layout rules (MOCAP_RIG_E_LAYOUT)",
                    -3: "in the start state a point is not in front of a camera that sees it, or the cost is not finite "
                        "(MOCAP_RIG_E_BEHIND)"}.get(status, f"status {status}")
            raise _abi.MocapError(status, "mocap_rig_bundle_adjust: " + what)
        return {"poses": d_poses.cpu().numpy(), "points": d_pts.cpu().numpy(), "status": status, "iterations": iters,
                "cost_initial": float(result[2]), "cost": float(result[3]), "history": hist.cpu().numpy()[:iters].copy()}

    def _intr_upload(self, view_offset, point_offset, obj_xy, img_uv):
        voff = np.ascontiguousarray(view_offset, np.int32).reshape(-1)
        poff = np.ascontiguousarray(point_offset, np.int32).reshape(-1)
        obj = np.ascontiguousarray(obj_xy, np.float64).reshape(-1, 2)
        img = np.ascontiguousarray(img_uv, np.float64).reshape(-1, 2)
        n_cams = len(voff) - 1
        if n_cams < 1 or voff[0] != 0 or (np.diff(voff) < 0).any():
            raise ValueError("view_offset must be [n_cams + 1], from 0, not descending")
        n_views = int(voff[-1])
        if n_views < 1 or len(poff) != n_views + 1 or poff[0] != 0 or (np.diff(poff) < 0).any():
            raise ValueError(f"point_offset must be [n_views + 1 = {n_views + 1}], from 0, not descending")
        if len(obj) != poff[-1] or len(img) != poff[-1] or len(obj) < 1:
            raise ValueError(f"obj_xy and img_uv must be [{poff[-1]}][2], got {obj.shape} and {img.shape}")
        if not (np.isfinite(obj).all() and np.isfinite(img).all()):
            raise ValueError("board points and pixels must be finite")
        dev = self.device
        return n_cams, n_views, voff, poff, torch.from_numpy(obj).to(dev), torch.from_numpy(img).to(dev)

    def intrinsics_linearize(self, view_offset, point_offset, obj_xy, img_uv, kd, view_poses, lam):
        n_cams, n_views, voff, poff, d_obj, d_img = self._intr_upload(view_offset, point_offset, obj_xy, img_uv)
        kd = np.ascontiguousarray(kd, np.float64).reshape(n_cams, 9)
        poses = np.ascontiguousarray(view_poses, np.float64).reshape(n_views, 12)
        dev = self.device
        d_kd, d_poses = torch.from_numpy(kd).to(dev), torch.from_numpy(poses).to(dev)
        cost = torch.zeros((n_cams,), dtype=torch.float64, device=dev)
        grad = torch.zeros((9 * n_cams + 6 * n_views,), dtype=torch.float64, device=dev)
        S = torch.zeros((n_cams, 9, 9), dtype=torch.float64, device=dev)
        rhs = torch.zeros((n_cams, 9), dtype=torch.float64, device=dev)
        status = torch.zeros((n_cams, 2), dtype=torch.int32, device=dev)
        ip = C.POINTER(C.c_int)
        _abi.check(self.lib.mocap_intrinsics_linearize(self._h, n_cams, voff.ctypes.data_as(ip), poff.ctypes.data_as(ip), _ptr(d_obj),
                                                       _ptr(d_img), _ptr(d_kd), _ptr(d_poses), float(lam), _ptr(cost), _ptr(grad), _ptr(S),
                                                       _ptr(rhs), _ptr(status), _stream()))
        self.sync()
        status = status.cpu().numpy()
        return {"cost": cost.cpu().numpy(), "gradient": grad.cpu().numpy(), "S": S.cpu().numpy(), "rhs": rhs.cpu().numpy(),
                "layout": status[:, 0].astype(bool), "behind": status[:, 1].astype(bool)}

    def intrinsics_calibrate(self, view_offset, point_offset, obj_xy, img_uv, image_sizes, start=None, max_iters=50, ftol=1e-12,
                             lambda0=1e-3):
        n_cams, n_views, voff, poff, d_obj, d_img = self._intr_upload(view_offset, point_offset, obj_xy, img_uv)
        size = np.ascontiguousarray(image_sizes, np.int32).reshape(n_cams, 2)
        if (size < 1).any():
            raise ValueError("image sizes must be positive")
        max_iters = int(max_iters)
        dev = self.device
        if start is None:
            d_kd = torch.full((n_cams, 9), float("nan"), dtype=torch.float64, device=dev)
            d_poses = torch.full((n_views, 12), float("nan"), dtype=torch.float64, device=dev)
        else:
            kd = np.ascontiguousarray(start[0], np.float64).reshape(n_cams, 9)
            poses = np.ascontiguousarray(start[1], np.float64).reshape(n_views, 12)
            if not (np.isfinite(kd).all() and np.isfinite(poses).all()):
                raise ValueError("the start must be finite")
            d_kd, d_poses = torch.from_numpy(kd).to(dev), torch.from_numpy(poses).to(dev)
        rms = torch.zeros((n_views,), dtype=torch.float64, device=dev)
        hist = torch.empty((n_cams, max_iters, 4), dtype=torch.float64, device=dev)
        result = torch.zeros((n_cams, 4), dtype=torch.float64, device=dev)
        ip = C.POINTER(C.c_int)
        _abi.check(self.lib.mocap_intrinsics_calibrate(self._h, n_cams, voff.ctypes.data_as(ip), poff.ctypes.data_as(ip), _ptr(d_obj),
                                                       _ptr(d_img), size.ctypes.data_as(ip), int(start is not None), max_iters,
                                                       float(ftol), float(lambda0), _ptr(d_kd), _ptr(d_poses), _ptr(rms), _ptr(hist),
                                                       _ptr(result), _stream()))
        self.sync()
        result, hist = result.cpu().numpy(), hist.cpu().numpy()
        iters = result[:, 1].astype(np.int64)
        return {"kd": d_kd.cpu().numpy(), "poses": d_poses.cpu().numpy(), "view_rms": rms.cpu().numpy(),
                "status": result[:, 0].astype(np.int64), "iterations": iters, "cost_initial": result[:, 2].copy(),
                "cost": result[:, 3].copy(), "history": [hist[c, :iters[c]].copy() for c in range(n_cams)]}

    def ba_problem(self, pts, valid=None):
        return BAProblem(self, pts, valid)

    def comm_init(self, unique_id, rank, world):
        buf = (C.c_char * _abi.COMM_ID_BYTES).from_buffer_copy(bytes(unique_id))
        _abi.check(self.lib.mocap_comm_init(self._h, C.cast(buf, C.c_void_p), int(rank), int(world)))
        self.comm_world = int(world)

    def comm_share(self, src):
        _abi.check(self.lib.mocap_comm_share(self._h, src._h))
        self.comm_world = src.comm_world

    def comm_destroy(self):
        _abi.check(self.lib.mocap_comm_destroy(self._h))
        self.comm_world = 1

    def allgather_centroids(self, local, out=None):
        assert local.is_cuda and local.is_contiguous() and local.dtype == torch.int32
        world = self.comm_world
        if out is None:
            out = torch.empty((world * local.shape[0],) + tuple(local.shape[1:]), dtype=torch.int32, device=local.device)
        assert out.is_contiguous() and out.numel() == world * local.numel() and out.dtype == torch.int32
        _abi.check(self.lib.mocap_allgather_centroids(self._h, _ptr(local), _ptr(out), local.numel(), _stream()))
        return out

    def tile_stats(self):
        a, b = C.c_uint64(0), C.c_uint64(0)
        _abi.check(self.lib.mocap_tile_stats(self._h, C.byref(a), C.byref(b)))
        return a.value, b.value

    def profile(self, on=True):
        _abi.check(self.lib.mocap_profile_enable(self._h, int(on)))

    def profile_read(self):
        ms = (C.c_double * 5)()
        n = (C.c_int * 5)()
        _abi.check(self.lib.mocap_profile_read(self._h, ms, n))
        return {"filter_ms": ms[0], "filter_launches": n[0], "contour_ms": ms[1], "contour_launches": n[1],
                "corr_ms": ms[2], "corr_launches": n[2], "scan_ms": ms[3], "scan_launches": n[3],
                "settle_ms": ms[4], "settle_launches": n[4]}


class BAProblem:

    def __init__(self, ctx, pts, valid=None):
        pts = np.ascontiguousarray(pts, np.float64)
        assert pts.ndim == 3 and pts.shape[2] == 2, pts.shape
        self.ctx, (self.N, self.C) = ctx, pts.shape[:2]
        valid = np.ones((self.N, self.C), np.uint8) if valid is None else np.ascontiguousarray(valid, np.uint8).reshape(self.N, self.C)
        self.d_pts = torch.from_numpy(pts).to(ctx.device)
        self.d_valid = torch.from_numpy(valid).to(ctx.device)
        self._res = np.empty((1, self.N), np.float32)
        self._cnt = np.empty(1, np.int32)

    def residuals(self, params):
        p = np.ascontiguousarray(params, np.float64)
        single = p.ndim == 1
        p = p.reshape(-1, 6 * (self.C - 1))
        B = p.shape[0]
        if self._res.shape[0] < B:
            self._res = np.empty((B, self.N), np.float32)
            self._cnt = np.empty(B, np.int32)
        ctx = self.ctx
        _abi.check(ctx.lib.mocap_ba_residuals(ctx._h, p.ctypes.data_as(C.POINTER(C.c_double)), B, _ptr(self.d_pts), _ptr(self.d_valid),
                                              self.N, self.C, self._res.ctypes.data_as(C.POINTER(C.c_float)),
                                              self._cnt.ctypes.data_as(C.POINTER(C.c_int)), _stream()))
        if single:
            return self._res[0, :self._cnt[0]].copy()
        return [self._res[b, :self._cnt[b]].copy() for b in range(B)]


def comm_available():
    _abi.check(_abi.load().mocap_comm_available())
    return True


def comm_unique_id():
    buf = (C.c_char * _abi.COMM_ID_BYTES)()
    _abi.check(_abi.load().mocap_comm_unique_id(C.cast(buf, C.c_void_p)))
    return bytes(buf)


_contexts = threading.local()


def default_context(width=1, height=1, n_slots=1, device=None):
    if device is None:
        device = torch.cuda.current_device() if torch.cuda.is_available() else 0
    key = (int(width), int(height), int(n_slots), int(device))
    cache = _contexts.__dict__.setdefault("cache", {})
    ctx = cache.get(key)
    if ctx is None:
        ctx = cache[key] = MocapContext(width, height, n_slots, device)
    return ctx
```

Measured before the change: 392,100 frames/s.

## Split wide tiles into column runs using per-tile column occupancy masks

Adds a per-tile 30-bit column-occupancy mask, kept alongside the existing row/column bounding boxes and set by the scan/mark kernels with atomicOr. When the settle kernel would promote a tile to the full-width 'wide' path, it now tries to cut the tile into a few disjoint column runs and emits box items only for those runs, with a default-on tuning knob to disable it. The intent is to avoid processing dark gaps between separated markers in the same tile. In exchange it adds extra atomics and memory traffic in the marking kernels, more shared-memory table state, and a new debug counter and work_stats API.

```diff
diff --git a/include/mocap_hip.h b/include/mocap_hip.h
--- a/include/mocap_hip.h
+++ b/include/mocap_hip.h
@@ -166,6 +166,7 @@
                                         long ints_per_rank, void* stream);
 
 MOCAP_API int mocap_tile_stats(mocap_ctx_t ctx, uint64_t* tiles, uint64_t* skipped);
+MOCAP_API int mocap_work_stats(mocap_ctx_t ctx, uint32_t out[3]);
 MOCAP_API int mocap_profile_enable(mocap_ctx_t ctx, int on);
 MOCAP_API int mocap_profile_read(mocap_ctx_t ctx, double ms[5], int launches[5]);
 
diff --git a/mocapv2_amd/_abi.py b/mocapv2_amd/_abi.py
--- a/mocapv2_amd/_abi.py
+++ b/mocapv2_amd/_abi.py
@@ -71,6 +71,7 @@
     "mocap_comm_destroy": [_vp],
     "mocap_allgather_centroids": [_vp, _vp, _vp, _l, _vp],
     "mocap_tile_stats": [_vp, C.POINTER(C.c_uint64), C.POINTER(C.c_uint64)],
+    "mocap_work_stats": [_vp, C.POINTER(C.c_uint32)],
     "mocap_profile_enable": [_vp, _i],
     "mocap_profile_read": [_vp, _dp, _ip],
 }
diff --git a/mocapv2_amd/csrc/abi.hip b/mocapv2_amd/csrc/abi.hip
--- a/mocapv2_amd/csrc/abi.hip
+++ b/mocapv2_amd/csrc/abi.hip
@@ -92,6 +92,7 @@
     int cluster = 1;
     int wide_quads_remap = 34, wide_quads_identity = 34;
     int wide_bands = 1;
+    int wide_split = 1;
     int wide_fork = 0;
     int box_prio = 0, scan_prio = 0, contour_prio = 0, corr_prio = 0;
     int box_stage_bytes = BOX_SCAP;
@@ -121,7 +122,7 @@
     {"rows", &Tuning::rows, 16, 68}, {"general_filter", &Tuning::general_filter, 0, 1}, {"skip_dark", &Tuning::skip_dark, 0, 1},
     {"dense_boxes", &Tuning::dense_boxes, 0, 1}, {"remap_pipeline", &Tuning::remap_pipeline, 0, 1}, {"cluster", &Tuning::cluster, 0, 1},
     {"wide_quads_remap", &Tuning::wide_quads_remap, 0, 100000}, {"wide_quads_identity", &Tuning::wide_quads_identity, 0, 100000},
-    {"wide_bands", &Tuning::wide_bands, 1, 4}, {"wide_fork", &Tuning::wide_fork, 0, 1},
+    {"wide_bands", &Tuning::wide_bands, 1, 4}, {"wide_fork", &Tuning::wide_fork, 0, 1}, {"wide_split", &Tuning::wide_split, 0, 1},
     {"box_prio", &Tuning::box_prio, 0, 1}, {"scan_prio", &Tuning::scan_prio, 0, 3}, {"contour_prio", &Tuning::contour_prio, 0, 3},
     {"corr_prio", &Tuning::corr_prio, 0, 3}, {"box_stage_bytes", &Tuning::box_stage_bytes, 0, BOX_SCAP},
     {"box_blocks_per_cu", &Tuning::box_blocks_per_cu, 0, 32}, {"box_timing", &Tuning::box_timing, 0, 1},
@@ -179,6 +180,7 @@
     Buf<uint32_t> tile_rows;
     int tile_rows_flip = 0;
     int tile_rows_hold[2] = {0, 0};
+    Buf<uint32_t> tile_cols;
     Buf<uint32_t> cur_box;
     Buf<BoxItem> items;
     Buf<uint4> wide_tiles;
@@ -515,6 +517,17 @@
     return MOCAP_OK;
 }
 
+int mocap_work_stats(mocap_ctx_t c, uint32_t out[3])
+{
+    if (!c || !out) return fail(MOCAP_E_INVALID, "mocap_work_stats: null argument");
+    if (set_device(c)) return MOCAP_E_HIP;
+    uint32_t cnt[16];
+    HIP_TRY(hipDeviceSynchronize());
+    HIP_TRY(hipMemcpy(cnt, c->n_items, sizeof(cnt), hipMemcpyDeviceToHost));
+    out[0] = cnt[0]; out[1] = cnt[8]; out[2] = cnt[9];
+    return MOCAP_OK;
+}
+
 int mocap_tile_stats(mocap_ctx_t c, uint64_t* tiles, uint64_t* skipped)
 {
     if (!c) return fail(MOCAP_E_INVALID, "null context");
@@ -630,7 +643,7 @@
     auto t5 = [](int n) { return (n - 1 < 2 ? n - 1 : 2) + 1; };
     auto t5full = [](int n) { return n < 5 ? n : 5; };
     const long long per_tap = 1024LL * (2LL * thr_mul - 2LL * b.base - 1), per_tap_alt = 1024LL * (2LL * thr_mul - 2LL * b.base_alt - 1);
-    if (!c->tile_rows || !c->reach || !c->cflags) ok = false;
+    if (!c->tile_rows || !c->tile_cols || !c->reach || !c->cflags) ok = false;
     if (ok && wmax > 0 && per_tap > 0) {
         b.allow = (int)((per_tap * t5full(c->W) * t5full(c->H) - 1) / wmax);
         const long long taps1 = t5(c->W) * t5full(c->H) < t5full(c->W) * t5(c->H) ? t5(c->W) * t5full(c->H) : t5full(c->W) * t5(c->H);
@@ -713,6 +726,9 @@
     a.tile_rows = c->tile_rows + (c->tile_rows_flip ? tr_words : 0);
     a.tile_rows_next = c->tile_rows + (c->tile_rows_flip ? 0 : tr_words);
     a.n_clear = c->tile_rows_hold[c->tile_rows_flip ^ 1];
+    a.tile_cols = c->tile_cols + (c->tile_rows_flip ? tr_words / 4 : 0);
+    a.tile_cols_next = c->tile_cols + (c->tile_rows_flip ? 0 : tr_words / 4);
+    a.wide_split = c->tune.wide_split;
     a.cluster = c->tune.cluster;
     a.cur_box = bt.own_mask ? c->cur_box : c->cur_box_ext;
     a.items = c->items; a.n_items = c->n_items; a.cap_items = (uint32_t)c->items.n;
@@ -727,7 +743,8 @@
     return a;
 }
 
-static BrightArgs bright_args(const mocap_ctx* c, const Batch& bt, const FilterPath& p, const ScanBounds& sb, uint32_t* tile_rows, bool scan_zeroes)
+static BrightArgs bright_args(const mocap_ctx* c, const Batch& bt, const FilterPath& p, const ScanBounds& sb, uint32_t* tile_rows, uint32_t* tile_cols,
+                              bool scan_zeroes)
 {
     const Tiling tl = tiling(c);
     uint64_t ncx64 = (uint64_t)((c->W + 7) / 8);
@@ -746,14 +763,15 @@
     b.zero_counters = scan_zeroes ? c->n_items.p : nullptr;
     b.block_ctr = c->n_items + 160;
     b.slices = c->tune.scan_slices; b.image0 = 0; b.slice_images = bt.n_images;
+    b.tile_cols = tile_cols;
     return b;
 }
 
-static int scan_tiles(mocap_ctx* c, const Batch& bt, const FilterPath& p, const ScanBounds& sb, uint32_t* tile_rows, bool scan_zeroes,
-                      BrightArgs& b, bool& mark_after_scan)
+static int scan_tiles(mocap_ctx* c, const Batch& bt, const FilterPath& p, const ScanBounds& sb, uint32_t* tile_rows, uint32_t* tile_cols,
+                      bool scan_zeroes, BrightArgs& b, bool& mark_after_scan)
 {
     const hipStream_t s = bt.s;
-    b = bright_args(c, bt, p, sb, tile_rows, scan_zeroes);
+    b = bright_args(c, bt, p, sb, tile_rows, tile_cols, scan_zeroes);
     const bool probe = sb.fixed_base < 0 && !c->probe_pending && sb.allow_alt >= 0 && sb.base_alt != sb.base && !p.bayer &&
                        (c->probe_age == 0 || c->probe_age >= 32);
     if (probe) {
@@ -895,7 +913,7 @@
     a.zero8 = bt.own_mask ? c->walk_count.p : nullptr;
     c->walk_count_zeroed = a.zero8 != nullptr;
     BrightArgs mark_args{}; bool mark_after_scan = false;
-    if (!a.dense) TRY(scan_tiles(c, bt, p, sb, a.tile_rows, scan_zeroes, mark_args, mark_after_scan));
+    if (!a.dense) TRY(scan_tiles(c, bt, p, sb, a.tile_rows, a.tile_cols, scan_zeroes, mark_args, mark_after_scan));
     else if (p.bayer) {
         launch_bayer_gray(p.bl, s);
         HIP_TRY(hipGetLastError());
@@ -1030,6 +1048,8 @@
     TRY(c->tile_rows.reserve(2 * init.size()));
     HIP_TRY(hipMemcpy(c->tile_rows, init.data(), sizeof(uint32_t) * init.size(), hipMemcpyHostToDevice));
     HIP_TRY(hipMemcpy(c->tile_rows + init.size(), init.data(), sizeof(uint32_t) * init.size(), hipMemcpyHostToDevice));
+    TRY(c->tile_cols.reserve(2 * tiles));
+    HIP_TRY(hipMemset(c->tile_cols, 0, sizeof(uint32_t) * 2 * tiles));
     const int hw0 = hot_map_words(c->H, c->W, 0), hw1 = hot_map_words(c->H, c->W, 1);
     TRY(c->hotmap.reserve(n_images * (hw0 > hw1 ? hw0 : hw1), true));
     for (size_t i = 0; i < init.size(); i++) init[i] = 1u;
@@ -1047,7 +1067,7 @@
     if ((size_t)n_images <= c->mask_images) return 0;
     c->mask_images = 0; c->last_images = 0;
     if (int rc = grow_mask_group(c, n_images)) {
-        c->mask.release(); c->cells.release(); c->tile_rows.release(); c->hotmap.release(); c->cur_box.release();
+        c->mask.release(); c->cells.release(); c->tile_rows.release(); c->tile_cols.release(); c->hotmap.release(); c->cur_box.release();
         c->items.release(); c->wide_tiles.release();
         return rc;
     }
diff --git a/mocapv2_amd/csrc/bayer_gray.hip b/mocapv2_amd/csrc/bayer_gray.hip
--- a/mocapv2_amd/csrc/bayer_gray.hip
+++ b/mocapv2_amd/csrc/bayer_gray.hip
@@ -185,9 +185,10 @@
         const uint2* __restrict__ reach = b.reach + (size_t)slot * n;
         const uint8_t* __restrict__ cflags = b.cflags + (size_t)slot * n;
         uint32_t* __restrict__ rows = b.tile_rows + (size_t)image * b.n_chunks * b.n_strips * 4;
+        uint32_t* __restrict__ cols = b.tile_cols + (size_t)image * b.n_chunks * b.n_strips;
         const int ci = cy * ncx + (x0 >> 3);
-        mark_hot_cell(b, reach, cflags, rows, ci, acc0);
-        mark_hot_cell(b, reach, cflags, rows, ci + 1, acc1);
+        mark_hot_cell(b, reach, cflags, rows, cols, ci, acc0);
+        mark_hot_cell(b, reach, cflags, rows, cols, ci + 1, acc1);
     }
 }
 
diff --git a/mocapv2_amd/csrc/blob_boxes.hip b/mocapv2_amd/csrc/blob_boxes.hip
--- a/mocapv2_amd/csrc/blob_boxes.hip
+++ b/mocapv2_amd/csrc/blob_boxes.hip
@@ -3,6 +3,7 @@
 #include <type_traits>
 #include "kernels.h"
 #include "bayer.h"
+#include "tile_cut.h"
 
 namespace mocap {
 
@@ -97,23 +98,6 @@
 {
     const int n = ((W + 7) >> 3) * ((H + 7) >> 3);
     hipLaunchKernelGGL(srcbox_kernel, dim3((n + 63) / 64), dim3(64), 0, s, map4, srcbox, H, W);
-}
-
-__device__ __forceinline__ void choose_split(int nb, int h, int& nx, int& ny)
-{
-    int best = 0x7fffffff;
-    nx = 1; ny = 1;
-    for (int cx = 1; cx <= 4; cx++) {
-        const int pb = (nb + cx - 1) / cx, Q = 2 * pb + 2;
-        if (Q > 64) continue;
-        const int rpw = 64 / Q, mr = BOX_HCAP / Q - 8;
-        if (mr < 1) continue;
-        const int cy = (h + mr - 1) / mr;
-        if (cx * cy > BOX_MAX_PARTS) continue;
-        const int ph = (h + cy - 1) / cy;
-        const int cost = cx * cy * ((ph + 8 + rpw - 1) / rpw + 8);
-        if (cost < best) { best = cost; nx = cx; ny = cy; }
-    }
 }
 
 __global__ __launch_bounds__(256) void settle_tiles_kernel(BoxArgs a)
@@ -138,7 +122,10 @@
     const size_t idx = ((size_t)image * a.n_chunks + chunk) * a.n_strips + strip;
     if (valid && !a.dense && image < n_all) {
         const uint4 nxt = *(const uint4*)(a.tile_rows_next + 4 * idx);
-        if (nxt.x <= nxt.y) *(uint4*)(a.tile_rows_next + 4 * idx) = make_uint4(0xffffffffu, 0u, 0xffffffffu, 0u);
+        if (nxt.x <= nxt.y) {
+            *(uint4*)(a.tile_rows_next + 4 * idx) = make_uint4(0xffffffffu, 0u, 0xffffffffu, 0u);
+            a.tile_cols_next[idx] = 0u;
+        }
     }
     valid = valid && image < a.n_images;
     const int tile_r0 = chunk * a.rows_per_chunk, tile_r1 = imin(tile_r0 + a.rows_per_chunk, a.H) - 1;
@@ -157,6 +144,8 @@
     if (!marked) { ox0 = 1; ox1 = 0; oy0 = 1; oy1 = 0; }
     int nx = 0, ny = 0, nb = 0, h = 0;
     bool wide = false;
+    uint32_t cut = 0u;
+    int cut_parts = 0;
     int ix0 = ox0, ix1 = ox1, iy0 = oy0, iy1 = oy1;
     int ux0 = bx0, ux1 = bx1, uy0 = by0, uy1 = by1;
     bool emits = marked;
@@ -187,7 +176,10 @@
         choose_split(nb, h, nx, ny);
         const int slot_ = image % a.cam_mod;
         const int limit = ((a.remap_bits >> slot_) & 1ull) ? a.wide_quads_remap : a.wide_quads_identity;
-        wide = emits && ix0 == ox0 && ix1 == ox1 && iy0 == oy0 && iy1 == oy1 && a.wide_tiles != nullptr && 2 * nb + 2 * nx >= limit;
+        const bool wide_box = emits && ix0 == ox0 && ix1 == ox1 && iy0 == oy0 && iy1 == oy1 && 2 * nb + 2 * nx >= limit;
+        if (wide_box && a.wide_split && !a.dense)
+            cut = cut_wide_tile(a.tile_cols[idx], (ox0 - tile_x0) >> 3, (ox1 - tile_x0) >> 3, h, limit, cut_parts);
+        wide = wide_box && !cut && a.wide_tiles != nullptr;
         if (wide) { ox0 = tile_x0; ox1 = tile_x1; ix0 = ox0; ix1 = ox1; }
     }
     const uint32_t nout_x = (uint32_t)ox0 | ((uint32_t)ox1 << 16), nout_y = (uint32_t)oy0 | ((uint32_t)oy1 << 16);
@@ -200,7 +192,7 @@
             const uint4 prev = *cb;
             pout_x = prev.x; pout_y = prev.y;
             const int px0 = (int)(prev.x & 0xffffu), px1 = (int)(prev.x >> 16), py0 = (int)(prev.y & 0xffffu), py1 = (int)(prev.y >> 16);
-            if (px0 <= px1) need_clear = !(marked && ox0 <= px0 && px1 <= ox1 && oy0 <= py0 && py1 <= oy1);
+            if (px0 <= px1) need_clear = cut || !(marked && ox0 <= px0 && px1 <= ox1 && oy0 <= py0 && py1 <= oy1);
             if (prev.x != nout_x || prev.y != nout_y || marked)
                 *cb = make_uint4(nout_x, nout_y, (uint32_t)bx0 | ((uint32_t)bx1 << 16), (uint32_t)by0 | ((uint32_t)by1 << 16));
             if (a.cells[idx] != 0u) a.cells[idx] = 0u;
@@ -237,7 +229,10 @@
             }
         }
     }
-    const int cnt = (wide || !emits) ? 0 : nx * ny;
+    if (uint64_t cb = __ballot(cut != 0u)) {
+        if (lane == 0) atomicAdd(a.n_items + 9, (uint32_t)__popcll(cb));
+    }
+    const int cnt = (wide || !emits) ? 0 : (cut ? cut_parts : nx * ny);
     int incl = cnt;
 #pragma unroll
     for (int d = 1; d < 64; d <<= 1) {
@@ -250,11 +245,11 @@
     if (lane == 0) base = atomicAdd(a.n_items, (uint32_t)wave_total);
     base = (uint32_t)__builtin_amdgcn_readfirstlane((int)base);
     uint32_t o = base + (uint32_t)(incl - cnt);
-    if (cnt) {
-        const int pb = (nb + nx - 1) / nx, ph = (h + ny - 1) / ny;
-        for (int jy = 0; jy < ny; jy++)
-            for (int jx = 0; jx < nx; jx++, o++) {
-                const int x0 = ix0 + 8 * pb * jx, x1 = imin(x0 + 8 * pb - 1, ix1);
+    auto emit = [&](int rx0, int rx1, int nbr, int nxr, int nyr, int ex0, int ex1) __attribute__((always_inline)) {
+        const int pb = (nbr + nxr - 1) / nxr, ph = (h + nyr - 1) / nyr;
+        for (int jy = 0; jy < nyr; jy++)
+            for (int jx = 0; jx < nxr; jx++, o++) {
+                const int x0 = rx0 + 8 * pb * jx, x1 = imin(x0 + 8 * pb - 1, rx1);
                 const int y0 = iy0 + ph * jy, y1 = imin(y0 + ph - 1, iy1);
                 if (o >= a.cap_items) continue;
                 uint4 it;
@@ -264,8 +259,20 @@
                 it.w = (uint32_t)y0 | ((uint32_t)y1 << 16);
                 if (x0 > x1 || y0 > y1) it.z = 1u;
                 ((uint4*)a.items)[2 * o] = it;
-                ((uint4*)a.items)[2 * o + 1] = make_uint4((uint32_t)ux0 | ((uint32_t)ux1 << 16), (uint32_t)uy0 | ((uint32_t)uy1 << 16), 0u, 0u);
-            }
+                ((uint4*)a.items)[2 * o + 1] = make_uint4((uint32_t)ex0 | ((uint32_t)ex1 << 16), (uint32_t)uy0 | ((uint32_t)uy1 << 16), 0u, 0u);
+            }
+    };
+    if (cnt && !cut) emit(ix0, ix1, nb, nx, ny, ux0, ux1);
+    else if (cnt) {
+        const int b_last = (tile_x1 - tile_x0) >> 3;
+        for (uint32_t m = cut; m;) {
+            const int b0 = __builtin_ctz(m), len = __builtin_ctz(~(m >> b0));
+            m &= ~(((1u << len) - 1u) << b0);
+            const int rx0 = tile_x0 + 8 * b0, rx1 = imin(rx0 + 8 * len - 1, tile_x1);
+            int nxr, nyr;
+            choose_split(len, h, nxr, nyr);
+            emit(rx0, rx1, len, nxr, nyr, imax(bx0, rx0 - (b0 == 0 ? 4 : 0)), imin(bx1, rx1 + (b0 + len - 1 == b_last ? 4 : 0)));
+        }
     }
 }
 
diff --git a/mocapv2_amd/csrc/blob_filter.hip b/mocapv2_amd/csrc/blob_filter.hip
--- a/mocapv2_amd/csrc/blob_filter.hip
+++ b/mocapv2_amd/csrc/blob_filter.hip
@@ -209,6 +209,7 @@
     const uint2* __restrict__ reach = a.reach + (size_t)slot * n;
     const uint8_t* __restrict__ cflags = a.cflags + (size_t)slot * n;
     uint32_t* __restrict__ rows = a.tile_rows + (size_t)image * a.n_chunks * a.n_strips * 4;
+    uint32_t* __restrict__ cols = a.tile_cols + (size_t)image * a.n_chunks * a.n_strips;
     const uint32_t base4 = (uint32_t)a.base * 0x01010101u, c8 = 8u * (uint32_t)a.base;
     uint32_t level[2] = {0u, 0u};
 #pragma unroll
@@ -226,7 +227,7 @@
             }
         }
         if (MAP) level[u] = in_range[u] ? hot_level(a, acc) : 0u;
-        else mark_hot_cell(a, reach, cflags, rows, ci[u], acc);
+        else mark_hot_cell(a, reach, cflags, rows, cols, ci[u], acc);
         if (a.probe && (image & 15) == 0) {
             const uint32_t alt4 = (uint32_t)a.base_alt * 0x01010101u, alt8 = 8u * (uint32_t)a.base_alt;
             uint32_t acc2 = 0;
@@ -269,7 +270,7 @@
 __global__ __launch_bounds__(256) void mark_tiles_kernel(BrightArgs a)
 {
     __shared__ uint16_t s_list[4][1024];
-    __shared__ uint32_t s_tab[4][32][5];
+    __shared__ uint32_t s_tab[4][32][6];
     const int lane = threadIdx.x & 63, wv = threadIdx.x >> 6;
     const int wpi = (a.hot_words + 255) >> 8;
     const int n_cells = ((a.W + 7) >> 3) * ((a.H + 7) >> 3);
@@ -286,19 +287,22 @@
 #pragma unroll
     for (int k = 0; k < 4; k++)
         if (wk[k] != 0u) hm[wave_word0 + 64 * k + lane] = 0u;
-    uint32_t (*tab)[5] = s_tab[wv];
-    if (lane < 32) { tab[lane][0] = 0xffffffffu; tab[lane][1] = 0xffffffffu; tab[lane][2] = 0u; tab[lane][3] = 0xffffffffu; tab[lane][4] = 0u; }
+    uint32_t (*tab)[6] = s_tab[wv];
+    if (lane < 32) { tab[lane][0] = 0xffffffffu; tab[lane][1] = 0xffffffffu; tab[lane][2] = 0u; tab[lane][3] = 0xffffffffu; tab[lane][4] = 0u; tab[lane][5] = 0u; }
     const int slot = image % a.cam_mod;
     const uint2* __restrict__ reach = a.reach + (size_t)slot * n_cells;
     const uint8_t* __restrict__ cflags = a.cflags + (size_t)slot * n_cells;
     uint32_t* __restrict__ rows = a.tile_rows + (size_t)image * a.n_chunks * a.n_strips * 4;
-    auto widen = [&](int t, uint32_t ya, uint32_t yb, uint32_t xa, uint32_t xb) __attribute__((always_inline)) {
+    uint32_t* __restrict__ cols = a.tile_cols + (size_t)image * a.n_chunks * a.n_strips;
+    auto widen = [&](int t, uint32_t ya, uint32_t yb, uint32_t xa, uint32_t xb, uint32_t bits) __attribute__((always_inline)) {
         const uint4 cur = *(const uint4*)(rows + 4 * t);
-        if (cur.x <= ya && cur.y >= yb && cur.z <= xa && cur.w >= xb) return;
-        atomicMin(&rows[4 * t], ya);
-        atomicMax(&rows[4 * t + 1], yb);
-        atomicMin(&rows[4 * t + 2], xa);
-        atomicMax(&rows[4 * t + 3], xb);
+        if (!(cur.x <= ya && cur.y >= yb && cur.z <= xa && cur.w >= xb)) {
+            atomicMin(&rows[4 * t], ya);
+            atomicMax(&rows[4 * t + 1], yb);
+            atomicMin(&rows[4 * t + 2], xa);
+            atomicMax(&rows[4 * t + 3], xb);
+        }
+        if ((cols[t] & bits) != bits) atomicOr(&cols[t], bits);
     };
 #pragma unroll 1
     for (int k = 0; k < 4; k++) {
@@ -337,12 +341,14 @@
                         for (int ch = ch0; ch <= ch1; ch++)
                             for (int st = st0; st <= st1; st++) {
                                 const int t = ch * a.n_strips + st, q = t & 31;
+                                const uint32_t bits = tile_column_bits(xa, xb, st);
                                 const uint32_t old = atomicCAS(&tab[q][0], 0xffffffffu, (uint32_t)t);
                                 if (old == 0xffffffffu || old == (uint32_t)t) {
                                     atomicMin(&tab[q][1], (uint32_t)ya); atomicMax(&tab[q][2], (uint32_t)yb);
                                     atomicMin(&tab[q][3], (uint32_t)xa); atomicMax(&tab[q][4], (uint32_t)xb);
+                                    atomicOr(&tab[q][5], bits);
                                 } else
-                                    widen(t, (uint32_t)ya, (uint32_t)yb, (uint32_t)xa, (uint32_t)xb);
+                                    widen(t, (uint32_t)ya, (uint32_t)yb, (uint32_t)xa, (uint32_t)xb, bits);
                             }
                     }
                 }
@@ -351,7 +357,7 @@
         __builtin_amdgcn_s_waitcnt(0xc07f);
         __builtin_amdgcn_wave_barrier();
     }
-    if (lane < 32 && tab[lane][0] != 0xffffffffu) widen((int)tab[lane][0], tab[lane][1], tab[lane][2], tab[lane][3], tab[lane][4]);
+    if (lane < 32 && tab[lane][0] != 0xffffffffu) widen((int)tab[lane][0], tab[lane][1], tab[lane][2], tab[lane][3], tab[lane][4], tab[lane][5]);
     __builtin_amdgcn_s_waitcnt(0xc07f);
     __builtin_amdgcn_wave_barrier();
     }
diff --git a/mocapv2_amd/csrc/kernels.h b/mocapv2_amd/csrc/kernels.h
--- a/mocapv2_amd/csrc/kernels.h
+++ b/mocapv2_amd/csrc/kernels.h
@@ -86,6 +86,9 @@
     uint32_t* tile_rows;
     uint32_t* tile_rows_next;
     int n_clear;
+    uint32_t* tile_cols;
+    uint32_t* tile_cols_next;
+    int wide_split;
     int cluster;
     uint32_t* cur_box;
     BoxItem* items; uint32_t* n_items; uint32_t cap_items;
@@ -187,6 +190,7 @@
     int hot_words;
     uint32_t* zero_counters;
     int mark_grid;
+    uint32_t* tile_cols;
 };
 int hot_map_words(int H, int W, int wide);
 void launch_mark_tiles(const BrightArgs& a, hipStream_t s);
diff --git a/mocapv2_amd/csrc/scan_mark.h b/mocapv2_amd/csrc/scan_mark.h
--- a/mocapv2_amd/csrc/scan_mark.h
+++ b/mocapv2_amd/csrc/scan_mark.h
@@ -14,7 +14,14 @@
     return s - c8;
 }
 
-__device__ __forceinline__ void widen_tile_boxes(const BrightArgs& a, const uint2 rc, uint32_t* __restrict__ rows)
+__host__ __device__ __forceinline__ uint32_t tile_column_bits(int xa, int xb, int st)
+{
+    const int tx0 = 240 * st;
+    const int ca = xa > tx0 ? (xa - tx0) >> 3 : 0, cb = (xb - tx0 < 239 ? xb - tx0 : 239) >> 3;
+    return (2u << cb) - (1u << ca);
+}
+
+__device__ __forceinline__ void widen_tile_boxes(const BrightArgs& a, const uint2 rc, uint32_t* __restrict__ rows, uint32_t* __restrict__ cols)
 {
     const int x0 = (int)(rc.x & 0xffffu), x1 = (int)(rc.x >> 16), y0 = (int)(rc.y & 0xffffu), y1 = (int)(rc.y >> 16);
     if (x0 > x1) return;
@@ -32,15 +39,21 @@
             atomicMin(&rows[4 * t + 2], (uint32_t)xa);
             atomicMax(&rows[4 * t + 3], (uint32_t)xb);
         }
+    for (int ch = ch0; ch <= ch1; ch++)
+        for (int st = st0; st <= st1; st++) {
+            const int t = ch * a.n_strips + st;
+            const uint32_t bits = tile_column_bits(xa, xb, st);
+            if ((cols[t] & bits) != bits) atomicOr(&cols[t], bits);
+        }
 }
 
 __device__ __forceinline__ void mark_hot_cell(const BrightArgs& a, const uint2* __restrict__ reach, const uint8_t* __restrict__ cflags,
-                                              uint32_t* __restrict__ rows, int ci, uint32_t acc)
+                                              uint32_t* __restrict__ rows, uint32_t* __restrict__ cols, int ci, uint32_t acc)
 {
     if ((int)acc > a.hot_corner) {
         const uint2 rc = reach[ci];
         const uint32_t fl = cflags[ci];
-        if ((int)acc > ((fl & 2u) ? a.hot_corner : (fl & 1u) ? a.hot_edge : a.hot)) widen_tile_boxes(a, rc, rows);
+        if ((int)acc > ((fl & 2u) ? a.hot_corner : (fl & 1u) ? a.hot_edge : a.hot)) widen_tile_boxes(a, rc, rows, cols);
     }
 }
 
diff --git a/mocapv2_amd/csrc/tile_cut.h b/mocapv2_amd/csrc/tile_cut.h
--- /dev/null
+++ b/mocapv2_amd/csrc/tile_cut.h
@@ -0,0 +1,56 @@
+#pragma once
+#include <stdint.h>
+#include "kernels.h"
+
+namespace mocap {
+
+__host__ __device__ __forceinline__ void choose_split(int nb, int h, int& nx, int& ny)
+{
+    int best = 0x7fffffff;
+    nx = 1; ny = 1;
+    for (int cx = 1; cx <= 4; cx++) {
+        const int pb = (nb + cx - 1) / cx, Q = 2 * pb + 2;
+        if (Q > 64) continue;
+        const int rpw = 64 / Q, mr = BOX_HCAP / Q - 8;
+        if (mr < 1) continue;
+        const int cy = (h + mr - 1) / mr;
+        if (cx * cy > BOX_MAX_PARTS) continue;
+        const int ph = (h + cy - 1) / cy;
+        const int cost = cx * cy * ((ph + 8 + rpw - 1) / rpw + 8);
+        if (cost < best) { best = cost; nx = cx; ny = cy; }
+    }
+}
+
+__host__ __device__ __forceinline__ uint32_t cut_wide_tile(uint32_t marks, int b0, int b1, int h, int limit, int& parts)
+{
+    parts = 0;
+    if (b0 < 0 || b1 > 29 || b0 > b1) return 0u;
+    uint32_t m = marks & ((2u << b1) - (1u << b0));
+    for (;;) {
+        const int runs = __builtin_popcount(m & ~(m << 1));
+        if (runs < 2) return 0u;
+        if (runs <= BOX_MAX_PARTS) {
+            bool ok = true;
+            int total = 0;
+            for (uint32_t r = m; r;) {
+                const int s = __builtin_ctz(r), len = __builtin_ctz(~(r >> s));
+                r &= ~(((1u << len) - 1u) << s);
+                int nx, ny;
+                choose_split(len, h, nx, ny);
+                ok = ok && 2 * len + 2 * nx < limit;
+                total += nx * ny;
+            }
+            if (ok && total <= BOX_MAX_PARTS) { parts = total; return m; }
+        }
+        const int lo = __builtin_ctz(m), hi = 31 - __builtin_clz(m);
+        int best_s = 0, best_len = 32;
+        for (uint32_t g = ~m & ((1u << hi) - (1u << lo));  g;) {
+            const int s = __builtin_ctz(g), len = __builtin_ctz(~(g >> s));
+            g &= ~(((1u << len) - 1u) << s);
+            if (len < best_len) { best_len = len; best_s = s; }
+        }
+        m |= ((1u << best_len) - 1u) << best_s;
+    }
+}
+
+}
diff --git a/mocapv2_amd/engine.py b/mocapv2_amd/engine.py
--- a/mocapv2_amd/engine.py
+++ b/mocapv2_amd/engine.py
@@ -495,6 +495,11 @@
         _abi.check(self.lib.mocap_tile_stats(self._h, C.byref(a), C.byref(b)))
         return a.value, b.value
 
+    def work_stats(self):
+        out = (C.c_uint32 * 3)()
+        _abi.check(self.lib.mocap_work_stats(self._h, out))
+        return int(out[0]), int(out[1]), int(out[2])
+
     def profile(self, on=True):
         _abi.check(self.lib.mocap_profile_enable(self._h, int(on)))
 
```

Measured after the change: 386,600 frames/s. -1.4%, worse.
